# baoe/AlignGraph

Measured on AMD Instinct MI355X. Metric: aligned reads/sec through graph build+extend, higher is better.
Workload: dtype u32

## Files before the change

### aligngraph_amd/__init__.py

```python
import ctypes
import os

_HERE = os.path.dirname(os.path.abspath(__file__))
LIB_PATH = os.environ.get("AGX_LIB_PATH", os.path.join(_HERE, "libagx.so"))

AGX_OK, AGX_E_IO, AGX_E_FORMAT, AGX_E_UNSUPPORTED, AGX_E_ALIGNMENT, AGX_E_DEVICE, AGX_E_ARG, AGX_E_OVERFLOW, AGX_E_NOGPU = 0, -1, -2, -3, -4, -5, -6, -7, -8
AGX_FLAG_KEEP_COUNTS = 1
AGX_FLAG_SPARSE_MIN = 2
AGX_FLAG_TIME_SECTIONS = 4
AGX_FLAG_ONE_SHOT = 8
AGX_FLAG_KEEP_PATHS = 16
AGX_FLAG_EDGE_SUPPORT = 32

EXPORTS = [
    "agx_version", "agx_device_count", "agx_device_memory", "agx_selftest_scan", "agx_unit_create", "agx_unit_destroy", "agx_unit_error", "agx_unit_set_reference",
    "agx_unit_set_contig_threads", "agx_unit_push_pairs", "agx_unit_load_files", "agx_unit_upload", "agx_unit_build", "agx_unit_download",
    "agx_unit_finish", "agx_result_free", "agx_unit_stats", "agx_unit_graph", "agx_graph_free", "agx_run_unit",
    "agx_reads_open", "agx_reads_close", "agx_unit_load_files_shared", "agx_run_unit_shared",
    "agx_unit_stage", "agx_unit_release", "agx_pool_trim", "agx_unit_cache_build", "agx_unit_cache_save", "agx_unit_hbm_needed",
    "agx_unit_trim", "agx_unit_unitigs", "agx_unit_unitigs_region", "agx_unitigs_free", "agx_unitigs_gfa", "agx_text_free",
    "agx_unit_walk_graph", "agx_walk_graph_free", "agx_unit_front", "agx_front_free",
    "agx_unit_unitigs_mapped", "agx_idmap_free", "agx_unit_walk_paths", "agx_walk_paths_free", "agx_unitigs_paths_gfa", "agx_unit_reprune",
    "agx_unit_edge_support", "agx_edge_support_free", "agx_unit_unitigs_support", "agx_link_support_free", "agx_unitigs_gfa_support",
    "agx_unit_walk_evidence", "agx_walk_evidence_free", "agx_walk_evidence_bed",
    "agx_test_scan", "agx_test_zero", "agx_test_copy_out",
]


class Params(ctypes.Structure):
    _fields_ = [("k", ctypes.c_uint32), ("insert_variation", ctypes.c_uint32), ("coverage", ctypes.c_uint32),
                ("batch", ctypes.c_uint32), ("device", ctypes.c_int32), ("flags", ctypes.c_uint32)]


class Run(ctypes.Structure):
    _fields_ = [("q", ctypes.c_uint32), ("t", ctypes.c_uint32), ("n", ctypes.c_uint32)]


class Hit(ctypes.Structure):
    _fields_ = [("slot1", ctypes.c_uint32), ("pos1", ctypes.c_uint32), ("pos2", ctypes.c_uint32), ("runs1", ctypes.c_uint32),
                ("runs2", ctypes.c_uint32), ("nruns1", ctypes.c_uint16), ("nruns2", ctypes.c_uint16), ("len", ctypes.c_uint16),
                ("rev1", ctypes.c_uint8), ("rev2", ctypes.c_uint8), ("back", ctypes.c_uint8), ("pad", ctypes.c_uint8 * 3)]


class ContiMer(ctypes.Structure):
    _fields_ = [("cid", ctypes.c_uint32), ("coff", ctypes.c_uint32), ("next_off", ctypes.c_uint32), ("next_item", ctypes.c_uint32),
                ("nuc", ctypes.c_char), ("pad", ctypes.c_char * 3)]


class PairBatch(ctypes.Structure):
    _fields_ = [("hits", ctypes.POINTER(Hit)), ("n_hits", ctypes.c_uint64), ("runs", ctypes.POINTER(Run)), ("n_runs", ctypes.c_uint64),
                ("bases", ctypes.c_char_p), ("stride", ctypes.c_uint32), ("n_slots", ctypes.c_uint32)]


class Result(ctypes.Structure):
    _fields_ = [("initial_contigs", ctypes.c_void_p), ("initial_len", ctypes.c_size_t), ("pre_extended", ctypes.c_void_p),
                ("pre_len", ctypes.c_size_t), ("extended", ctypes.c_void_p), ("extended_len", ctypes.c_size_t)]


class Stats(ctypes.Structure):
    _fields_ = [(n, ctypes.c_uint64) for n in ("n_pos", "n_ref", "n_hits", "n_runs", "n_nodes", "n_tiles", "n_tile_entries", "n_big_tiles",
                                                "n_edge_overflow", "pairs_in_file", "sam_line_pairs")] + \
               [(n, ctypes.c_double) for n in ("ms_parse", "ms_thread", "ms_upload", "ms_prep", "ms_bin", "ms_node_sweep", "ms_node_big",
                                                "ms_edge_sweep", "ms_compact", "ms_download", "ms_walk")] + \
               [("node_sweep_launches", ctypes.c_uint32), ("edge_sweep_launches", ctypes.c_uint32)] + \
               [(n, ctypes.c_uint64) for n in ("n_walk_ids", "n_special", "n_fetched", "download_bytes")] + \
               [(n, ctypes.c_double) for n in ("ms_edge_fast", "ms_edge_slow")] + [("n_mid_tiles", ctypes.c_uint64), ("ms_build_span", ctypes.c_double)] + \
               [(n, ctypes.c_double) for n in ("ms_stage", "ms_upload_dev")] + \
               [(n, ctypes.c_uint64) for n in ("upload_bytes", "device_bytes", "pinned_bytes_cached", "device_bytes_cached", "n_spilled")] + \
               [("build_attempts", ctypes.c_uint32), ("from_cache", ctypes.c_uint32), ("dense_lists", ctypes.c_uint32), ("rows_by_reference", ctypes.c_uint32)] + \
               [("n_edge_slow", ctypes.c_uint64), ("reprune_attempts", ctypes.c_uint32), ("ms_reprune", ctypes.c_double)] + \
               [("ms_edge_support", ctypes.c_double), ("n_support_events", ctypes.c_uint64), ("ms_walk_evidence", ctypes.c_double)]


class Graph(ctypes.Structure):
    _fields_ = [("n_pos", ctypes.c_uint32), ("n_nodes", ctypes.c_uint32), ("n_edges", ctypes.c_uint32),
                ("node_start", ctypes.POINTER(ctypes.c_uint32)), ("node_key", ctypes.POINTER(ctypes.c_uint32)),
                ("node_cnt", ctypes.POINTER(ctypes.c_int32)), ("node_slen", ctypes.POINTER(ctypes.c_uint32)),
                ("edge_start", ctypes.POINTER(ctypes.c_uint32)), ("edge_dst", ctypes.POINTER(ctypes.c_uint32))]


class Unitigs(ctypes.Structure):
    _fields_ = [("n_segs", ctypes.c_uint32), ("n_links", ctypes.c_uint32), ("n_bases", ctypes.c_uint64),
                ("head_pos", ctypes.POINTER(ctypes.c_uint32)), ("head_var", ctypes.POINTER(ctypes.c_uint32)), ("n_nodes", ctypes.POINTER(ctypes.c_uint32)),
                ("last_pos", ctypes.POINTER(ctypes.c_uint32)), ("coverage", ctypes.POINTER(ctypes.c_uint64)), ("seq_off", ctypes.POINTER(ctypes.c_uint64)),
                ("seq", ctypes.c_void_p), ("link_from", ctypes.POINTER(ctypes.c_uint32)), ("link_to", ctypes.POINTER(ctypes.c_uint32))]


class EdgeSupport(ctypes.Structure):
    _fields_ = [("n_nodes", ctypes.c_uint32), ("n_edges", ctypes.c_uint32), ("n_events", ctypes.c_uint64), ("n_contributions", ctypes.c_uint64)] + \
               [(n, ctypes.POINTER(ctypes.c_uint32)) for n in ("edge_start", "edge_dst", "edge_cnt")]


class IdMap(ctypes.Structure):
    _fields_ = [("n_runs", ctypes.c_uint32), ("n_pos", ctypes.c_uint32), ("n_ids", ctypes.c_uint32)] + \
               [(n, ctypes.POINTER(ctypes.c_uint32)) for n in ("id_first", "id_last", "seg", "rank_first")]


class WalkPaths(ctypes.Structure):
    _fields_ = [("n_recs", ctypes.c_uint32), ("n_stretches", ctypes.c_uint64), ("rec_len", ctypes.POINTER(ctypes.c_uint64)), ("st_off", ctypes.POINTER(ctypes.c_uint64)),
                ("id_first", ctypes.POINTER(ctypes.c_uint32)), ("id_last", ctypes.POINTER(ctypes.c_uint32)), ("base_off", ctypes.POINTER(ctypes.c_uint64)),
                ("joined", ctypes.POINTER(ctypes.c_uint8))]


class WalkEvidence(ctypes.Structure):
# ... 269 lines not shown
    def load_files(self, tmp_dir, unit, reads=None):
        self._check(lib().agx_unit_load_files_shared(self._h, tmp_dir.encode(), unit, reads._h if reads is not None else None))

    def cache_save(self, tmp_dir, unit):
        self._check(lib().agx_unit_cache_save(self._h, tmp_dir.encode(), unit))

    def stage(self):
        self._check(lib().agx_unit_stage(self._h))

    def hbm_needed(self):
        v = ctypes.c_uint64(0)
        self._check(lib().agx_unit_hbm_needed(self._h, ctypes.byref(v)))
        return v.value

    def upload(self):
        self._check(lib().agx_unit_upload(self._h))

    def trim(self):
        v = ctypes.c_uint64(0)
        self._check(lib().agx_unit_trim(self._h, ctypes.byref(v)))
        return v.value

    def release(self):
        self._check(lib().agx_unit_release(self._h))

    def build(self):
        self._check(lib().agx_unit_build(self._h))

    def reprune(self, coverage):
        if not 0 <= int(coverage) <= 0xFFFFFFFF:
            raise AgxError(AGX_E_ARG, "reprune: coverage is an unsigned 32-bit number")
        self._check(lib().agx_unit_reprune(self._h, int(coverage)))
        self.params.coverage = int(coverage)

    def download(self):
        self._check(lib().agx_unit_download(self._h))

    def finish(self):
        r = Result()
        self._check(lib().agx_unit_finish(self._h, ctypes.byref(r)))
        return _take(r)

    def finish_views(self):
        r = Result()
        self._check(lib().agx_unit_finish(self._h, ctypes.byref(r)))
        return ResultViews(r)

    def stats(self):
        s = Stats()
        self._check(lib().agx_unit_stats(self._h, ctypes.byref(s)))
        return {n: getattr(s, n) for n, _ in Stats._fields_}

    def graph(self):
        import numpy as np
        g = Graph()
        self._check(lib().agx_unit_graph(self._h, ctypes.byref(g)))

        def arr(p, n, dt):
            return np.ctypeslib.as_array(p, shape=(n,)).astype(dt, copy=True) if n else np.zeros(0, dt)
        out = {"n_pos": g.n_pos, "n_nodes": g.n_nodes, "n_edges": g.n_edges,
               "node_start": arr(g.node_start, g.n_pos + 1, "uint32"), "node_key": arr(g.node_key, g.n_nodes * 6, "uint32").reshape(-1, 6),
               "node_cnt": arr(g.node_cnt, g.n_nodes * 6, "int32").reshape(-1, 6), "node_slen": arr(g.node_slen, g.n_nodes, "uint32"),
               "edge_start": arr(g.edge_start, g.n_nodes + 1, "uint32"), "edge_dst": arr(g.edge_dst, g.n_edges, "uint32")}
        lib().agx_graph_free(ctypes.byref(g))
        return out

    def walk_graph(self, streamed=False, all_node=False):
        g = WalkGraph()
        g.want_all_node = 1 if all_node else 0
        self._check(lib().agx_unit_walk_graph(self._h, 1 if streamed else 0, ctypes.byref(g)))
        try:
            return walk_graph_arrays(g)
        finally:
            lib().agx_walk_graph_free(ctypes.byref(g))

    def front(self):
        f = Front()
        self._check(lib().agx_unit_front(self._h, ctypes.byref(f)))
        try:
            return front_arrays(f)
        finally:
            lib().agx_front_free(ctypes.byref(f))

    def _window(self, region, min_coverage):
        lo, hi = region if region is not None else (0, self.stats()["n_pos"])
        cov = self.params.coverage if min_coverage is None else min_coverage
        for v in (lo, hi, cov):
            if not 0 <= int(v) <= 0xFFFFFFFF:
                raise AgxError(AGX_E_ARG, "unitigs: region bounds and min_coverage are unsigned 32-bit numbers")
        return int(lo), int(hi), int(cov)

    def _export(self, t, region, min_coverage):
        if region is None and min_coverage is None:
            self._check(lib().agx_unit_unitigs(self._h, ctypes.byref(t)))
            return
        self._check(lib().agx_unit_unitigs_region(self._h, *self._window(region, min_coverage), ctypes.byref(t)))

    def edge_support(self):
        import numpy as np
        s = EdgeSupport()
        self._check(lib().agx_unit_edge_support(self._h, ctypes.byref(s)))
        try:
            def arr(p, n):
                return np.ctypeslib.as_array(p, shape=(n,)).astype("uint32", copy=True) if n else np.zeros(0, "uint32")
            return {"n_nodes": s.n_nodes, "n_edges": s.n_edges, "n_events": s.n_events, "n_contributions": s.n_contributions,
                    "edge_start": arr(s.edge_start, s.n_nodes + 1), "edge_dst": arr(s.edge_dst, s.n_edges), "edge_cnt": arr(s.edge_cnt, s.n_edges)}
        finally:
            lib().agx_edge_support_free(ctypes.byref(s))

    def _export_support(self, t, region, min_coverage, m=None):
        sup = ctypes.POINTER(ctypes.c_uint32)()
        self._check(lib().agx_unit_unitigs_support(self._h, *self._window(region, min_coverage), ctypes.byref(t), ctypes.byref(sup), ctypes.byref(m) if m is not None else None))
        return sup

    def unitigs(self, region=None, min_coverage=None, id_map=False, edge_support=False):
        if edge_support:
            return self._unitigs_support(region, min_coverage, id_map)
        t = Unitigs()
        if not id_map:
            self._export(t, region, min_coverage)
            try:
                return _unitigs_arrays(t)
            finally:
                lib().agx_unitigs_free(ctypes.byref(t))
        m = IdMap()
        self._check(lib().agx_unit_unitigs_mapped(self._h, *self._window(region, min_coverage), ctypes.byref(t), ctypes.byref(m)))
        try:
            out = _unitigs_arrays(t)
            out["id_map"] = _idmap_arrays(m)
            return out
        finally:
            lib().agx_unitigs_free(ctypes.byref(t))
            lib().agx_idmap_free(ctypes.byref(m))

    def _unitigs_support(self, region, min_coverage, id_map):
        import numpy as np
        t, m = Unitigs(), IdMap() if id_map else None
        sup = self._export_support(t, region, min_coverage, m)
        try:
            out = _unitigs_arrays(t)
            out["link_support"] = np.ctypeslib.as_array(sup, shape=(t.n_links,)).astype("uint32", copy=True) if t.n_links else np.zeros(0, "uint32")
            if id_map:
                out["id_map"] = _idmap_arrays(m)
            return out
        finally:
            lib().agx_unitigs_free(ctypes.byref(t))
            lib().agx_link_support_free(sup)
            if id_map:
                lib().agx_idmap_free(ctypes.byref(m))

    def walk_paths(self):
        import numpy as np
        w = WalkPaths()
        self._check(lib().agx_unit_walk_paths(self._h, ctypes.byref(w)))
        try:
            def arr(p, n, dt):
                return np.ctypeslib.as_array(p, shape=(n,)).astype(dt, copy=True) if n else np.zeros(0, dt)
            nr, ns = w.n_recs, w.n_stretches
            return {"rec_len": arr(w.rec_len, nr, "uint64"), "st_off": arr(w.st_off, nr + 1, "uint64"), "id_first": arr(w.id_first, ns, "uint32"),
                    "id_last": arr(w.id_last, ns, "uint32"), "base_off": arr(w.base_off, ns, "uint64"), "joined": arr(w.joined, ns, "uint8")}
        finally:
            lib().agx_walk_paths_free(ctypes.byref(w))

    def walk_evidence(self, w=None, min_depth=0, min_support=0, tracks=False, records=None):
        import numpy as np
        if w is None:
# ... 184 lines not shown
```

### aligngraph_amd/csrc/agx_core.h

```cpp
#pragma once
#include <stdint.h>
#include "../../include/agx.h"

#if defined(__HIPCC__)
#define AGX_HD __host__ __device__ __forceinline__
#else
#define AGX_HD inline
#endif

typedef uint32_t agx_u32;
typedef uint16_t agx_u16;
typedef uint8_t agx_u8;

#define AGX_NONE 0xFFFFFFFFu
#define AGX_TILE 64u
#ifndef AGX_REGION_TILES
#define AGX_REGION_TILES 32u
#endif
#define AGX_REGION_PAD 32u
#ifndef AGX_MAXV_LDS
#define AGX_MAXV_LDS 2u
#endif
#ifndef AGX_SWEEP_FIRST
#define AGX_SWEEP_FIRST 1
#endif
#define AGX_MAXV_MID 4u
#define AGX_MAXV_BIG 64u
#define AGX_MAXV_HUGE 1024u
#define AGX_MAXE 4u
#define AGX_EP25 25



enum { AGX_WF_REV1 = 1, AGX_WF_REV2 = 2, AGX_WF_LEFT2 = 4, AGX_WF_RUNS1 = 8, AGX_WF_RUNS2 = 16,
       AGX_WF_DUP = 32 };
struct agx_whit {
    agx_u32 a, b, row;
    agx_u16 len; agx_u8 flags, back;
};
struct agx_wside { agx_u32 runs1, runs2, nruns; };
struct agx_wrun { agx_u32 t; agx_u16 q, n; };
AGX_HD agx_whit agx_pack_hit(const agx_hit &h, agx_u32 side_index) {
    agx_whit w; w.a = h.nruns1 ? 0u : h.pos1; w.b = h.nruns2 ? 0u : h.pos2; w.row = h.slot1; w.len = h.len; w.back = h.back;
    w.flags = (agx_u8)((h.rev1 ? AGX_WF_REV1 : 0) | (h.rev2 ? AGX_WF_REV2 : 0) | ((h.pad[0] & 1u) ? AGX_WF_LEFT2 : 0) | (h.nruns1 ? AGX_WF_RUNS1 : 0) | (h.nruns2 ? AGX_WF_RUNS2 : 0));
    if (h.nruns1) w.a = side_index; else if (h.nruns2) w.b = side_index;
    return w;
}
AGX_HD agx_hit agx_unpack_hit(const agx_whit &w, const agx_wside *sides) {
    agx_hit h; h.slot1 = w.row; h.len = w.len; h.back = w.back; h.rev1 = (w.flags & AGX_WF_REV1) ? 1 : 0; h.rev2 = (w.flags & AGX_WF_REV2) ? 1 : 0;
    h.pad[0] = (w.flags & AGX_WF_LEFT2) ? 1 : 0; h.pad[1] = h.pad[2] = 0;
    h.pos1 = (w.flags & AGX_WF_RUNS1) ? 0u : w.a; h.pos2 = (w.flags & AGX_WF_RUNS2) ? 0u : w.b; h.runs1 = h.runs2 = 0; h.nruns1 = h.nruns2 = 0;
    if (w.flags & (AGX_WF_RUNS1 | AGX_WF_RUNS2)) {
        const agx_wside sd = sides[(w.flags & AGX_WF_RUNS1) ? w.a : w.b];
        if (w.flags & AGX_WF_RUNS1) { h.runs1 = sd.runs1; h.nruns1 = (agx_u16)(sd.nruns & 0xFFFFu); }
        if (w.flags & AGX_WF_RUNS2) { h.runs2 = sd.runs2; h.nruns2 = (agx_u16)(sd.nruns >> 16); }
    }
    return h;
}
struct agx_refx { agx_u32 pos, len, byte; };
AGX_HD agx_u32 agx_ref_code(agx_u32 c) { return c == 'A' ? 0u : c == 'C' ? 1u : c == 'G' ? 2u : c == 'T' ? 3u : 4u; }
AGX_HD char agx_ref_base(agx_u32 code) { return (char)((0x54474341u >> (8u * (code & 3u))) & 0xFFu); }

struct agx_cmkey { agx_u32 cid, coff; };
struct agx_cmhead { agx_u32 cid, coff, n, start; };


enum { AGX_HF_AREV = 1, AGX_HF_SKIP = 2, AGX_HF_BNONE = 4 };

struct agx_dhit {
    agx_u32 a_t0, b_t0;
    agx_u32 a_runs, b_runs;
    agx_u32 a_slot;
    agx_u16 len, jstar;
    agx_u16 a_nruns, b_nruns;
    agx_u32 flags;
    agx_u32 x_lo, x_hi;
};


enum { AGX_NF_DEAD = 1, AGX_NF_CONTIG = 2, AGX_NF_EOVF = 4 };

struct agx_sref { agx_u32 slot; agx_u32 qlen; };

enum { AGX_F_CID = 0, AGX_F_COFF, AGX_F_CID0, AGX_F_COFF0, AGX_F_OFF0, AGX_F_COV, AGX_F_A, AGX_F_C, AGX_F_G, AGX_F_T, AGX_F_N, AGX_F_S0, AGX_F_S1, AGX_NF };
static_assert(AGX_F_C == AGX_F_A + 1 && AGX_F_G == AGX_F_A + 2 && AGX_F_T == AGX_F_A + 3 && AGX_F_N == AGX_F_A + 4, "agx_class_vote_code relies on the order of the vote counters");

struct agx_key { agx_u32 cid, coff, cid0, coff0, off0; };

AGX_HD int agx_absdiff(agx_u32 a, agx_u32 b) { int d = (int)(a - b); return d < 0 ? -d : d; }

AGX_HD agx_u32 agx_within(agx_u32 a, agx_u32 b, int win) { return (agx_u32)(a - b + (agx_u32)win) <= 2u * (agx_u32)win ? 1u : 0u; }
AGX_HD agx_u32 agx_clause_ab(agx_u32 ac, agx_u32 ao, agx_u32 bc, agx_u32 bo, int win) {
    return ((agx_u32)(ac != bc) | (agx_u32)(ac == AGX_NONE) | agx_within(ao, bo, win)) & 1u;
}
AGX_HD agx_u32 agx_clause_c(agx_u32 ao, agx_u32 bo, int win) { return ((agx_u32)(ao == AGX_NONE) | (agx_u32)(bo == AGX_NONE) | agx_within(ao, bo, win)) & 1u; }

#if defined(__HIP_DEVICE_COMPILE__)
AGX_HD agx_u32 agx_uload(const agx_u32 *p, size_t i) { return ((const __attribute__((address_space(4))) agx_u32 *)p)[i]; }
#else
AGX_HD agx_u32 agx_uload(const agx_u32 *p, size_t i) { return p[i]; }
#endif

struct agx_bucket { agx_u32 *base; agx_u32 stride; agx_u32 maxv; agx_u32 packed; };
#define AGX_NFP 10u
static_assert(AGX_F_COV == AGX_F_OFF0 + 1 && AGX_F_A == AGX_F_COV + 1 && AGX_F_S0 == AGX_F_N + 1 && AGX_NFP == AGX_NF - 3,
              "packed buckets: the six counters from AGX_F_COV on pair up into three words, and agx_b maps S0 / S1 three words down");
AGX_HD agx_u32 &agx_b(const agx_bucket &b, agx_u32 v, agx_u32 f) { return b.base[(b.packed ? v * AGX_NFP + (f >= (agx_u32)AGX_F_S0 ? f - 3u : f) : v * AGX_NF + f) * b.stride]; }
AGX_HD agx_u32 &agx_cnt_word(const agx_bucket &b, agx_u32 v, agx_u32 f) { return b.base[(v * AGX_NFP + (agx_u32)AGX_F_COV + ((f - (agx_u32)AGX_F_COV) >> 1)) * b.stride]; }
template <bool LDS_ADD> AGX_HD void agx_bucket_add(agx_u32 &ref, agx_u32 val) {
#if defined(__HIP_DEVICE_COMPILE__)
    if (LDS_ADD) { (void)__hip_atomic_fetch_add(&ref, val, __ATOMIC_RELAXED, __HIP_MEMORY_SCOPE_WAVEFRONT); return; }
#endif
    ref += val;
}
AGX_HD agx_u32 agx_cnt_get(const agx_bucket &b, agx_u32 v, agx_u32 f) {
    if (b.packed) return (agx_cnt_word(b, v, f) >> (16u * ((f - (agx_u32)AGX_F_COV) & 1u))) & 0xFFFFu;
    return agx_b(b, v, f);
}
template <bool LDS_ADD> AGX_HD void agx_cnt_add(const agx_bucket &b, agx_u32 v, agx_u32 f, agx_u32 val) {
    if (b.packed) agx_bucket_add<LDS_ADD>(agx_cnt_word(b, v, f), val << (16u * ((f - (agx_u32)AGX_F_COV) & 1u)));
    else agx_bucket_add<LDS_ADD>(agx_b(b, v, f), val);
}
AGX_HD void agx_cnt_init(const agx_bucket &b, agx_u32 v, agx_u32 cov) {
    if (b.packed) { agx_cnt_word(b, v, AGX_F_COV) = cov; agx_cnt_word(b, v, AGX_F_C) = 0; agx_cnt_word(b, v, AGX_F_T) = 0; }
    else { agx_b(b, v, AGX_F_COV) = cov; agx_b(b, v, AGX_F_A) = 0; agx_b(b, v, AGX_F_C) = 0; agx_b(b, v, AGX_F_G) = 0; agx_b(b, v, AGX_F_T) = 0; agx_b(b, v, AGX_F_N) = 0; }
}

AGX_HD bool agx_compatible(const agx_key &k, const agx_bucket &b, agx_u32 v, int iv) {
    const agx_u32 c = agx_b(b, v, AGX_F_CID), o = agx_b(b, v, AGX_F_COFF), c0 = agx_b(b, v, AGX_F_CID0), o0 = agx_b(b, v, AGX_F_COFF0), m = agx_b(b, v, AGX_F_OFF0);
    return (agx_clause_ab(k.cid, k.coff, c, o, AGX_EP25) & agx_clause_ab(k.cid0, k.coff0, c0, o0, 2 * iv + AGX_EP25) & agx_clause_c(k.off0, m, 2 * iv + AGX_EP25)) != 0;
}


AGX_HD agx_u32 agx_pos_b(const agx_dhit &d, const agx_run *runs, agx_u32 q) {
    if (d.b_nruns == 0) return d.b_t0 + q;
    agx_u32 res = AGX_NONE;
    for (agx_u32 i = 0; i < d.b_nruns; i++) { const agx_run r = runs[d.b_runs + i]; const agx_u32 o = q - r.q; res = (q >= r.q && o < r.n) ? r.t + o : res; }
    return res;
}

// ... 1032 lines not shown
```

### aligngraph_amd/csrc/agx_engine.cpp

```cpp
#include <hip/hip_runtime_api.h>
#include <hsa/hsa.h>
#include <hsa/hsa_ext_amd.h>
#include <fcntl.h>
#include <sys/stat.h>
#include <unistd.h>

#include <algorithm>
#include <chrono>
#include <cstdio>
#include <cstdlib>
#include <cstring>
#include <memory>
#include <string>
#include <mutex>
#include <system_error>
#include <thread>
#include <type_traits>
#include <pthread.h>
#include <atomic>
#include <condition_variable>
#include <functional>
#include <vector>

#include "agx_host.h"
// ... 102 lines not shown
                try { f(); } catch (...) { }
                l.lock(); running[s] = false; cv.notify_all();
            }
        });
        started = true;
    }
    bool submit(int s, std::function<void()> f) {
        if (!started) return false;
        std::unique_lock<std::mutex> l(m);
        cv.wait(l, [&] { return !queued[s] && !running[s]; });
        job[s] = std::move(f); queued[s] = true; cv.notify_all();
        return true;
    }
    void wait(int s) { if (!started) return; std::unique_lock<std::mutex> l(m); cv.wait(l, [&] { return !queued[s] && !running[s]; }); }
    ~UnitHelper() { if (started) { { std::lock_guard<std::mutex> l(m); stop = true; } cv.notify_all(); th.join(); } }
};

struct WalkerPool {
    enum { N = 64 };
    struct Slot { std::thread th; std::mutex m; std::condition_variable cv; std::function<void()> job; bool queued = false, running = false, taken = false, stop = false; };
    Slot slot[N]; std::mutex take_m; bool started = false;
    void start() {
        if (started) return;
        started = true;
        for (Slot &s : slot) {
            try {
                s.th = std::thread([&s] {
                    pthread_setname_np(pthread_self(), "agx-walker");
                    std::unique_lock<std::mutex> l(s.m);
                    for (;;) {
                        s.cv.wait(l, [&s] { return s.stop || s.queued; });
                        if (s.stop) return;
                        std::function<void()> f = std::move(s.job); s.queued = false; s.running = true;
                        l.unlock();
                        try { f(); } catch (...) { }
                        l.lock(); s.running = false; s.cv.notify_all();
                    }
                });
            } catch (...) { s.taken = true; }
        }
    }
    int take() { std::lock_guard<std::mutex> l(take_m); start(); for (int i = 0; i < N; i++) if (!slot[i].taken) { slot[i].taken = true; return i; } return -1; }
    void give(int i) { std::lock_guard<std::mutex> l(take_m); slot[i].taken = false; }
    void run(int i, std::function<void()> f) { Slot &s = slot[i]; std::unique_lock<std::mutex> l(s.m); s.cv.wait(l, [&s] { return !s.queued && !s.running; }); s.job = std::move(f); s.queued = true; s.cv.notify_all(); }
    void wait(int i) { Slot &s = slot[i]; std::unique_lock<std::mutex> l(s.m); s.cv.wait(l, [&s] { return !s.queued && !s.running; }); }
    ~WalkerPool() { for (Slot &s : slot) if (s.th.joinable()) { { std::lock_guard<std::mutex> l(s.m); s.stop = true; } s.cv.notify_all(); s.th.join(); } }
};
WalkerPool &walker_pool() { static WalkerPool p; return p; }
inline int walkers_now(size_t n_pos) {
    const int want = walkers_wanted(n_pos);
    if (want <= 4 || getenv("AGX_WALK_SPLIT_WALKERS")) return want;
    static const int ranks = [] { const char *e = getenv("LOCAL_WORLD_SIZE"); const int n = e ? atoi(e) : 1; return n < 1 ? 1 : n; }();
    const int cpus = (int)usable_cpus() / ranks;
    return want <= cpus ? want : cpus < 4 ? 4 : cpus;
}

static std::atomic<int> g_walks_pending{0};
static std::atomic<int> g_units_alive{0};

struct agx_unit {
    agx_params prm{};
    std::string err;
    Threads T; Pairs P;
    UnitView V;
    size_t n_chain_str = 0;
    struct Mapped { void *p = nullptr; size_t n = 0; void reset() { if (p) munmap(p, n); p = nullptr; n = 0; } ~Mapped() { reset(); } } cache_map;
    agx_u32 n_seg0 = 0, stride = 0, n_slots = 0, n_rows = 0; unsigned long long pairs_in_file = 0, sam_pairs = 0;
    bool have_ref = false, have_threads = false, staged = false, uploaded = false, built = false, downloaded = false;
    bool consumed = false;
    bool pending_walk = false;
    bool trimmed = false;
    bool expanded = false;
    hipEvent_t ev_built = nullptr;
    UnitOutput out; OutBuf out_initial; bool out_ready = false;
    UnitHelper helper;
    hsa_signal_t dl_signal{}; hsa_agent_t dl_agent{}; bool dl_sdma = false;
    enum { DL_SIGNALS = AGX_DL_PIECES + 2 };
    hsa_signal_t dl_piece[DL_SIGNALS] = {}; bool dl_piece_made = false, dl_streaming = false; agx_cut_args cuts{}; agx_u32 cut_main[AGX_DL_PIECES + 1] = {}, cut_side[AGX_DL_PIECES + 1] = {};
    double dl_t0 = 0, dl_est_ms = 0; size_t dl_stream_bytes = 0; std::atomic<bool> dl_timed{false};
    DevArena arena;
    PBuf<agx_whit> s_hits; PBuf<agx_wside> s_sides; PBuf<agx_wrun> s_runs; PBuf<agx_u8> s_codes; PBuf<unsigned long long> s_other; PBuf<agx_u32> s_jump; size_t n_other = 0, n_sides = 0, n_jump = 0;
    PBuf<agx_u8> s_ref; PBuf<agx_refx> s_refx; size_t n_refx = 0; bool ref_packed = false;
    PBuf<agx_u32> s_chain_end, s_region_off; PBuf<agx_cmseg> s_segs; size_t n_segs = 0;
    PBuf<agx_whit> s_hits_t; PBuf<agx_u8> s_codes_t; PBuf<unsigned long long> s_other_t; size_t n_other_t = 0; bool tiled = false; std::vector<agx_u32> slot_row;
    agx_u32 front_windows = 1;
    agx_u32 n_win = 1, win_tile[9] = {};
    hipEvent_t ev_rows[8] = {}, ev_win[8] = {}, ev_sw0[8] = {}, ev_sw1[8] = {};
    PBuf<agx_u32> s_perm, s_tfirst, s_jump_at; agx_u32 lookback = 2;
    PBuf<char> s_landing;
    PBuf<agx_cntrun> s_cntruns; PBuf<agx_chunk> s_cntchunks, s_segchunks; PBuf<agx_u32> s_segindex; size_t n_cntruns = 0, n_cntchunks = 0, n_segchunks = 0, n_segindex = 0;
    PBuf<agx_u16> s_units; PBuf<agx_u8> s_rowcnt; PBuf<agx_u32> s_blockoff, s_blockfirst, s_anchor; size_t n_units = 0, n_rowcnt = 0, n_blockoff = 0, n_blockfirst = 0, n_anchor = 0, n_rows_explicit = 0; bool rows_diffed = false;
    size_t nh = 0, n_runs = 0, n_cm = 0, n_codes = 0; agx_u32 maxlen = 0;
    std::vector<agx_u32> row_slot;
    std::vector<uint64_t> row_off;
    std::shared_ptr<agx::ReadsIndex> reads_keep;
    std::unique_ptr<agx::FileView> reads_map;
    bool pairs_staged = false;
    agx::PairsFile pairs_file;
    DBuf<agx_u32> d_cm_start; DBuf<agx_cmkey> d_cm; DBuf<agx_cmhead> d_cm_head; DBuf<char> d_ref; DBuf<agx_cmseg> d_segs;
    DBuf<agx_run> d_runs; DBuf<agx_u8> d_codes, d_vcodes; DBuf<unsigned long long> d_other;
    DBuf<agx_u16> d_units; DBuf<agx_u8> d_rowcnt; DBuf<agx_u32> d_blockoff, d_blockfirst, d_anchor;
    DBuf<agx_cntrun> d_cntruns; DBuf<agx_chunk> d_cntchunks, d_segchunks; DBuf<agx_u32> d_jump, d_segindex;
    DBuf<agx_whit> d_whits; DBuf<agx_wside> d_wsides; DBuf<agx_wrun> d_wruns; DBuf<agx_u8> d_wref; DBuf<agx_refx> d_refx;
    DBuf<agx_dhit> d_dhit; DBuf<agx_u32> d_tile_cnt, d_tile_off, d_cursor, d_unsorted, d_tile_recs, d_scan_tmp, d_words; DBuf<unsigned long long> d_scan_desc; size_t scan_desc_n = 0;
    agx_u32 pool_cap = 0, spill_lo = 0, ovf_cap = 0, list_cap = 0, sp_cap = 0;
    DBuf<agx_u32> d_pool_cnt, d_region_off; agx_u32 n_regions = 0;
    DBuf<agx_u32> d_node_start, d_slow_list, d_perm, d_tfirst, d_ckey, d_long; DBuf<agx_u16> d_node_cnt; DBuf<agx_u8> d_pos_succ;
    DBuf<agx_u32> d_cid, d_coff, d_cid0, d_coff0, d_off0, d_next; DBuf<agx_u8> d_base, d_flags; DBuf<agx_sref> d_sref; DBuf<int> d_counts;
    DBuf<agx_u32> d_e_cnt, d_ovf_cnt, d_sup_tot, d_lsup;
    bool support_valid = false; uint64_t sup_events = 0, sup_adds = 0;
    DBuf<char> d_ut;
    DBuf<agx_edge_ovf> d_ovf; DBuf<agx_u32> d_mid_list, d_big_list, d_scratch, d_huge_list, d_scratch_huge; bool huge = false, dense = false;
    agx_u32 n_ids = 0;
    DBuf<agx_u32> d_side_pk, d_tile_side, d_tile_side_start, d_aid_of; DBuf<char> d_a_str;
    DBuf<agx_u8> d_a_meta, d_a_mark; DBuf<agx_walknode> d_fetch, d_sp_node; DBuf<agx_u32> d_a_nid; DBuf<agx_edge_ovf> d_a_ovf; agx_compact_args walk_args{};
    DBuf<agx_u32> d_chain_end, d_side_xpos, d_sp_cnt, d_sp_rank; DBuf<unsigned long long> d_sp_bits;
    agx_u32 n_chain_end = 0, n_special = 0, n_words = 0;
    size_t keep_end = 0;
    PBuf<char> h_a_str; PBuf<agx_u8> h_a_meta; PBuf<agx_u32> h_side_xpos, h_sp_rank; PBuf<unsigned long long> h_sp_bits;
    PBuf<agx_walknode> h_sp_node, h_fetch; PBuf<agx_edge_ovf> h_a_ovf; PBuf<agx_hop> h_sp_hop; DBuf<agx_hop> d_sp_hop;
    PBuf<agx_u32> h_words;
    agx_u32 n_nodes = 0, n_ovf = 0, n_tiles = 0, n_tile_entries = 0, n_big = 0, n_mid = 0, n_slow = 0;
    Boundaries ev; hipEvent_t ev_front = nullptr, ev_passA = nullptr, ev_passJ = nullptr, ev_up0 = nullptr, ev_uploaded = nullptr, ev_dl = nullptr, ev_hits = nullptr;
    bool up_timed = false;
    agx_stats stats{};
    ~agx_unit() {
        arena.reset();
        if (pending_walk) g_walks_pending.fetch_sub(1);
        ev.destroy();
        for (hipEvent_t e : {ev_front, ev_passA, ev_passJ, ev_up0, ev_uploaded, ev_dl, ev_built, ev_hits}) if (e) (void)hipEventDestroy(e);
        for (auto *arr : {ev_rows, ev_win, ev_sw0, ev_sw1}) for (int i = 0; i < 8; i++) if (arr[i]) (void)hipEventDestroy(arr[i]);
        if (dl_signal.handle) (void)hsa_signal_destroy(dl_signal);
        if (dl_piece_made) for (hsa_signal_t g : dl_piece) if (g.handle) (void)hsa_signal_destroy(g);
    }
};

namespace {

struct DeviceTurn { std::mutex m; hipStream_t main = nullptr, front = nullptr, up = nullptr, down = nullptr;
                    hipEvent_t sweep_done[2] = {nullptr, nullptr}, build_done[2] = {nullptr, nullptr};
                    unsigned long long n = 0; bool prev_exclusive = false; hipEvent_t prev_node = nullptr;
                    std::mutex up_m, down_m, make_m;
                    void make() {
                        std::lock_guard<std::mutex> l(make_m);
                        if (main) return;
                        HIP_OK(hipStreamCreateWithFlags(&up, hipStreamNonBlocking)); HIP_OK(hipStreamCreateWithFlags(&front, hipStreamNonBlocking));
                        HIP_OK(hipStreamCreateWithFlags(&down, hipStreamNonBlocking));
                        for (auto &e : sweep_done) HIP_OK(hipEventCreateWithFlags(&e, hipEventDisableTiming));
                        for (auto &e : build_done) HIP_OK(hipEventCreateWithFlags(&e, hipEventDisableTiming));
                        HIP_OK(hipStreamCreateWithFlags(&main, hipStreamNonBlocking));
                    } };
DeviceTurn &turn_of(int device) { static DeviceTurn turns[64]; return turns[device & 63]; }

static const bool g_trace_gap = getenv("AGX_TRACE_GAP") != nullptr;
static const bool g_scan1 = getenv("AGX_SCAN_LEGACY") == nullptr;
static const bool g_debug_sync = getenv("AGX_DEBUG_SYNC") != nullptr;
#define g_tiny (getenv("AGX_TEST_SMALL_CAPS") != nullptr)
#define AGX_CHECKPOINT(name) do { if (g_debug_sync) { hipError_t e_ = hipStreamSynchronize(st); fprintf(stderr, "[agx debug] %s: %s\n", name, hipGetErrorString(e_)); } } while (0)

void join_dl_helper(agx_unit *u);
void drop_outputs(agx_unit *u);
void start_helper(agx_unit *u);

enum { W_CUT = 34 , W_TOTAL = W_CUT + 2 * (AGX_DL_PIECES + 1) };
enum { W_ERR = 0, W_POOL = 1, W_BIGCOUNT = 2, W_STATUS = 3, W_OVFCOUNT = 4, W_SLOWCOUNT = 5, W_LONGCOUNT = 6 , W_UNUSED7 = 7, W_MIDCOUNT = 8, W_JUMPCOUNT = 9, W_SPILL = 10, W_HUGECOUNT = 11, W_N = 12 };

agx_cut_args stream_cuts(agx_u32 n_pos) {
    agx_cut_args C; memset(&C, 0, sizeof C);
    const char *force = getenv("AGX_STREAM_PIECES");
    if (getenv("AGX_NO_STREAM_DOWNLOAD") || n_pos < 4096) return C;
    size_t m = force ? (size_t)atoi(force) : n_pos < AGX_TWO_WALKERS_MIN ? 0 : n_pos / 4000000u;
    if (!force && m && m < 2) m = 2;
    if (m > AGX_DL_PIECES) m = AGX_DL_PIECES;
    if (m > n_pos / 1024u) m = n_pos / 1024u;
    for (size_t w = 0; w < m; w++) C.word[w] = (agx_u32)(((unsigned long long)n_pos * w / m) >> 6);
    C.word[m] = n_pos >> 6; C.n = (agx_u32)m;
    return C;
}

void fill_sweep_args(agx_unit *u, agx_sweep_args &S) {
    memset(&S, 0, sizeof S);
    S.cm_start = u->d_cm_start.p; S.cm = u->d_cm.p; S.cm_head = u->d_cm_head.p; S.ref = u->d_ref.p;
    S.dhit = u->d_dhit.p; S.runs = u->d_runs.p; S.vcodes = u->d_vcodes.p; S.stride = u->stride;
    S.tile_off = u->d_tile_off.p; S.tile_recs = (decltype(S.tile_recs))u->d_tile_recs.p;
    S.n_pos = (agx_u32)u->V.n_pos; S.n_tiles = u->n_tiles; S.k = u->prm.k; S.iv = (int)u->prm.insert_variation; S.coverage = (int)u->prm.coverage;
    S.node_start = u->d_node_start.p; S.node_cnt = u->d_node_cnt.p; S.pos_succ = u->d_pos_succ.p; S.side_pk = u->d_side_pk.p; S.tile_side = u->d_tile_side.p;
    S.nk_cid = u->d_cid.p; S.nk_coff = u->d_coff.p; S.nk_cid0 = u->d_cid0.p; S.nk_coff0 = u->d_coff0.p; S.nk_off0 = u->d_off0.p;
    S.n_base = u->d_base.p; S.n_flags = u->d_flags.p; S.n_sref = u->d_sref.p; S.n_next = u->d_next.p;
    S.n_counts = (u->prm.flags & AGX_FLAG_KEEP_COUNTS) ? u->d_counts.p : nullptr;
    S.pool_cap = u->pool_cap;
    S.sweep_stats = nullptr;
}

inline bool want_tiled() { return !getenv("AGX_NO_TILED_UPLOAD"); }
template <class B> inline void alloc_file_order(B &buf, size_t count) { if (want_tiled()) buf.alloc_plain(count); else buf.alloc(count); }
void *alloc_pair_array(agx_unit *u, int which, size_t bytes) {
    switch (which) {
    case SA_HITS:  alloc_file_order(u->s_hits, bytes / sizeof(agx_whit) + 1); return u->s_hits.p;
    case SA_SIDES: u->s_sides.alloc(bytes / sizeof(agx_wside) + 1); return u->s_sides.p;
    case SA_RUNS:  u->s_runs.alloc(bytes / sizeof(agx_wrun) + 1); return u->s_runs.p;
    case SA_CODES: alloc_file_order(u->s_codes, bytes); return u->s_codes.p;
    case SA_JUMP:  u->s_jump.alloc(bytes / 4 + 1); return u->s_jump.p;
    default:       u->s_other.alloc(bytes / 8 + 1); return u->s_other.p;
    }
}
void alloc_pair_arrays(agx_unit *u) {
    alloc_pair_array(u, SA_HITS, u->nh * sizeof(agx_whit)); alloc_pair_array(u, SA_SIDES, u->n_sides * sizeof(agx_wside)); alloc_pair_array(u, SA_JUMP, u->n_jump * 4);
    alloc_pair_array(u, SA_RUNS, u->n_runs * sizeof(agx_wrun)); alloc_pair_array(u, SA_CODES, u->n_codes + 16); alloc_pair_array(u, SA_OTHER, u->n_other * 8);
}
struct UnitSink : StageSink {
    agx_unit *u; explicit UnitSink(agx_unit *x) : u(x) {}
    void *take(int which, size_t bytes) override { return alloc_pair_array(u, which, bytes); }
};
void adopt_pairs(agx_unit *u, StagedPairs &S) {
    u->nh = S.nh; u->n_runs = S.n_runs; u->n_sides = S.n_sides; u->n_jump = S.n_jump; u->n_codes = S.n_codes; u->n_other = S.n_other; u->stride = S.stride; u->maxlen = S.maxlen;
    u->pairs_in_file = S.n_pairs_in_file; u->sam_pairs = S.n_sam_pairs;
    u->row_off.swap(S.row_off); u->row_slot.swap(S.row_slot); u->n_rows = S.n_rows;
}
void stage_cm_layout(agx_unit *u, const agx_u8 *cm_cnt, size_t n_pos, const agx_cmseg *segs, size_t n_segs) {
    CmLayout L; build_cm_layout(cm_cnt, n_pos, segs, n_segs, L);
    u->n_cntruns = L.cnt_runs.size(); u->n_cntchunks = L.cnt_chunks.size(); u->n_segchunks = L.seg_chunks.size();
    u->s_cntruns.alloc(u->n_cntruns + 1); u->s_cntchunks.alloc(u->n_cntchunks + 1); u->s_segchunks.alloc(u->n_segchunks + 1);
    if (u->n_cntruns) memcpy(u->s_cntruns.p, L.cnt_runs.data(), u->n_cntruns * sizeof(agx_cntrun));
    if (u->n_cntchunks) memcpy(u->s_cntchunks.p, L.cnt_chunks.data(), u->n_cntchunks * sizeof(agx_chunk));
    if (u->n_segchunks) memcpy(u->s_segchunks.p, L.seg_chunks.data(), u->n_segchunks * sizeof(agx_chunk));
    build_seg_index(segs, u->n_seg0, n_pos, L.seg_index);
    u->n_segindex = L.seg_index.size(); u->s_segindex.alloc(u->n_segindex + 1); memcpy(u->s_segindex.p, L.seg_index.data(), u->n_segindex * 4);
}
void stage_reference(agx_unit *u, const char *ref, size_t n_pos, unsigned threads) {
    std::vector<agx_refx> others;
    u->s_ref.alloc((n_pos + 3) / 4 + 32);
    u->ref_packed = getenv("AGX_REF_RAW") == nullptr && pack_reference(ref, n_pos, std::min(threads, 8u), u->s_ref.p, others);
    if (u->ref_packed) { u->n_refx = others.size(); u->s_refx.alloc(u->n_refx + 1); if (u->n_refx) memcpy(u->s_refx.p, others.data(), u->n_refx * sizeof(agx_refx)); return; }
    u->n_refx = 0; u->s_ref.alloc(n_pos + 16);
    const unsigned T = std::max(1u, std::min(threads, 8u));
    on_threads(T, [&](unsigned t) { const size_t lo = n_pos * t / T, hi = n_pos * (t + 1) / T; memcpy(u->s_ref.p + lo, ref + lo, hi - lo); });
}
struct GraphCounts { size_t n_pos, n_ids, n_special, n_ovf; };
enum { GA_BITS = 0, GA_RANK, GA_STR, GA_META, GA_XPOS, GA_NODE, GA_HOP, GA_OVF, GA_N };
template <class F> void graph_arrays(agx_unit *u, const GraphCounts &c, F f) {
    const size_t words = c.n_ids / 64 + 1, sides = c.n_ids - c.n_pos;
    f(GA_BITS, u->h_sp_bits, u->d_sp_bits, words, 1); f(GA_RANK, u->h_sp_rank, u->d_sp_rank, words, 1);
    f(GA_STR, u->h_a_str, u->d_a_str, c.n_ids, 1); f(GA_META, u->h_a_meta, u->d_a_meta, c.n_ids, 64);
    f(GA_XPOS, u->h_side_xpos, u->d_side_xpos, sides, 1);
    f(GA_NODE, u->h_sp_node, u->d_sp_node, c.n_special, 1); f(GA_HOP, u->h_sp_hop, u->d_sp_hop, c.n_special, 2);
    f(GA_OVF, u->h_a_ovf, u->d_a_ovf, c.n_ovf, 1);
}
const int GRAPH_CUT_ORDER[GA_N] = {GA_NODE, GA_META, GA_STR, GA_HOP, GA_XPOS, GA_BITS, GA_RANK, GA_OVF};
inline GraphCounts graph_counts(const agx_unit *u) { return GraphCounts{u->V.n_pos, u->n_ids, u->n_special, u->n_ovf}; }
inline size_t graph_bytes(agx_unit *u, const GraphCounts &c) {
    size_t sum = 0; graph_arrays(u, c, [&](int, auto &h, auto &, size_t n, size_t) { sum += n * sizeof(*h.p); }); return sum;
}
inline GraphCounts helper_estimate(size_t n_pos) { const size_t ni = n_pos + n_pos / 8 + 4096; return GraphCounts{n_pos, ni, ni / 8 + 4096, 63}; }
inline GraphCounts landing_estimate(size_t n_pos) { const size_t ni = n_pos + n_pos / 16 + 4096; return GraphCounts{n_pos, ni, ni / 10 + 4096, 0}; }

const int LANDING_ROOMS = 8;
template <class F> void landing_rooms(agx_unit *u, F f) {
    f(u->s_codes, true); f(u->s_hits, true); f(u->s_landing, false); f(u->s_codes_t, true); f(u->s_hits_t, true); f(u->s_runs, true); f(u->s_sides, true); f(u->s_other, true);
}

void reserve_landing(agx_unit *u) {
    if (!(u->prm.flags & AGX_FLAG_ONE_SHOT)) { u->s_landing.release(); return; }
    const GraphCounts c = landing_estimate(u->V.n_pos); const size_t ni = c.n_ids, ns = c.n_special;
    const size_t need = 2 * (ni + 512) + ns * (sizeof(agx_walknode) + sizeof(agx_hop)) + ni / 4 + (4u << 20);
    size_t have = 0; landing_rooms(u, [&](auto &b, bool input) { if (input) have += b.block_bytes(); });
    if (need > have * 85 / 100) u->s_landing.alloc(need - have * 85 / 100 + (ni + 512)); else u->s_landing.release();
}
void adopt_row_diffs(agx_unit *u, const RowDiffs &D, unsigned threads) {
    u->n_units = D.n_units; u->n_rowcnt = D.cnt.size(); u->n_blockoff = D.block_off.size(); u->n_blockfirst = D.block_first.size(); u->n_anchor = D.anchor_bits.size(); u->n_rows_explicit = D.n_explicit;
    u->s_units.alloc(u->n_units + 2); u->s_rowcnt.alloc(u->n_rowcnt); u->s_blockoff.alloc(u->n_blockoff); u->s_blockfirst.alloc(u->n_blockfirst); u->s_anchor.alloc(u->n_anchor);
    const unsigned T = std::max(1u, std::min(threads, 8u));
    on_threads(T, [&](unsigned t) { const size_t lo = u->n_units * t / T, hi = u->n_units * (t + 1) / T; if (hi > lo) memcpy(u->s_units.p + lo, D.units.data() + lo, (hi - lo) * 2); });
    memcpy(u->s_rowcnt.p, D.cnt.data(), u->n_rowcnt); memcpy(u->s_blockoff.p, D.block_off.data(), u->n_blockoff * 4); memcpy(u->s_blockfirst.p, D.block_first.data(), u->n_blockfirst * 4); memcpy(u->s_anchor.p, D.anchor_bits.data(), u->n_anchor * 4);
    u->rows_diffed = true;
}
void stage_rows(agx_unit *u, unsigned threads) {
    u->rows_diffed = false; u->n_units = u->n_rowcnt = u->n_blockoff = u->n_blockfirst = u->n_anchor = u->n_rows_explicit = 0;
    const char *on = getenv("AGX_ROW_DIFF");
    if (want_tiled()) return;
    if (!on || atoi(on) == 0 || !u->ref_packed || u->n_rows == 0 || u->nh == 0) return;
    const double t0 = now_ms();
    RowDiffs D;
    if (!build_row_diffs(u->s_hits.p, u->nh, u->s_sides.p, u->n_sides, u->s_runs.p, u->n_runs, u->s_codes.p, u->n_rows, u->stride, (const agx_u32 *)u->s_ref.p, u->V.n_pos ? u->V.n_pos : u->T.ref.size(), threads, D)) return;
    if (D.n_units * 2 + D.cnt.size() + (D.block_off.size() + D.block_first.size() + D.anchor_bits.size()) * 4 >= u->n_codes) return;
    adopt_row_diffs(u, D, threads);
    if (getenv("AGX_LOAD_TIMING")) fprintf(stderr, "[agx load] read rows against the reference: %.1f ms, %zu rows (%zu as they are), %.1f -> %.1f bytes per row\n", now_ms() - t0, (size_t)u->n_rows, u->n_rows_explicit,
                                          (double)u->n_codes / u->n_rows, (double)(u->n_units * 2 + u->n_rowcnt + (u->n_blockoff + u->n_blockfirst + u->n_anchor) * 4) / u->n_rows);
}
void stage_order(agx_unit *u, unsigned threads) {
    const double t0 = now_ms();
    const size_t n_pos = u->V.n_pos ? u->V.n_pos : u->T.ref.size(), n_tiles = (n_pos + AGX_TILE - 1) / AGX_TILE;
    u->lookback = agx_tile_lookback(u->maxlen, u->prm.k);
    u->s_perm.alloc(u->nh + 1); u->s_tfirst.alloc(n_tiles + 2); u->s_jump_at.alloc(u->n_jump + 1);
    order_hits(u->s_hits.p, u->nh, u->s_sides.p, u->s_runs.p, u->s_jump.p, u->n_jump, n_pos, threads, u->s_perm.p, u->s_tfirst.p, u->s_jump_at.p);
    if (getenv("AGX_LOAD_TIMING")) fprintf(stderr, "[agx load] hits in tile order: %.1f ms (%zu hits, %zu tiles, window of %u tiles)\n", now_ms() - t0, u->nh, n_tiles, u->lookback);
}
void stage_tiled(agx_unit *u, unsigned threads) {
    u->tiled = false; u->n_other_t = 0; u->slot_row.clear(); u->n_win = 1;
    const size_t nh = u->nh, s4 = u->stride / 4;
    if (u->rows_diffed || getenv("AGX_NO_TILED_UPLOAD") || nh == 0 || u->n_rows == 0) { u->s_hits_t.release(); u->s_codes_t.release(); u->s_other_t.release(); return; }
    const double t0 = now_ms();
    u->s_hits_t.alloc(nh + 1); u->s_codes_t.alloc(nh * s4 + 16); u->slot_row.resize(nh);
    const agx_whit *wh = u->s_hits.p; const agx_wside *sd = u->s_sides.p; const agx_wrun *wr = u->s_runs.p; const agx_u32 *perm = u->s_perm.p;
    const size_t n_rows = u->n_rows; std::vector<agx_u8> has_other((n_rows + 7) / 8, 0);
    for (size_t j = 0; j < u->n_other; j++) { const size_t r = (size_t)(u->s_other.p[j] / u->stride); if (r < n_rows) has_other[r >> 3] |= (agx_u8)(1u << (r & 7)); }
    auto idx0 = [&](const agx_whit &w) -> agx_u32 {
        if (!(w.flags & AGX_WF_RUNS1)) return w.a;
        const agx_wside &g = sd[w.a]; const agx_wrun &r = wr[g.runs1];
        return r.q == 0 ? r.t : AGX_NONE;
    };
    const unsigned T = std::max(1u, std::min(threads, 16u));
    std::vector<std::vector<unsigned long long>> others(T);
    on_threads(T, [&](unsigned t) {
        const size_t AHEAD = 48, NEAR = 24;
        for (size_t i = nh * t / T, hi = nh * (t + 1) / T; i < hi; i++) {
            if (i + AHEAD < hi) __builtin_prefetch(wh + perm[i + AHEAD]);
            if (i + NEAR < hi) { const char *c = (const char *)(u->s_codes.p + (size_t)wh[perm[i + NEAR]].row * s4); __builtin_prefetch(c); if (s4 > 40) __builtin_prefetch(c + 64); }
            const agx_u32 h = perm[i]; agx_whit w = wh[h];
            const agx_u32 row = w.row;
            u->slot_row[i] = row;
            memcpy(u->s_codes_t.p + i * s4, u->s_codes.p + (size_t)row * s4, s4);
            bool dup = false;
            if (w.back) { const agx_u32 me = idx0(w); for (agx_u32 e = 1; e <= w.back && !dup; e++) dup = agx_absdiff(me, idx0(wh[h - e])) < (int)w.len; }
            w.row = h; if (dup) w.flags |= (agx_u8)AGX_WF_DUP;
            u->s_hits_t.p[i] = w;
            if (has_other[row >> 3] & (1u << (row & 7))) {
                const unsigned long long lo = (unsigned long long)row * u->stride, *b = u->s_other.p, *e = b + u->n_other;
                for (const unsigned long long *at = std::lower_bound(b, e, lo); at != e && *at < lo + u->stride; ++at) others[t].push_back((unsigned long long)i * u->stride + (*at - lo));
            }
        }
    });
    size_t no = 0; for (auto &v : others) no += v.size();
    u->s_other_t.alloc(no + 1); u->n_other_t = no;
    { size_t at = 0; for (auto &v : others) { if (!v.empty()) memcpy(u->s_other_t.p + at, v.data(), v.size() * 8); at += v.size(); } }
    u->tiled = true;
    const size_t n_pos = u->V.n_pos ? u->V.n_pos : u->T.ref.size(), n_tiles = (n_pos + AGX_TILE - 1) / AGX_TILE;
    size_t W = getenv("AGX_UPLOAD_WINDOWS") ? (size_t)atoi(getenv("AGX_UPLOAD_WINDOWS")) : n_pos / 8000000u;
    W = std::max<size_t>(1, std::min<size_t>(std::min<size_t>(W, 8), n_tiles));
    u->n_win = (agx_u32)W;
    for (size_t w = 0; w <= W; w++) u->win_tile[w] = (agx_u32)(n_tiles * w / W);
    if (getenv("AGX_LOAD_TIMING")) fprintf(stderr, "[agx load] tile-ordered upload forms: %.1f ms (%zu hits, %zu listed bases, %u windows)\n", now_ms() - t0, nh, no, u->n_win);
}

void stage_rows_tiled(agx_unit *u, unsigned threads) {
    if (!u->tiled || !u->ref_packed || u->stride > AGX_ROW_MAXSTRIDE) return;
    const char *env = getenv("AGX_ROW_DIFF");
    const size_t n_pos = u->V.n_pos ? u->V.n_pos : u->T.ref.size();
    if (!env || atoi(env) == 0) return;
    const double t0 = now_ms();
    RowDiffs D;
    if (!build_row_diffs(u->s_hits_t.p, u->nh, u->s_sides.p, u->n_sides, u->s_runs.p, u->n_runs, u->s_codes_t.p, u->nh, u->stride, (const agx_u32 *)u->s_ref.p, n_pos, threads, D, true)) return;
    if (D.n_units * 2 + D.cnt.size() + (D.block_off.size() + D.block_first.size() + D.anchor_bits.size()) * 4 >= u->nh * (u->stride / 4)) return;
    adopt_row_diffs(u, D, threads);
    if (getenv("AGX_LOAD_TIMING")) fprintf(stderr, "[agx load] tile-ordered rows against the reference: %.1f ms, %zu rows (%zu as they are), %.1f -> %.1f bytes per row\n", now_ms() - t0, u->nh, u->n_rows_explicit,
                                          (double)(u->stride / 4), (double)(u->n_units * 2 + u->n_rowcnt + (u->n_blockoff + u->n_blockfirst + u->n_anchor) * 4) / u->nh);
}

void finish_staging(agx_unit *u, unsigned threads_rows, unsigned threads) {
    stage_rows(u, threads_rows);
    stage_order(u, threads);
    stage_tiled(u, threads);
    stage_rows_tiled(u, threads);
    u->V.slot_row = u->tiled ? u->slot_row.data() : nullptr;
    reserve_landing(u);
    u->staged = true; u->consumed = false; u->uploaded = false; u->built = false; u->downloaded = false;
}

void stage_inputs(agx_unit *u) {
    if (!u->have_ref || !u->have_threads) throw Error{E_ARG, "reference and contig threads must be set before upload"};
    if (u->consumed && u->pairs_staged) throw Error{E_ARG, "one-shot unit: its staged read alignments were overwritten by the download; load the unit again"};
    const double t0 = now_ms();
    HIP_OK(hipSetDevice(u->prm.device));
    u->cache_map.reset(); u->reads_map.reset();
    const size_t n_pos = u->T.ref.size();
    if (n_pos == 0 || n_pos >= 0xFFFFFF00ull) throw Error{E_ARG, "unit sequence is empty or too long"};
    if (u->T.cm_cnt.size() != n_pos) throw Error{E_ARG, "conti-mer chains were not built"};
    { size_t el = 0; for (const agx_cmseg &g : u->T.segs) el += g.len; if (el != u->T.n_cm) throw Error{E_ARG, "conti-mer runs were not built"}; }
    u->n_seg0 = u->T.n_seg0; u->n_cm = u->T.n_cm;
    u->n_segs = u->T.segs.size(); u->s_segs.alloc(u->n_segs + 1);
    if (u->n_segs) memcpy(u->s_segs.p, u->T.segs.data(), u->n_segs * sizeof(agx_cmseg));
    std::vector<agx_u32> ce(u->T.chain_end_pos); std::sort(ce.begin(), ce.end()); ce.erase(std::unique(ce.begin(), ce.end()), ce.end());
    u->n_chain_end = (agx_u32)ce.size(); u->s_chain_end.alloc(ce.size() + 1);
    if (!ce.empty()) memcpy(u->s_chain_end.p, ce.data(), ce.size() * 4);
    const unsigned threads = loader_threads(u->P.bases.size() + n_pos + u->nh * 64);
    stage_reference(u, u->T.ref.data(), n_pos, threads);
    stage_cm_layout(u, u->T.cm_cnt.data(), n_pos, u->T.segs.data(), u->n_segs);
    if (!u->pairs_staged) {
        UnitSink sink(u); StagedPairs S;
        u->n_slots = u->P.n_slots;
        stage_pairs(u->P, u->prm.k, threads, sink, S);
        adopt_pairs(u, S);
    }
    UnitView V = view_of(u->T, u->P);
    if (u->pairs_staged && u->pairs_file.fv) {
        const agx::PairsFile &F = u->pairs_file;
        V.bases = nullptr; V.row_off = nullptr; V.stride = u->stride; V.codes2 = (const agx_u8 *)F.sec(pairsfile::S_CODES);
        V.other_idx = (const unsigned long long *)F.sec(pairsfile::S_OTHER); V.other_byte = (const agx_u8 *)F.sec(pairsfile::S_OTHERB); V.n_other = (size_t)F.H.n_other;
    } else if (u->pairs_staged) { V.bases = u->reads_keep ? u->reads_keep->fv.p : nullptr; V.stride = u->stride; V.row_off = u->row_off.data(); }
    u->V = V; u->n_chain_str = u->T.chain_str.size();
    finish_staging(u, threads, threads);
    u->stats.ms_stage = now_ms() - t0;
}

namespace cache {
enum { S_HITS = 0, S_RUNS, S_CODES, S_SEGS, S_CHAIN_END, S_ROWS, S_REF, S_CM_CNT, S_CHAIN_STR, S_INITIAL, S_BASES, S_OTHER, S_SIDES, S_JUMP, S_OTHERB, S_N };
struct Header {
    char magic[8]; agx_u32 version, batch; unsigned long long stamp[6][2];
    unsigned long long n_pos, n_ref, nh, n_runs, n_cm, n_segs, n_seg0, n_rows, n_chain_end, n_codes, pairs_in_file, sam_pairs;
    agx_u32 stride, maxlen, n_slots, k;
    agx_u32 rows_in_reads;
    agx_u32 slot_stride;
    unsigned long long n_sides, n_jump;
    agx_u32 sizes[5];
    unsigned long long off[S_N], len[S_N];
};
const char MAGIC[8] = {'A', 'G', 'X', 'U', 'N', 'I', 'T', '7'};
void stamps(const std::string &d, int unit, unsigned long long st[6][2]) {
    const std::string s = std::to_string(unit);
    const std::string f[6] = {d + "/_genome." + s + ".fa", d + "/_contigs.fa", d + "/_contigs_genome." + s + ".psl", d + "/_reads.fa", d + "/_reads_genome." + s + ".bowtie", pairsfile::path_of(d, unit)};
    for (int i = 0; i < 6; i++) { struct stat sb; if (stat(f[i].c_str(), &sb) != 0) { st[i][0] = st[i][1] = ~0ull; continue; }
        st[i][0] = (unsigned long long)sb.st_size; st[i][1] = (unsigned long long)sb.st_mtim.tv_sec * 1000000000ull + (unsigned long long)sb.st_mtim.tv_nsec; }
}
std::string path_of(const std::string &d, int unit) { return d + "/_agx_unit." + std::to_string(unit) + ".bin"; }
}

struct Piece { char *mem; unsigned long long off, len; };
void cut_pieces(std::vector<Piece> &pieces, const void *mem, unsigned long long off, unsigned long long len) {
    for (unsigned long long a = 0; a < len; a += 32ull << 20) pieces.push_back(Piece{(char *)mem + a, off + a, std::min<unsigned long long>(32ull << 20, len - a)});
// ... 140 lines not shown
            });
            unsigned long long total = 0; for (unsigned t = 0; t < threads; t++) { total += part[t]; fine = fine && !bad3[t]; }
            fine = fine && total == H.n_cm;
        }
        for (size_t i = 0; i < u->n_chain_end && fine; i++) fine = u->s_chain_end.p[i] < H.n_pos;
        if (fine && in_reads) { const uint64_t *ro = (const uint64_t *)(base + H.off[S_ROWS]); for (size_t r = 0; r < H.n_rows && fine; r++) fine = ro[r] + H.maxlen <= reads_map->n && ro[r] < reads_map->n; }
        if (fine && !in_reads && !from_codes) { const agx_u32 *rs = (const agx_u32 *)(base + H.off[S_ROWS]); for (size_t r = 0; r < H.n_rows && fine; r++) fine = rs[r] < H.n_slots; }
        for (size_t i = 1; i < u->n_other && fine && from_codes; i++) fine = u->s_other.p[i - 1] < u->s_other.p[i];
    }
    if (!fine) { u->cache_map.reset(); return false; }
    const double tv = now_ms();
    stage_reference(u, base + H.off[S_REF], H.n_pos, threads);
    const double tr = now_ms();
    stage_cm_layout(u, (const agx_u8 *)(base + H.off[S_CM_CNT]), H.n_pos, u->s_segs.p, u->n_segs);
    if (getenv("AGX_LOAD_TIMING")) fprintf(stderr, "[agx load] cache: buffers + read + checks %.1f ms, reference %.1f ms, conti-mer layout %.1f ms\n", tv - t0, tr - tv, now_ms() - tr);
    UnitView V; V.ref = base + H.off[S_REF]; V.n_pos = H.n_pos; V.n_ref = (agx_u32)H.n_ref; V.cm_cnt = (const agx_u8 *)(base + H.off[S_CM_CNT]); V.chain_str = base + H.off[S_CHAIN_STR];
    V.hop = nullptr; V.segs = (const agx_cmseg *)(base + H.off[S_SEGS]); V.n_seg0 = (agx_u32)H.n_seg0; V.stride = (in_reads || from_codes) ? H.stride : H.slot_stride; V.initial = base + H.off[S_INITIAL]; V.n_initial = H.len[S_INITIAL];
    u->row_off.clear(); u->row_slot.clear();
    if (from_codes) { V.bases = nullptr; V.codes2 = (const agx_u8 *)(base + H.off[S_CODES]); V.other_idx = (const unsigned long long *)(base + H.off[S_OTHER]); V.other_byte = (const agx_u8 *)(base + H.off[S_OTHERB]); V.n_other = u->n_other; }
    else if (in_reads) { u->reads_map = std::move(reads_map); V.bases = u->reads_map->p; V.row_off = (const uint64_t *)(base + H.off[S_ROWS]); }
    else { V.bases = base + H.off[S_BASES]; u->row_slot.assign((const agx_u32 *)(base + H.off[S_ROWS]), (const agx_u32 *)(base + H.off[S_ROWS]) + H.n_rows); }
    u->V = V; u->n_chain_str = (size_t)H.len[S_CHAIN_STR]; u->pairs_staged = false;
    finish_staging(u, std::max(threads, std::min(8u, usable_cpus())), std::max(threads, std::min(16u, usable_cpus())));
    u->have_ref = u->have_threads = true;
    u->stats.ms_stage = now_ms() - t0; u->stats.ms_parse = 0; u->stats.ms_thread = 0; u->stats.from_cache = 1;
    return true;
}

agx_u32 spill_min(const agx_unit *u) { const size_t n_pos = u->V.n_pos; return (agx_u32)std::min<size_t>(g_tiny ? 64 : n_pos / 8 + 65536, 0x10000000u); }

unsigned long long layout_regions(agx_unit *u, const agx_u32 *demand, agx_u32 main_cap, bool apply, hipStream_t st, size_t *sent = nullptr) {
    const agx_u32 R = u->n_regions;
    u->s_region_off.alloc((size_t)R + 1);
    agx_u32 *off = u->s_region_off.p;
    unsigned long long at = 0;
    for (agx_u32 r = 0; r < R; r++) {
        off[r] = (agx_u32)std::min<unsigned long long>(at, 0xFFFFFFFFull);
        at += demand ? (unsigned long long)demand[r] + demand[r] / 8 + 64 : main_cap / R;
    }
    const unsigned long long need = at + spill_min(u);
    if (!apply || need > u->pool_cap) return need;
    off[R] = (agx_u32)at; u->spill_lo = (agx_u32)at;
    HIP_OK(hipMemcpyAsync(u->d_region_off.p, off, ((size_t)R + 1) * 4, hipMemcpyHostToDevice, st));
    if (sent) *sent += ((size_t)R + 1) * 4;
    return need;
}

struct Take {
    DevArena *arena = nullptr; size_t bytes = 0;
    template <class B> void operator()(B &b, size_t count) {
        bytes += (count * sizeof(*b.p) + 255) & ~(size_t)255;
        if constexpr (!std::is_const_v<B>) if (arena) { b.release(); b.alloc(*arena, count); }
    }
    template <class M> void note(M &member, size_t v) { if constexpr (!std::is_const_v<M>) if (arena) member = (M)v; }
};
inline size_t codes_bytes(const agx_unit *u) { return u->tiled ? u->nh * (u->stride / 4) : u->n_codes; }
inline size_t others_up(const agx_unit *u) { return u->tiled ? u->n_other_t : u->n_other; }
inline agx_u32 tiles_of(const agx_unit *u) { return (agx_u32)((u->V.n_pos + AGX_TILE - 1) / AGX_TILE); }
inline agx_u32 regions_of(const agx_unit *u) { return (tiles_of(u) + AGX_REGION_TILES - 1) / AGX_REGION_TILES; }
inline agx_u32 words_of(const agx_unit *u, agx_u32 pool_cap) { return (agx_u32)((u->V.n_pos + pool_cap) / 64 + 1); }
inline size_t scan_desc_of(const agx_unit *u, agx_u32 pool_cap) { return (std::max<size_t>(tiles_of(u), words_of(u, pool_cap)) + 1) / 4096 + 2; }

template <class U> void pool_bufs(U *u, agx_u32 cap, Take &t) {
    const size_t n_pos = u->V.n_pos, ids_cap = n_pos + cap, n_words = words_of(u, cap);
    t.note(u->pool_cap, cap); t.note(u->n_words, n_words); t.note(u->scan_desc_n, scan_desc_of(u, cap));
    const size_t kcap = (size_t)cap + AGX_SLOW_V;
    t(u->d_aid_of, (size_t)cap + 1); t(u->d_a_nid, ids_cap + 1); t(u->d_off0, kcap); t(u->d_sref, cap); t(u->d_next, (size_t)cap * AGX_MAXE); t(u->d_fetch, 65536);
    t.note(u->keep_end, t.arena ? t.arena->first_block_at() : 0);
    t(u->d_cid, kcap); t(u->d_coff, kcap); t(u->d_cid0, kcap); t(u->d_coff0, kcap); t(u->d_base, cap); t(u->d_flags, cap);
    if (u->prm.flags & AGX_FLAG_KEEP_COUNTS) t(u->d_counts, (size_t)cap * 6);
    if (u->prm.flags & AGX_FLAG_EDGE_SUPPORT) t(u->d_e_cnt, (size_t)cap * AGX_MAXE);
    t(u->d_a_str, ids_cap + 1); t(u->d_a_meta, ids_cap + 16); t(u->d_a_mark, ids_cap + 2); t(u->d_side_xpos, (size_t)cap + 1);
    t(u->d_sp_bits, n_words + 1); t(u->d_sp_cnt, n_words + 1); t(u->d_sp_rank, n_words + 2);
    const size_t nb = (std::max<size_t>(n_pos, n_words) + 1 + 1023) / 1024;
    t(u->d_scan_tmp, 2 * (nb + 1) + 2 * ((nb + 1023) / 1024 + 1) + 16); t(u->d_scan_desc, 3 * scan_desc_of(u, cap));
}
template <class U> void fixed_bufs(U *u, Take &t) {
    const size_t n_pos = u->V.n_pos, nh = u->nh, n_tiles = tiles_of(u), n_regions = regions_of(u);
    t(u->d_cm_start, n_pos + 2); t(u->d_cm, u->n_cm + 1); t(u->d_ref, n_pos + 16); t(u->d_cm_head, n_pos + 1);
    t(u->d_segs, u->n_segs + 1); t(u->d_cntruns, u->n_cntruns + 1); t(u->d_cntchunks, u->n_cntchunks + 1); t(u->d_segchunks, u->n_segchunks + 1); t(u->d_segindex, u->n_segindex + 1);
    t(u->d_runs, u->n_runs + 1); t(u->d_vcodes, codes_bytes(u) * 4 + 16); t(u->d_other, others_up(u) + 1);
    if (u->rows_diffed) { t(u->d_units, u->n_units + 2); t(u->d_rowcnt, u->n_rowcnt); t(u->d_blockoff, u->n_blockoff); t(u->d_blockfirst, u->n_blockfirst); t(u->d_anchor, u->n_anchor); }
    else t(u->d_codes, codes_bytes(u) + 16);
    t(u->d_whits, nh + 1); t(u->d_wsides, u->n_sides + 1); t(u->d_wruns, u->n_runs + 1); t(u->d_jump, u->n_jump + 1);
    if (u->ref_packed) { t(u->d_wref, (n_pos + 3) / 4 + 32); t(u->d_refx, u->n_refx + 1); }
    t(u->d_dhit, nh + 1);
    t(u->d_perm, nh + 1); t(u->d_tfirst, n_tiles + 2); t(u->d_ckey, nh + 1); t(u->d_long, AGX_LONG_MAX);
    t(u->d_tile_cnt, n_tiles + 1); t(u->d_tile_off, n_tiles + 2); t(u->d_cursor, n_tiles + 1);
    t(u->d_words, W_TOTAL);
    t(u->d_chain_end, (size_t)u->n_chain_end + 1);
    t(u->d_node_start, n_pos); t(u->d_node_cnt, n_pos); t(u->d_pos_succ, n_pos); t(u->d_slow_list, n_pos + 64);
    t(u->d_side_pk, n_pos + 2); t(u->d_tile_side, n_tiles + 2); t(u->d_tile_side_start, n_tiles + 2);
    t(u->d_big_list, n_tiles + 1); t(u->d_mid_list, n_tiles + 1);
    t(u->d_scratch, (size_t)AGX_BIG_WAVES * AGX_NF * AGX_MAXV_BIG * 64);
    t(u->d_region_off, n_regions + 1); t(u->d_pool_cnt, n_regions * AGX_REGION_PAD);
    if (u->prm.flags & AGX_FLAG_EDGE_SUPPORT) t(u->d_sup_tot, 2 * n_tiles + 2);
}
template <class U> void list_bufs(U *u, agx_u32 cap, Take &t) { t.note(u->list_cap, cap); t(u->d_unsorted, (size_t)cap + 1); t(u->d_tile_recs, ((size_t)cap + 4) * 8); }
template <class U> void ovf_bufs(U *u, agx_u32 cap, Take &t) { t.note(u->ovf_cap, cap); t(u->d_ovf, cap); t(u->d_a_ovf, (size_t)cap + 1); if (u->prm.flags & AGX_FLAG_EDGE_SUPPORT) t(u->d_ovf_cnt, cap); }
template <class U> void sparse_bufs(U *u, agx_u32 cap, Take &t) { t.note(u->sp_cap, cap); t(u->d_sp_node, (size_t)cap + 1); t(u->d_sp_hop, (size_t)cap + 2); }

void do_release(agx_unit *u);

struct Carve {
    char *base; size_t at = 0;
    template <class T> void operator()(T *&p, size_t n) { at = (at + 255) & ~(size_t)255; p = base ? (T *)(base + at) : nullptr; at += (n ? n : 1) * sizeof(T); }
    size_t bytes() const { return at + 256; }
};
inline size_t scan_words(size_t n, size_t block) { return 2 * ((n + block - 1) / block + 1) + 2 * ((n + block * block - 1) / (block * block) + 1); }

size_t unitig_layout(size_t cap, size_t n_pos, size_t n_ovf, char *base, agx_unitig_args *A, agx_u32 **words) {
    Carve take{base};
    agx_unitig_args T{}; agx_unitig_args &X = A ? *A : T; agx_u32 *w = nullptr, *R = nullptr;
    size_t hash_n = 64; while (hash_n < 2 * n_ovf) hash_n *= 2;
    const size_t nwin = (cap + 63) / 64, nmax = std::max(std::max(cap, n_pos), nwin) + 1;
    take(w, 8); take(R, 5 * cap + n_ovf);
    take(X.indeg, cap); take(X.succ, cap); take(X.osucc, cap); take(X.nxt, cap); take(X.haspred, cap);
    take(X.ovf_hash, hash_n); take(X.ovf_first, n_ovf); take(X.wcnt, nwin + 1); take(X.woff, nwin + 1);
    for (int i = 0; i < 2; i++) { take(X.anc[i], cap); take(X.off[i], cap); }
    take(X.p_seg, cap); take(X.hcnt, n_pos + 1); take(X.hoff, n_pos + 1);
    take(X.s_len, cap + 1); take(X.s_links, cap + 1); take(X.s_hpos, cap); take(X.s_hvar, cap); take(X.s_last, cap); take(X.s_cov, cap);
    take(X.s_off, cap + 1); take(X.l_off, cap + 1); take(X.l_cur, cap + 1);
    take(X.scan_tmp, scan_words(nmax, 4096) + 8);
    if (base) {
        X.pos_of = R; X.outs = R + cap; X.oout = R + 2 * cap; X.p_len = R + 3 * cap; X.p_next = R + 4 * cap;
        X.l_to = R; X.link_cap = (agx_u32)std::min<size_t>(5 * cap + n_ovf, 0xFFFFFFFFull); X.seq = (char *)X.succ; X.seq_cap = (agx_u32)std::min<size_t>(4 * cap, 0xFFFFFFFFull);
        X.hash_mask = (agx_u32)(hash_n - 1);
        if (words) *words = w;
    }
    return take.bytes();
}

size_t unitig_region_layout(size_t cap, size_t n_win, size_t kept, size_t n_ovf, char *base, agx_unitig_region_args *A, agx_u32 **words) {
    Carve take{base};
    agx_unitig_region_args T{}; agx_unitig_region_args &R = A ? *A : T; agx_unitig_args &X = R.U; agx_u32 *w = nullptr, *L = nullptr;
    size_t hash_n = 64; while (hash_n < 2 * n_ovf) hash_n *= 2;
    const size_t ngrp = (kept + 63) / 64, nmax = std::max(n_win, cap) + 1;
    take(w, 8); take(R.rmap, cap); take(R.cntw, n_win + 1); take(R.offw, n_win + 1);
    take(X.scan_tmp, scan_words(nmax, 4096) + 8);
    take(X.ovf_hash, hash_n); take(X.ovf_first, n_ovf);
    take(R.l_slot, kept); take(X.pos_of, kept); take(L, 4 * kept + n_ovf);
    take(X.indeg, kept); take(X.succ, kept); take(X.osucc, kept); take(X.nxt, kept); take(X.haspred, kept);
    take(X.wcnt, ngrp + 1); take(X.woff, ngrp + 1); take(X.hcnt, ngrp + 1); take(X.hoff, ngrp + 1);
    for (int i = 0; i < 2; i++) { take(X.anc[i], kept + 1); take(X.off[i], kept + 1); }
    take(X.p_seg, kept);
    take(X.s_len, kept + 1); take(X.s_links, kept + 1); take(X.s_hpos, kept); take(X.s_hvar, kept); take(X.s_last, kept); take(X.s_cov, kept);
    if (base) {
        X.outs = L; X.oout = L + kept; X.p_len = L + 2 * kept; X.p_next = L + 3 * kept;
        X.l_to = L; X.link_cap = (agx_u32)std::min<size_t>(4 * kept + n_ovf, 0xFFFFFFFFull); X.seq = (char *)X.succ; X.seq_cap = (agx_u32)std::min<size_t>(4 * kept, 0xFFFFFFFFull);
        X.s_off = X.anc[0]; X.l_off = X.off[0]; X.l_cur = X.anc[1];
        X.hash_mask = (agx_u32)(hash_n - 1);
        if (words) *words = w;
    }
    return take.bytes();
}

size_t idmap_layout(size_t ids, size_t runs, char *base, agx_idmap_args *A) {
    Carve take{base};
    agx_idmap_args T{}; agx_idmap_args &M = A ? *A : T;
    take(M.flag, ids + 1); take(M.foff, ids + 1);
    take(M.scan_tmp, scan_words(ids + 1, 1024) + 16);
    take(M.r_first, runs); take(M.r_last, runs); take(M.r_seg, runs); take(M.r_rank, runs);
    return take.bytes();
}
size_t evidence_layout(size_t n_st, size_t n_recs, size_t chunk, bool tracks, char *base, agx_evidence_args *A, agx_u32 **words) {
    Carve take{base};
    agx_evidence_args T{}; agx_evidence_args &E = A ? *A : T; agx_u32 *w = nullptr;
    take(w, 8);
    take(E.T.st_first, n_st); take(E.T.st_base, n_st); take(E.T.st_rec, n_st); take(E.T.st_pre, n_st + 1); take(E.T.st_join, n_st + 1);
    take(E.r_steps, n_recs); take(E.r_dsum, n_recs); take(E.r_dmin, n_recs); take(E.r_smin, n_recs);
    take(E.c_depth, chunk); take(E.c_step, chunk);
    if (tracks) take(E.c_votes, chunk);
    take(E.flag, chunk + 1); take(E.foff, chunk + 1); take(E.scan_tmp, scan_words(chunk + 1, 1024) + 16);
    take(E.iv_rec, chunk); take(E.iv_first, chunk); take(E.iv_last, chunk); take(E.iv_dmin, chunk); take(E.iv_smin, chunk);
    if (base) { E.noedge = w + 1; E.err = w; if (words) *words = w; }
    return take.bytes();
}
inline bool keeps_paths(const agx_unit *u) { return (u->prm.flags & (AGX_FLAG_KEEP_PATHS | AGX_FLAG_KEEP_COUNTS)) == (AGX_FLAG_KEEP_PATHS | AGX_FLAG_KEEP_COUNTS); }
size_t mapped_scratch(size_t cap, size_t n_pos, size_t n_nodes, size_t n_ids, size_t n_ovf, size_t *map_at) {
    const size_t kept = std::min(n_nodes, cap), sides = n_ids > n_pos ? n_ids - n_pos : 0;
    const size_t front = (std::max(unitig_layout(cap, n_pos, n_ovf, nullptr, nullptr, nullptr), unitig_region_layout(cap, n_pos, kept, n_ovf, nullptr, nullptr, nullptr)) + 255) & ~(size_t)255;
    if (map_at) *map_at = front;
    return front + idmap_layout(n_pos + sides, std::min(kept, n_pos + sides), nullptr, nullptr);
}

struct Plan { agx_u32 pool_cap, list_cap, ovf_cap, sp_cap; size_t exact, total; };
inline size_t win_row(const agx_unit *u, agx_u32 w) { const size_t a = u->rows_diffed ? 63 : 15;
    return w == 0 ? 0 : w >= u->n_win ? u->nh : std::min<size_t>(u->nh, ((size_t)u->s_tfirst.p[u->win_tile[w]] + a) & ~a); }
inline size_t regrow_slack(size_t exact) { return exact / 64 + (64u << 10) * 100; }
Plan plan_capacities(const agx_unit *u) {
    const size_t n_pos = u->V.n_pos, nh = u->nh;
    Plan P;
    const agx_u32 main_cap = (agx_u32)std::min<size_t>(g_tiny ? n_pos / 8 + 64 : n_pos + n_pos / 4 + 4096, 0xE0000000ull);
    P.pool_cap = u->pool_cap ? u->pool_cap : main_cap + spill_min(u);
    const double per_hit = 1.0 + (u->maxlen > u->prm.k ? (double)(u->maxlen - u->prm.k) : 0.0) / AGX_TILE;
    P.list_cap = u->list_cap ? u->list_cap : (agx_u32)std::min<double>(g_tiny ? (double)nh / 2 + 16 : (double)nh * per_hit * 1.1 + 4096, 4.0e9);
    P.ovf_cap = u->ovf_cap ? u->ovf_cap : (g_tiny ? 4u : 1u << 16);
    const size_t ids_cap = n_pos + P.pool_cap;
    P.sp_cap = u->sp_cap ? u->sp_cap : (agx_u32)std::min<size_t>(g_tiny ? 32 : ids_cap / 4 + 4096, 0xFFFFFF00ull);
    Take m; pool_bufs(u, P.pool_cap, m); fixed_bufs(u, m); list_bufs(u, P.list_cap, m); ovf_bufs(u, P.ovf_cap, m); sparse_bufs(u, P.sp_cap, m);
    P.exact = m.bytes;
    auto aligned = [](size_t b) { return (b + 255) & ~(size_t)255; };
    const size_t counters = (u->prm.flags & AGX_FLAG_EDGE_SUPPORT) ? aligned((size_t)P.pool_cap * AGX_MAXE * 4) + aligned((size_t)P.ovf_cap * 4) + aligned((2 * (size_t)tiles_of(u) + 2) * 4) : 0;
    const size_t plain = P.exact - counters;
    P.total = plain + regrow_slack(plain) + ((u->prm.flags & AGX_FLAG_KEEP_COUNTS) ? unitig_layout(P.pool_cap, n_pos, P.ovf_cap, nullptr, nullptr, nullptr) : 0);
    if (keeps_paths(u)) P.total += idmap_layout(n_pos + P.pool_cap, P.pool_cap, nullptr, nullptr);
    if (counters) P.total = round_block(P.total) + counters;
    return P;
}

void do_upload(agx_unit *u) {
    if (u->consumed) throw Error{E_ARG, "one-shot unit: hand its inputs over again before another upload"};
    if (!u->staged) stage_inputs(u);
    if (u->arena.used()) do_release(u);
    u->out.paths.clear(); u->out.paths_ready = false;
    const double t0 = now_ms();
    HIP_OK(hipSetDevice(u->prm.device));
    const size_t n_pos = u->V.n_pos, nh = u->nh;
    u->arena.device = u->prm.device;
    u->n_tiles = tiles_of(u); u->n_regions = regions_of(u);
    const Plan plan = plan_capacities(u);
    u->arena.reserve(plan.total);
    Take t{&u->arena};
    pool_bufs(u, plan.pool_cap, t);
    fixed_bufs(u, t); list_bufs(u, plan.list_cap, t); ovf_bufs(u, plan.ovf_cap, t); sparse_bufs(u, plan.sp_cap, t);
    if (u->arena.used() != plan.exact) throw Error{E_DEVICE, "internal: the unit's buffers take " + std::to_string(u->arena.used()) + " bytes, its layout measured " + std::to_string(plan.exact)};
    u->h_words.alloc(W_TOTAL);
    DeviceTurn &turn = turn_of(u->prm.device);
    turn.make();
    hipStream_t st = turn.up;
    trace(u, "upload: allocate", t0, n_pos);
    const double tq = now_ms();
    try {
        std::lock_guard<std::mutex> up_turn(turn.up_m);
        u->up_timed = u->ev.all;
        if (u->up_timed) HIP_OK(hipEventRecord(u->ev_up0, st));
        static const size_t chunk = getenv("AGX_UP_CHUNK_MB") ? (size_t)atoi(getenv("AGX_UP_CHUNK_MB")) << 20 : 0;
        size_t sent = 0;
        auto up = [&](void *dst, const void *src, size_t bytes) {
            for (size_t at = 0; at < bytes;) { const size_t m = chunk ? std::min(chunk, bytes - at) : bytes; HIP_OK(hipMemcpyAsync((char *)dst + at, (const char *)src + at, m, hipMemcpyHostToDevice, st)); at += m; }
            sent += bytes;
        };
        up(u->d_segs.p, u->s_segs.p, u->n_segs * sizeof(agx_cmseg)); up(u->d_cntruns.p, u->s_cntruns.p, u->n_cntruns * sizeof(agx_cntrun));
        up(u->d_cntchunks.p, u->s_cntchunks.p, u->n_cntchunks * sizeof(agx_chunk)); up(u->d_segchunks.p, u->s_segchunks.p, u->n_segchunks * sizeof(agx_chunk)); up(u->d_segindex.p, u->s_segindex.p, u->n_segindex * 4);
        up(u->d_whits.p, u->tiled ? u->s_hits_t.p : u->s_hits.p, nh * sizeof(agx_whit)); up(u->d_wsides.p, u->s_sides.p, u->n_sides * sizeof(agx_wside)); up(u->d_wruns.p, u->s_runs.p, u->n_runs * sizeof(agx_wrun)); up(u->d_jump.p, u->s_jump_at.p, u->n_jump * 4);
        if (!u->tiled) up(u->d_perm.p, u->s_perm.p, nh * 4);
        up(u->d_tfirst.p, u->s_tfirst.p, ((size_t)u->n_tiles + 2) * 4);
        HIP_OK(hipEventRecord(u->ev_hits, st));
        auto small = [&] {
            up(u->d_other.p, u->tiled ? u->s_other_t.p : u->s_other.p, others_up(u) * 8);
            if (u->ref_packed) { up(u->d_wref.p, u->s_ref.p, (n_pos + 3) / 4); up(u->d_refx.p, u->s_refx.p, u->n_refx * sizeof(agx_refx)); } else up(u->d_ref.p, u->s_ref.p, n_pos);
            up(u->d_chain_end.p, u->s_chain_end.p, (size_t)u->n_chain_end * 4);
            layout_regions(u, nullptr, u->pool_cap - spill_min(u), true, st, &sent);
        };
        auto tables = [&] { up(u->d_blockoff.p, u->s_blockoff.p, u->n_blockoff * 4); up(u->d_blockfirst.p, u->s_blockfirst.p, u->n_blockfirst * 4); up(u->d_anchor.p, u->s_anchor.p, u->n_anchor * 4); };
        if (u->tiled) {
            small();
            if (u->rows_diffed) tables();
            const size_t s4 = u->stride / 4;
            for (agx_u32 w = 0; w < u->n_win; w++) {
                const size_t r_lo = win_row(u, w), r_hi = win_row(u, w + 1);
                if (u->rows_diffed) {
                    const size_t b_lo = r_lo / 64, b_hi = (r_hi + 63) / 64, c_hi = std::min<size_t>(u->n_rowcnt, b_hi * 64);
                    up(u->d_rowcnt.p + r_lo, u->s_rowcnt.p + r_lo, c_hi - r_lo);
                    up(u->d_units.p + u->s_blockoff.p[b_lo], u->s_units.p + u->s_blockoff.p[b_lo], ((size_t)u->s_blockoff.p[b_hi] - u->s_blockoff.p[b_lo]) * 2);
                } else up(u->d_codes.p + r_lo * s4, u->s_codes_t.p + r_lo * s4, (r_hi - r_lo) * s4);
                HIP_OK(hipEventRecord(u->ev_rows[w], st));
            }
        } else {
            if (u->rows_diffed) { up(u->d_units.p, u->s_units.p, u->n_units * 2); up(u->d_rowcnt.p, u->s_rowcnt.p, u->n_rowcnt); tables(); }
            else up(u->d_codes.p, u->s_codes.p, u->n_codes);
            small();
        }
        HIP_OK(hipEventRecord(u->ev_uploaded, st));
        u->stats.upload_bytes = sent;
    } catch (...) { (void)hipStreamSynchronize(st); throw; }
    u->expanded = false;
    trace(u, "upload: queue copies", tq, n_pos);
    auto dl_buffers = [u, n_pos] {
        static std::mutex one_at_a_time;
        std::lock_guard<std::mutex> l(one_at_a_time);
        const double th0 = now_ms();
        try {
            if (hipSetDevice(u->prm.device) != hipSuccess) return;
            graph_arrays(u, helper_estimate(n_pos), [](int, auto &h, auto &, size_t n, size_t pad) { h.alloc(n + pad); });
        } catch (...) { }
        trace(u, "helper: download buffers", th0, n_pos);
    };
    if (!(u->prm.flags & AGX_FLAG_ONE_SHOT)) u->helper.submit(UnitHelper::DL, dl_buffers);
    start_helper(u);

    u->uploaded = true; u->built = false; u->downloaded = false; u->support_valid = false;
    if (!u->pending_walk) { u->pending_walk = true; g_walks_pending.fetch_add(1); }
    u->stats.ms_upload = now_ms() - t0;
    u->stats.device_bytes = u->arena.capacity();
    u->stats.rows_by_reference = u->rows_diffed ? (uint32_t)((u->tiled ? u->nh : u->n_rows) - u->n_rows_explicit) : 0u;
}

void prepare_outputs(agx_unit *u) {
    if (u->out_ready) return;
    struct Slots { std::mutex m; std::condition_variable cv; int free = 4; } static slots;
    { std::unique_lock<std::mutex> l(slots.m); slots.cv.wait(l, [] { return slots.free > 0; }); slots.free--; }
    struct Give { ~Give() { { std::lock_guard<std::mutex> l(slots.m); slots.free++; } slots.cv.notify_one(); } } give;
    try {
        const size_t n_pos = u->V.n_pos;
        u->out.pre_extended.n = 0; u->out.extended.n = 0; u->out_initial.n = 0;
        u->out.pre_extended.reserve(n_pos + n_pos / 8 + 8192); u->out.pre_extended.prefault();
        u->out.extended.reserve(n_pos + n_pos / 16 + 4096); u->out.extended.prefault();
        u->out_initial.reserve(u->V.n_initial);
        if (u->V.n_initial) u->out_initial.append(u->V.initial, u->V.n_initial);
        u->out_ready = true;
    } catch (...) { u->out_ready = false; }
}
void join_helper(agx_unit *u) { u->helper.wait(UnitHelper::OUT); }
void join_dl_helper(agx_unit *u) { u->helper.wait(UnitHelper::DL); }
void drop_outputs(agx_unit *u) { join_helper(u); u->out_ready = false; }
void start_helper(agx_unit *u) {
    join_helper(u);
    if (u->out_ready) return;
    u->helper.submit(UnitHelper::OUT, [u] { const double th0 = now_ms(); prepare_outputs(u); trace(u, "helper: output buffers", th0, u->V.n_pos); });
}

template <class F> void queue_walk_prep(agx_unit *u, hipStream_t st, F before_counters) {
    const agx_u32 n_pos = (agx_u32)u->V.n_pos;
    agx_compact_args C; memset(&C, 0, sizeof C);
    C.node_start = u->d_node_start.p; C.node_cnt = u->d_node_cnt.p; C.n_flags = u->d_flags.p; C.n_base = u->d_base.p;
    C.nk_off0 = u->d_off0.p; C.n_sref = u->d_sref.p; C.n_next = u->d_next.p; C.ref = u->d_ref.p; C.n_pos = n_pos;
    C.side_pk = u->d_side_pk.p; C.tile_side_start = u->d_tile_side_start.p; C.aid_of = u->d_aid_of.p;
    C.a_str = u->d_a_str.p; C.a_meta = u->d_a_meta.p; C.a_nid = u->d_a_nid.p; C.ovf = u->d_ovf.p; C.n_ovf = 0; C.a_ovf = u->d_a_ovf.p;
    C.abort = u->d_words.p + W_STATUS;
    C.a_mark = u->d_a_mark.p; C.side_xpos = u->d_side_xpos.p; C.sparse_min = (u->prm.flags & AGX_FLAG_SPARSE_MIN) ? 1u : 0u;
    C.sp_bits = u->d_sp_bits.p; C.sp_cnt = u->d_sp_cnt.p; C.sp_rank = u->d_sp_rank.p; C.sp_node = u->d_sp_node.p; C.sp_cap = u->sp_cap;
    C.segs = u->d_segs.p; C.n_seg0 = u->n_seg0; C.cm_start = u->d_cm_start.p; C.sp_hop = u->d_sp_hop.p; C.seg_index = u->d_segindex.p;
    if (g_scan1) agx_launch_exclusive_scan1(u->d_tile_side.p, u->d_tile_side_start.p, u->n_tiles, u->d_scan_desc.p + u->scan_desc_n, st);
    else agx_launch_exclusive_scan(u->d_tile_side.p, u->d_tile_side_start.p, u->n_tiles, u->d_scan_tmp.p, st);
    agx_launch_compact(&C, u->d_chain_end.p, u->n_chain_end, u->d_words.p + W_OVFCOUNT, u->ovf_cap, st);
    AGX_CHECKPOINT("compact");
    u->cuts = stream_cuts(n_pos); u->cuts.cut_out = u->d_words.p + W_CUT;
    agx_launch_special(&C, u->n_words, u->d_sp_rank.p, u->d_scan_tmp.p, g_scan1 ? u->d_scan_desc.p + 2 * u->scan_desc_n : nullptr,
                       u->d_words.p + W_N, u->d_tile_off.p + u->n_tiles, u->d_tile_side_start.p + u->n_tiles, u->d_pool_cnt.p, u->n_regions, u->d_words.p + W_POOL, u->cuts.n ? &u->cuts : nullptr, st);
    u->walk_args = C;
    AGX_CHECKPOINT("special");
    before_counters();
    {   void *dst = u->h_words.dev(); const void *src = u->d_words.p; const size_t bytes = W_TOTAL * 4;
        agx_launch_copy_out(&dst, &src, &bytes, 1, st); }
    HIP_OK(hipEventRecord(u->ev_built, st));
}

void do_build(agx_unit *u) {
    if (!u->uploaded) do_upload(u);
    HIP_OK(hipSetDevice(u->prm.device));
    const agx_u32 n_pos = (agx_u32)u->V.n_pos, nh = (agx_u32)u->nh;
    hipStream_t st = nullptr;
    u->stats.node_sweep_launches = u->stats.edge_sweep_launches = 0;
    u->support_valid = false; u->stats.n_support_events = 0;
    agx_u32 swept_windows = 1; bool swept_timed = false;
    for (int attempt = 0;; attempt++) {
        if (attempt > 8) throw Error{E_DEVICE, "build did not converge"};
        const size_t ids_cap = (size_t)n_pos + u->pool_cap;

        const double tb0 = now_ms();
        const bool early = !u->expanded && attempt == 0 && !u->ev.all;
        HIP_OK(wait_event(early ? u->ev_hits : u->ev_uploaded));
        trace(u, "build: wait for upload", tb0, n_pos);
        const double tb1 = now_ms();
        DeviceTurn &turn = turn_of(u->prm.device);
        std::unique_lock<std::mutex> my_turn(turn.m);
        st = turn.front;
        if (turn.n) HIP_OK(hipStreamWaitEvent(st, (u->ev.all || turn.prev_exclusive) ? turn.build_done[(turn.n - 1) & 1] : turn.sweep_done[(turn.n - 1) & 1], 0));
        if (u->ev.all) HIP_OK(hipEventRecord(u->ev.first, st));
        if (!u->expanded) {
            agx_launch_expand_runs(u->d_wruns.p, u->d_runs.p, (agx_u32)u->n_runs, st);
            agx_launch_cm_tables(u->d_cntruns.p, u->d_cntchunks.p, (agx_u32)u->n_cntchunks, u->d_segs.p, u->d_segchunks.p, (agx_u32)u->n_segchunks, u->d_cm_start.p, u->d_cm.p, u->d_cm_head.p, n_pos, (agx_u32)u->n_cm, st);
        }
        {
            agx_zero_args Z; memset(&Z, 0, sizeof Z);
            auto seg = [&](int i, agx_u32 *ptr, size_t words) { Z.p[i] = ptr; Z.n[i] = (agx_u32)words; };
            seg(0, u->d_words.p, W_TOTAL); seg(1, u->d_tile_cnt.p, (size_t)u->n_tiles + 1); seg(2, u->d_cursor.p, (size_t)u->n_tiles + 1);
            seg(3, u->d_pool_cnt.p, (size_t)u->n_regions * AGX_REGION_PAD); seg(4, u->d_tile_side.p + u->n_tiles, 1); seg(5, u->d_sp_cnt.p, (size_t)u->n_words + 1);
            seg(6, reinterpret_cast<agx_u32 *>(u->d_scan_desc.p), 6 * u->scan_desc_n); seg(7, reinterpret_cast<agx_u32 *>(u->d_sp_bits.p), 2 * ((size_t)u->n_words + 1));
            agx_launch_zero(&Z, st);
            HIP_OK(hipMemsetAsync(u->d_a_mark.p, 0, ids_cap + 2, st));
        }
        u->ev.begin(); u->ev.mark(B_START, st);
        agx_prep_args PA{(const agx_whit *)u->d_whits.p, (const agx_wside *)u->d_wsides.p, u->d_runs.p, u->d_dhit.p, nh, u->prm.k, n_pos, u->d_tile_cnt.p, u->d_words.p + W_ERR,
                         u->d_perm.p, u->d_tfirst.p, u->d_ckey.p, u->lookback, u->d_long.p, u->d_words.p + W_LONGCOUNT, u->tiled ? 1u : 0u, u->d_perm.p};
        agx_launch_hit_prep(&PA, st);
        AGX_CHECKPOINT("hit_prep");
        u->ev.mark(B_PREP, st);
        if (g_scan1) agx_launch_exclusive_scan1(u->d_tile_cnt.p, u->d_tile_off.p, u->n_tiles, u->d_scan_desc.p, st);
        else agx_launch_exclusive_scan(u->d_tile_cnt.p, u->d_tile_off.p, u->n_tiles, u->d_scan_tmp.p, st);
        agx_fill_args FA{u->d_tile_off.p, u->d_tfirst.p, u->d_perm.p, u->d_ckey.p, u->d_dhit.p, u->d_runs.p, u->d_tile_recs.p, u->d_unsorted.p, u->n_tiles, u->list_cap, u->prm.k, u->lookback,
                         u->d_long.p, u->d_words.p + W_LONGCOUNT, u->d_words.p + W_ERR, u->d_words.p + W_STATUS, u->dense ? 1u : 0u};
        agx_launch_tile_fill(&FA, st);
        if (u->dense) {
            agx_bin_args BA{u->d_dhit.p, nh, u->d_tile_off.p, u->d_cursor.p, u->d_unsorted.p, u->list_cap, u->d_words.p + W_LONGCOUNT};
            agx_launch_bin_fill(&BA, st);
            agx_launch_tile_sort(&FA, st);
        }
        AGX_CHECKPOINT("tile_sort");
        const bool windows = !u->expanded && u->tiled;
        const agx_u32 n_win = (windows && early) ? u->n_win : 1u;
        agx_u32 wt[9]; size_t wr[9];
        for (agx_u32 w = 0; w <= n_win; w++) { wt[w] = n_win == 1 ? (w ? u->n_tiles : 0u) : u->win_tile[w]; wr[w] = n_win == 1 ? (w ? (size_t)nh : 0) : win_row(u, w); }
        swept_windows = windows ? n_win : 1u; swept_timed = windows;
        if (!u->expanded) {
            if (!windows) {
                const size_t n_bases = codes_bytes(u) * 4;
                if (early) HIP_OK(hipStreamWaitEvent(st, u->ev_uploaded, 0));
                if (u->rows_diffed) agx_launch_expand_rows(u->d_whits.p, (agx_u32)nh, u->d_wsides.p, u->d_wruns.p, u->d_anchor.p, u->d_blockfirst.p, u->d_rowcnt.p, u->d_blockoff.p, u->d_units.p, u->d_wref.p, u->d_vcodes.p, u->n_rows, u->stride, u->d_other.p, u->n_other, st);
                else agx_launch_expand_codes(u->d_codes.p, u->d_vcodes.p, (n_bases + 15) / 16 * 16, u->d_other.p, u->n_other, st);
                if (u->ref_packed) agx_launch_expand_ref(u->d_wref.p, u->d_ref.p, ((size_t)n_pos + 15) / 16 * 16, u->d_refx.p, (agx_u32)u->n_refx, st);
            } else {
                if (early) HIP_OK(hipStreamWaitEvent(st, u->ev_rows[0], 0));
                if (u->ref_packed) agx_launch_expand_ref(u->d_wref.p, u->d_ref.p, ((size_t)n_pos + 15) / 16 * 16, u->d_refx.p, (agx_u32)u->n_refx, st);
            }
            u->expanded = true;
        }
        HIP_OK(hipEventRecord(u->ev_front, st));
        if (windows) {
            const size_t s4 = u->stride / 4;
            for (agx_u32 w = 0; w < n_win; w++) {
                const size_t r_lo = wr[w], r_hi = wr[w + 1];
                if (early && w) HIP_OK(hipStreamWaitEvent(st, u->ev_rows[w], 0));
                const unsigned long long *ob = u->s_other_t.p, *oe = ob + u->n_other_t;
                const size_t o_lo = (size_t)(std::lower_bound(ob, oe, (unsigned long long)r_lo * u->stride) - ob), o_hi = (size_t)(std::lower_bound(ob, oe, (unsigned long long)r_hi * u->stride) - ob);
                const size_t b_lo = r_lo * s4 * 4, b_hi = r_hi == (size_t)nh ? (codes_bytes(u) * 4 + 15) / 16 * 16 : r_hi * s4 * 4;
                if (r_hi <= r_lo) { HIP_OK(hipEventRecord(u->ev_win[w], st)); continue; }
                if (u->rows_diffed) agx_launch_expand_rows(u->d_whits.p, (agx_u32)nh, u->d_wsides.p, u->d_wruns.p, u->d_anchor.p, u->d_blockfirst.p + r_lo / 64, u->d_rowcnt.p + r_lo, u->d_blockoff.p + r_lo / 64, u->d_units.p, u->d_wref.p,
                                                           u->d_vcodes.p + b_lo, (agx_u32)(r_hi - r_lo), u->stride, nullptr, 0, st);
                else agx_launch_expand_codes(u->d_codes.p + r_lo * s4, u->d_vcodes.p + b_lo, b_hi - b_lo, nullptr, 0, st);
                agx_launch_patch_codes(u->d_other.p + o_lo, o_hi - o_lo, u->d_vcodes.p, st);
                HIP_OK(hipEventRecord(u->ev_win[w], st));
            }
        }
        st = turn.main;
        HIP_OK(hipStreamWaitEvent(st, u->ev_front, 0));
        u->ev.mark(B_BIN, st);
        agx_node_kargs K; fill_sweep_args(u, K.S);
#ifdef AGX_SWEEP_STATS
        K.S.sweep_stats = u->d_words.p + W_N + 6;
#endif
        K.pool_cnt = u->d_pool_cnt.p; K.region_off = u->d_region_off.p; K.spill_lo = u->spill_lo; K.spill_cnt = u->d_words.p + W_SPILL;
        K.mid_count = u->d_words.p + W_MIDCOUNT; K.mid_list = u->d_mid_list.p; K.mid_n = u->d_words.p + W_MIDCOUNT;
        K.big_count = u->d_words.p + W_BIGCOUNT; K.big_list = u->d_big_list.p; K.status = u->d_words.p + W_STATUS;
        K.list_cap = u->list_cap; K.big_n = u->d_words.p + W_BIGCOUNT; K.scratch = u->d_scratch.p;
        K.slow_list = u->d_slow_list.p; K.slow_count = u->d_words.p + W_SLOWCOUNT; K.fallback_queued = 1u;
        K.huge_count = u->d_words.p + W_HUGECOUNT; K.huge_n = u->d_words.p + W_HUGECOUNT; K.huge_list = u->d_huge_list.p; K.scratch_huge = u->d_scratch_huge.p; K.huge_queued = u->huge ? 1u : 0u;
        for (agx_u32 w = 0; w < n_win; w++) {
            K.tile_lo = windows ? wt[w] : 0u; K.tile_hi = windows ? wt[w + 1] : u->n_tiles;
            if (windows) { HIP_OK(hipStreamWaitEvent(st, u->ev_win[w], 0)); HIP_OK(hipEventRecord(u->ev_sw0[w], st)); }
            agx_launch_node_sweep(&K, st);
            if (windows) HIP_OK(hipEventRecord(u->ev_sw1[w], st));
        }
        AGX_CHECKPOINT("node_sweep");
        u->ev.mark(B_NODE, st); u->stats.node_sweep_launches++;
        hipEvent_t trace_from = turn.prev_node; turn.prev_node = u->ev.e[B_NODE];
        HIP_OK(hipEventRecord(turn.sweep_done[turn.n & 1], st));
        agx_launch_node_sweep_big(&K, st);
        if (u->huge) agx_launch_node_sweep_huge(&K, st);
        AGX_CHECKPOINT("node_sweep_big");
        u->ev.mark(B_BIG, st);
        agx_edge_kargs E; fill_sweep_args(u, E.S); E.ovf = u->d_ovf.p; E.ovf_count = u->d_words.p + W_OVFCOUNT; E.ovf_cap = u->ovf_cap; E.list_cap = u->list_cap;
        E.n_hits = nh; E.jump_list = u->d_jump.p; E.n_jump = (agx_u32)u->n_jump; E.abort = u->d_words.p + W_STATUS; E.big_list = u->d_big_list.p; E.big_n = u->d_words.p + W_BIGCOUNT; E.slow_list = u->d_slow_list.p; E.slow_count = u->d_words.p + W_SLOWCOUNT;
        agx_launch_edge_sweep(&E, st);
        AGX_CHECKPOINT("edge_sweep");
        const bool side_j = !u->ev.all && !g_debug_sync;
        if (side_j) {
            HIP_OK(hipEventRecord(u->ev_passA, st));
            HIP_OK(hipStreamWaitEvent(turn.front, u->ev_passA, 0));
            agx_launch_edge_jump(&E, turn.front);
            HIP_OK(hipEventRecord(u->ev_passJ, turn.front));
        } else {
            agx_launch_edge_jump(&E, st);
            AGX_CHECKPOINT("edge_jump");
        }
        u->ev.mark(B_EDGE, st);
        agx_launch_edge_slow(&E, st);
        AGX_CHECKPOINT("edge_slow");
        u->ev.mark(B_SLOW, st);
        if (side_j) HIP_OK(hipStreamWaitEvent(st, u->ev_passJ, 0));
        queue_walk_prep(u, st, [&] {
            u->ev.mark(B_COMPACT, st);
            u->stats.edge_sweep_launches++;
            if (u->ev.all) HIP_OK(hipEventRecord(u->ev.last, st));
            HIP_OK(hipEventRecord(turn.build_done[turn.n & 1], st));
        });
        turn.n++; turn.prev_exclusive = u->ev.all;
        my_turn.unlock();
        trace(u, "build: queue kernels", tb1, n_pos);
        const double tb2 = now_ms();
        HIP_OK(wait_event(u->ev_built));
        trace(u, "build: wait for kernels", tb2, n_pos);
        HIP_OK(hipGetLastError());
        if (g_trace_gap && trace_from && trace_from != u->ev.e[B_NODE]) {
            float f = 0; if (hipEventElapsedTime(&f, trace_from, u->ev.e[B_BIN]) == hipSuccess) fprintf(stderr, "[agx gap] %.3f ms between sweeps, %.3f ms sweep\n", f, u->ev.ms(B_NODE)); else (void)hipGetLastError(); }
        const agx_u32 *w = u->h_words.p;
        if (w[W_ERR] & 1u) throw Error{E_ALIGNMENT, "BOWTIE ALIGNMENT ERROR"};
        if (w[W_ERR] & 2u) throw Error{E_UNSUPPORTED, "read alignment beyond the end of the unit sequence"};
        if (w[W_ERR] & (4u | 8u)) throw Error{E_DEVICE, (w[W_ERR] & 4u) ? "internal: the staged order of the hits is not the order of their first tiles" : "internal: a tile's list does not hold what its histogram counted"};
        u->n_tile_entries = w[W_N];
        bool again = false; Take grow{&u->arena};
        if ((w[W_STATUS] & 16u) && !u->dense) { u->dense = true; HIP_OK(hipEventRecord(u->ev_uploaded, turn.down)); continue; }
        if (u->n_tile_entries > u->list_cap) { list_bufs(u, u->n_tile_entries + u->n_tile_entries / 8 + 1024, grow); again = true; }
        else {
            if ((w[W_STATUS] & 2u) && !u->huge) {
                u->huge = true; u->d_huge_list.alloc(u->arena, (size_t)u->n_tiles + 1); u->d_scratch_huge.alloc(u->arena, (size_t)AGX_HUGE_WAVES * AGX_NF * AGX_MAXV_HUGE * 64);
                HIP_OK(hipEventRecord(u->ev_uploaded, turn.down)); continue;
            }
            if (w[W_STATUS] & 2u) throw Error{E_OVERFLOW, "more than " + std::to_string(AGX_MAXV_HUGE) + " node variants at one position"};
            if (w[W_STATUS] & 1u) {
                std::vector<agx_u32> padded((size_t)u->n_regions * AGX_REGION_PAD), demand(u->n_regions);
                HIP_OK(hipMemcpyAsync(padded.data(), u->d_pool_cnt.p, padded.size() * 4, hipMemcpyDeviceToHost, turn.down)); HIP_OK(hipStreamSynchronize(turn.down));
                for (agx_u32 r = 0; r < u->n_regions; r++) demand[r] = padded[(size_t)r * AGX_REGION_PAD];
                const unsigned long long need = layout_regions(u, demand.data(), 0, false, turn.down);
                if (need >= 0xFFFFFF00ull) throw Error{E_OVERFLOW, "node table exceeds 2^32 entries"};
                if (need > u->pool_cap) pool_bufs(u, (agx_u32)need, grow);
                layout_regions(u, demand.data(), 0, true, turn.down);
                again = true;
            } else if (w[W_OVFCOUNT] > u->ovf_cap) { ovf_bufs(u, w[W_OVFCOUNT] + w[W_OVFCOUNT] / 2 + 1024, grow); again = true; }
            else if (w[W_N + 2] > u->sp_cap) { sparse_bufs(u, w[W_N + 2] + w[W_N + 2] / 8 + 1024, grow); again = true; }
        }
        if (again) { HIP_OK(hipEventRecord(u->ev_uploaded, turn.down)); continue; }
        u->n_nodes = w[W_POOL]; u->n_big = w[W_BIGCOUNT]; u->n_mid = w[W_MIDCOUNT]; u->n_ovf = w[W_OVFCOUNT]; u->n_slow = w[W_SLOWCOUNT];
        const unsigned long long ids = (unsigned long long)n_pos + w[W_N + 1];
        if (ids >= 0xFFFFFF00ull) throw Error{E_OVERFLOW, "walk graph exceeds 2^32 ids"};
        u->n_ids = (agx_u32)ids; u->n_special = w[W_N + 2];
        u->stats.build_attempts = (uint32_t)attempt + 1; u->stats.n_spilled = w[W_SPILL]; u->stats.dense_lists = w[W_LONGCOUNT] > AGX_LONG_MAX ? 2u : w[W_LONGCOUNT] ? 1u : 0u;
#ifdef AGX_SWEEP_STATS
        {   const agx_u32 *c = w + W_N + 6;
            fprintf(stderr, "[agx sweep stats] wave-entries %u (lanes with an arrival %u = %.1f per entry); leave the fast path: %u entries / %u lanes; of those not a first store: %u / %u; "
                            "variant 0 incompatible: %u / %u; several candidate keys: %u / %u; entries with a multi-run record %u\n",
                    c[0], c[3], c[0] ? (double)c[3] / c[0] : 0.0, c[4], c[5], c[6], c[7], c[8], c[9], c[10], c[11], c[12]); }
#endif
        break;
    }
    u->built = true; u->downloaded = false; u->trimmed = false; u->front_windows = swept_windows;
    u->stats.ms_build_span = u->ev.all ? u->ev.span() : 0.0;
    u->stats.ms_prep = u->ev.ms(B_PREP); u->stats.ms_bin = u->ev.ms(B_BIN); u->stats.ms_node_sweep = u->ev.ms(B_NODE);
    if (swept_windows >= 1 && swept_timed) {
        double sum = 0; for (agx_u32 w = 0; w < swept_windows; w++) { float f = 0; if (hipEventElapsedTime(&f, u->ev_sw0[w], u->ev_sw1[w]) == hipSuccess) sum += f; else (void)hipGetLastError(); }
        u->stats.ms_node_sweep = sum;
    }
    u->stats.ms_node_big = u->ev.ms(B_BIG); u->stats.ms_edge_fast = u->ev.ms(B_EDGE); u->stats.ms_edge_slow = u->ev.ms(B_SLOW); u->stats.ms_edge_sweep = u->stats.ms_edge_fast + u->stats.ms_edge_slow; u->stats.ms_compact = u->ev.ms(B_COMPACT);
    if (u->up_timed) { float f = 0; if (hipEventElapsedTime(&f, u->ev_up0, u->ev_uploaded) == hipSuccess) u->stats.ms_upload_dev = f; else (void)hipGetLastError(); }
}

void stream_wait_all(agx_unit *u);

void do_reprune(agx_unit *u, uint32_t coverage) {
    const double t0 = now_ms();
    if (!(u->prm.flags & AGX_FLAG_KEEP_COUNTS)) throw Error{E_ARG, "reprune: the unit was created without AGX_FLAG_KEEP_COUNTS (the per-node coverage stays on the device only with it)"};
    if (coverage > 0x7FFFFFFFu) throw Error{E_ARG, "reprune: coverage above 2^31 - 1 (the prune compares signed numbers)"};
    if (!u->built || u->trimmed) throw Error{E_ARG, "reprune: the unit is not built (call agx_unit_build; not after agx_unit_trim or agx_unit_release)"};
    if ((u->prm.flags & AGX_FLAG_ONE_SHOT) && (u->consumed || u->downloaded)) throw Error{E_ARG, "reprune: a one-shot unit is re-pruned before its download or finish (its landing memory is used once)"};
    HIP_OK(hipSetDevice(u->prm.device));
    stream_wait_all(u);
    join_helper(u);
    u->out.paths.clear(); u->out.paths_ready = false;
    const agx_u32 n_pos = (agx_u32)u->V.n_pos;
    DeviceTurn &turn = turn_of(u->prm.device);
    struct Failed { agx_unit *u; bool armed; ~Failed() { if (armed) u->built = false; } } failed{u, true};
    for (int attempt = 0;; attempt++) {
        if (attempt > 2) throw Error{E_DEVICE, "reprune did not converge"};
        const size_t ids_cap = (size_t)n_pos + u->pool_cap;
        {
            std::unique_lock<std::mutex> my_turn(turn.m);
            hipStream_t st = turn.main;
            agx_zero_args Z; memset(&Z, 0, sizeof Z);
            auto seg = [&](int i, agx_u32 *ptr, size_t words) { Z.p[i] = ptr; Z.n[i] = (agx_u32)words; };
            seg(0, u->d_words.p + W_N, W_TOTAL - W_N); seg(1, u->d_tile_side.p + u->n_tiles, 1); seg(2, u->d_sp_cnt.p, (size_t)u->n_words + 1);
            seg(3, reinterpret_cast<agx_u32 *>(u->d_scan_desc.p + u->scan_desc_n), 4 * u->scan_desc_n); seg(4, reinterpret_cast<agx_u32 *>(u->d_sp_bits.p), 2 * ((size_t)u->n_words + 1));
            agx_launch_zero(&Z, st);
            HIP_OK(hipMemsetAsync(u->d_a_mark.p, 0, ids_cap + 2, st));
            agx_reprune_args R; memset(&R, 0, sizeof R);
            R.node_start = u->d_node_start.p; R.node_cnt = u->d_node_cnt.p; R.nk_cid = u->d_cid.p; R.n_counts = u->d_counts.p; R.n_flags = u->d_flags.p;
            R.side_pk = u->d_side_pk.p; R.tile_side = u->d_tile_side.p; R.n_pos = n_pos; R.pool_cap = u->pool_cap; R.coverage = (int)coverage; R.abort = u->d_words.p + W_STATUS;
            agx_launch_reprune(&R, u->n_tiles, st);
            AGX_CHECKPOINT("reprune");
            queue_walk_prep(u, st, [] {});
        }
        HIP_OK(wait_event(u->ev_built));
        HIP_OK(hipGetLastError());
        const agx_u32 *w = u->h_words.p;
        if (w[W_STATUS]) throw Error{E_DEVICE, "internal: reprune of a unit whose build left a status word"};
        u->stats.reprune_attempts = (uint32_t)attempt + 1;
        if (w[W_N + 2] > u->sp_cap) { Take grow{&u->arena}; sparse_bufs(u, w[W_N + 2] + w[W_N + 2] / 8 + 1024, grow); u->stats.device_bytes = u->arena.capacity(); continue; }
        const unsigned long long ids = (unsigned long long)n_pos + w[W_N + 1];
        if (ids >= 0xFFFFFF00ull) throw Error{E_OVERFLOW, "walk graph exceeds 2^32 ids"};
        u->n_ids = (agx_u32)ids; u->n_special = w[W_N + 2];
        break;
    }
    failed.armed = false;
    u->prm.coverage = coverage; u->downloaded = false;
    u->stats.ms_reprune = now_ms() - t0;
    trace(u, "reprune", t0, n_pos);
}

void download_buffers(agx_unit *u) {
    const GraphCounts c = graph_counts(u);
    join_dl_helper(u);
    if (u->prm.flags & AGX_FLAG_ONE_SHOT) {
        struct Room { char *at; size_t left; } room[LANDING_ROOMS]; int rooms = 0;
        landing_rooms(u, [&](auto &b, bool) { room[rooms++] = Room{(char *)b.p, b.block_bytes()}; });
        u->consumed = true; u->staged = false;
        size_t want[GA_N]; char *at[GA_N] = {};
        graph_arrays(u, c, [&](int which, auto &h, auto &, size_t n, size_t pad) { h.release(); want[which] = ((n + pad) * sizeof(*h.p) + 255) & ~(size_t)255; });
        for (const int which : GRAPH_CUT_ORDER) for (Room &r : room) if (r.at && r.left >= want[which]) { at[which] = r.at; r.at += want[which]; r.left -= want[which]; break; }
        graph_arrays(u, c, [&](int which, auto &h, auto &, size_t n, size_t pad) { if (at[which]) h.borrow((decltype(h.p))at[which], n + pad); });
    }
    graph_arrays(u, c, [](int, auto &h, auto &, size_t n, size_t pad) { h.alloc(n + pad); });
}

void do_download(agx_unit *u) {
    if (!u->built) do_build(u);
    HIP_OK(hipSetDevice(u->prm.device));
    const double t0 = now_ms();
    const GraphCounts c = graph_counts(u); const size_t n_pos = c.n_pos, ni = c.n_ids, ns = c.n_special;
    DeviceTurn &turn = turn_of(u->prm.device);
    download_buffers(u);
    u->dl_streaming = false;
    {
        void *dst[GA_N]; const void *src[GA_N]; size_t bytes[GA_N]; int n = 0;
        graph_arrays(u, c, [&](int, auto &h, auto &d, size_t count, size_t) { if (ni && count) { dst[n] = h.p; src[n] = d.p; bytes[n] = count * sizeof(*h.p); n++; } });
        bool by_engines = u->dl_sdma && n > 0;
        if (by_engines) {
            hsa_signal_store_relaxed(u->dl_signal, n);
            int queued = 0;
            for (; queued < n; queued++) if (hsa_amd_memory_async_copy(dst[queued], hsa_copy().cpu, src[queued], u->dl_agent, bytes[queued], 0, nullptr, u->dl_signal) != HSA_STATUS_SUCCESS) break;
            if (queued < n) hsa_signal_subtract_relaxed(u->dl_signal, n - queued);
            hsa_signal_value_t v;
            do v = hsa_signal_wait_scacquire(u->dl_signal, HSA_SIGNAL_CONDITION_LT, 1, UINT64_MAX, HSA_WAIT_STATE_BLOCKED); while (v >= 1);
            if (queued < n || v < 0) { u->dl_sdma = false; by_engines = false; }
        }
        if (!by_engines) {
            std::lock_guard<std::mutex> l(turn.down_m);
            for (int i = 0; i < n; i++) HIP_OK(hipMemcpyAsync(dst[i], src[i], bytes[i], hipMemcpyDeviceToHost, turn.down));
            HIP_OK(hipEventRecord(u->ev_dl, turn.down));
        }
    }
    const double t1 = now_ms();
    HIP_OK(wait_event(u->ev_dl));
    if (getenv("AGX_DL_TIMING")) fprintf(stderr, "[agx download] buffers %.2f ms, copies %.2f ms (%zu ids, %zu records)\n", t1 - t0, now_ms() - t1, ni, ns);
    memset(u->h_a_meta.p + ni, 0, 64);
    u->stats.n_walk_ids = ni; u->stats.n_special = ns;
    u->stats.download_bytes = graph_bytes(u, c);
    u->downloaded = true;
    u->stats.ms_download = now_ms() - t0;
    trace(u, u->dl_sdma ? "download (copy engines)" : "download (hipMemcpyAsync)", t0, n_pos);
}

// ... 195 lines not shown
            HIP_OK(hipMemcpy(out + (size_t)s * (m + G), d_out[s].p, (m + G) * 4, hipMemcpyDeviceToHost));
            if (form == 1) HIP_OK(hipMemcpy(desc + (size_t)s * (nb + G), d_desc[s].p, (nb + G) * 8, hipMemcpyDeviceToHost));
            else HIP_OK(hipMemcpy(tmp + (size_t)s * (tw + G), d_tmp[s].p, (tw + G) * 4, hipMemcpyDeviceToHost));
        }
    } catch (const Error &) { rc = AGX_E_DEVICE; }
      catch (const std::bad_alloc &) { rc = AGX_E_ARG; }
    for (hipStream_t s : st) if (s) (void)hipStreamDestroy(s);
    return rc;
}

int agx_test_zero(int device, const uint32_t *len, uint32_t *words) {
    if (!len || !words) return AGX_E_ARG;
    try {
        HIP_OK(hipSetDevice(device));
        const size_t G = AGX_TEST_GUARD;
        DBuf<agx_u32> d[8];
        DevArena arena; arena.device = device;
        agx_zero_args Z; memset(&Z, 0, sizeof Z);
        for (int s = 0; s < 8; s++) {
            d[s].alloc(arena, (size_t)len[s] + 2 * G); HIP_OK(hipMemset(d[s].p, 0xA5, ((size_t)len[s] + 2 * G) * 4));
            Z.p[s] = d[s].p + G; Z.n[s] = len[s];
        }
        HIP_OK(hipDeviceSynchronize());
        agx_launch_zero(&Z, nullptr);
        HIP_OK(hipGetLastError());
        HIP_OK(hipDeviceSynchronize());
        size_t at = 0;
        for (int s = 0; s < 8; s++) { HIP_OK(hipMemcpy(words + at, d[s].p, ((size_t)len[s] + 2 * G) * 4, hipMemcpyDeviceToHost)); at += (size_t)len[s] + 2 * G; }
        return AGX_OK;
    } catch (const Error &) { return AGX_E_DEVICE; }
      catch (const std::bad_alloc &) { return AGX_E_ARG; }
}

int agx_test_copy_out(int device, int n_seg, const uint64_t *bytes, const uint8_t *src, uint8_t *dst) {
    if (n_seg < 1 || n_seg > 16 || !bytes || !src || !dst) return AGX_E_ARG;
    try {
        HIP_OK(hipSetDevice(device));
        const size_t G = AGX_TEST_GUARD * 4;
        DBuf<agx_u8> d_src[16]; PBuf<agx_u8> h_dst;
        DevArena arena; arena.device = device;
        size_t total = 0, at = 0, from = 0;
        for (int s = 0; s < n_seg; s++) total += ((size_t)bytes[s] + 15) / 16 * 16 + G;
        h_dst.alloc(total); memset(h_dst.p, 0xA5, total);
        void *dp[16]; const void *sp[16]; size_t nbytes[16];
        for (int s = 0; s < n_seg; s++) {
            const size_t r = ((size_t)bytes[s] + 15) / 16 * 16;
            d_src[s].alloc(arena, r);
            if (r) HIP_OK(hipMemcpy(d_src[s].p, src + from, r, hipMemcpyHostToDevice));
            dp[s] = (char *)h_dst.dev() + at; sp[s] = d_src[s].p; nbytes[s] = (size_t)bytes[s];
            at += r + G; from += r;
        }
        HIP_OK(hipDeviceSynchronize());
        agx_launch_copy_out(dp, sp, nbytes, n_seg, nullptr);
        HIP_OK(hipGetLastError());
        HIP_OK(hipDeviceSynchronize());
        memcpy(dst, h_dst.p, total);
        return AGX_OK;
    } catch (const Error &) { return AGX_E_DEVICE; }
      catch (const std::bad_alloc &) { return AGX_E_ARG; }
}

int agx_device_memory(int device, uint64_t *free_bytes, uint64_t *total_bytes) {
    size_t f = 0, t = 0;
    if (hipSetDevice(device) != hipSuccess || hipMemGetInfo(&f, &t) != hipSuccess) return AGX_E_DEVICE;
    if (free_bytes) *free_bytes = f;
    if (total_bytes) *total_bytes = t;
    return AGX_OK;
}

int agx_unit_create(const agx_params *p, agx_unit **out) {
    if (!p || !out) return AGX_E_ARG;
    *out = nullptr;
    if (p->k == 0 || p->k >= 32768) return AGX_E_ARG;
    int n = 0;
    if (hipGetDeviceCount(&n) != hipSuccess || n <= 0) return AGX_E_NOGPU;
    if (p->device < 0 || p->device >= n) return AGX_E_ARG;
    agx_unit *u = new (std::nothrow) agx_unit();
    if (!u) return AGX_E_ARG;
    u->prm = *p; if (u->prm.batch == 0) u->prm.batch = 1000000;
    const int rc = guarded(u, [&] {
        try { u->helper.start(); } catch (...) { }
        HIP_OK(hipSetDevice(p->device));
        u->ev.init(); u->ev.all = (u->prm.flags & AGX_FLAG_TIME_SECTIONS) != 0;
        for (hipEvent_t *e : {&u->ev_front, &u->ev_passA, &u->ev_passJ}) HIP_OK(hipEventCreateWithFlags(e, hipEventDisableTiming));
        for (hipEvent_t *e : {&u->ev_dl, &u->ev_built, &u->ev_hits}) HIP_OK(hipEventCreateWithFlags(e, hipEventDisableTiming));
        HIP_OK(hipEventCreate(&u->ev_up0)); HIP_OK(hipEventCreate(&u->ev_uploaded));
        for (int i = 0; i < 8; i++) { HIP_OK(hipEventCreateWithFlags(&u->ev_rows[i], hipEventDisableTiming)); HIP_OK(hipEventCreateWithFlags(&u->ev_win[i], hipEventDisableTiming)); HIP_OK(hipEventCreate(&u->ev_sw0[i])); HIP_OK(hipEventCreate(&u->ev_sw1[i])); }
        u->dl_sdma = hsa_copy().agent_of(p->device, u->dl_agent) && hsa_signal_create(0, 0, nullptr, &u->dl_signal) == HSA_STATUS_SUCCESS;
    });
    if (rc != AGX_OK) { delete u; return rc; }
    g_units_alive.fetch_add(1);
    *out = u;
    return AGX_OK;
}

void agx_unit_destroy(agx_unit *u) { if (u) { (void)hipSetDevice(u->prm.device); do_release(u); delete u; if (g_units_alive.fetch_sub(1) == 1) out_cache_trim(); } }

const char *agx_unit_error(const agx_unit *u) { return u ? u->err.c_str() : "null unit"; }

int agx_unit_set_reference(agx_unit *u, const char *bases, uint32_t n) {
    if (!u || (!bases && n)) return AGX_E_ARG;
    return guarded(u, [&] { drop_outputs(u); u->T = Threads(); u->T.ref.assign(bases, n); u->T.n_ref = n; u->have_ref = true; u->have_threads = false; u->staged = false; u->uploaded = false; u->built = false; });
}

int agx_unit_set_contig_threads(agx_unit *u, const char *appended, uint32_t n_appended, const uint32_t *cm_start, const agx_contimer *cm, uint32_t n_cm,
                                const char *initial_contigs, size_t initial_len) {
    if (!u || !cm_start || (!cm && n_cm) || (!appended && n_appended)) return AGX_E_ARG;
    return guarded(u, [&] {
        if (!u->have_ref) throw Error{E_ARG, "set the reference first"};
        drop_outputs(u);
        u->T.ref.resize(u->T.n_ref); u->T.ref.append(appended ? appended : "", n_appended);
        const size_t n_pos = u->T.ref.size();
        u->T.cm_start.assign(cm_start, cm_start + n_pos + 1);
        if (u->T.cm_start[n_pos] != n_cm) throw Error{E_ARG, "cm_start does not end at n_cm"};
        u->T.cm.resize(n_cm);
        for (uint32_t i = 0; i < n_cm; i++) {
            if (cm[i].next_off != AGX_NONE && cm[i].next_off >= n_pos) throw Error{E_ARG, "conti-mer link beyond the position array"};
            u->T.cm[i] = ContiMer{cm[i].nuc, cm[i].cid, cm[i].coff, cm[i].next_off, cm[i].next_item};
        }
        u->T.initial_contigs.assign(initial_contigs ? initial_contigs : "", initial_len);
        build_chains(u->T);
        u->have_threads = true; u->staged = false; u->uploaded = false; u->built = false;
    });
}

int agx_unit_push_pairs(agx_unit *u, const agx_pair_batch *b) {
    if (!u || !b) return AGX_E_ARG;
    return guarded(u, [&] {
        drop_outputs(u);
        if (u->pairs_staged) { u->pairs_staged = false; u->row_off.clear(); u->reads_keep.reset(); u->P = Pairs(); }
        if (u->P.hits.empty()) { u->P = Pairs(); u->P.stride = b->stride; }
        if (b->stride != u->P.stride) throw Error{E_ARG, "all batches of a unit must use one read stride"};
        const agx_u32 slot0 = u->P.n_slots, run0 = (agx_u32)u->P.runs.size();
        for (uint64_t i = 0; i < b->n_hits; i++) {
            agx_hit h = b->hits[i];
            if (h.len == 0 || h.len > b->stride || (uint64_t)h.slot1 + 1 >= b->n_slots) throw Error{E_ARG, "hit names a read slot outside the batch"};
            if ((h.nruns1 && (uint64_t)h.runs1 + h.nruns1 > b->n_runs) || (h.nruns2 && (uint64_t)h.runs2 + h.nruns2 > b->n_runs)) throw Error{E_ARG, "hit names runs outside the batch"};
            if (h.back > i) throw Error{E_ARG, "hit.back reaches before the batch"};
            h.slot1 += slot0; if (h.nruns1) h.runs1 += run0; if (h.nruns2) h.runs2 += run0;
            u->P.hits.push_back(h);
        }
        u->P.runs.insert(u->P.runs.end(), b->runs, b->runs + b->n_runs);
        u->P.bases.append(b->bases, (size_t)b->n_slots * b->stride);
        u->P.n_slots += b->n_slots;
        u->staged = false; u->uploaded = false; u->built = false;
    });
}

struct agx_reads { std::shared_ptr<agx::ReadsIndex> idx; };

int agx_reads_open(const char *reads_fa, agx_reads **out, char *err, size_t err_len) {
    if (!reads_fa || !out) return AGX_E_ARG;
    *out = nullptr;
    try { std::unique_ptr<agx_reads> r(new agx_reads); r->idx.reset(reads_index_open(reads_fa), reads_index_close); *out = r.release(); return AGX_OK; }
    catch (const Error &e) { if (err && err_len) snprintf(err, err_len, "%s", e.msg.c_str()); return e.code ? e.code : AGX_E_ARG; }
    catch (const std::exception &e) { if (err && err_len) snprintf(err, err_len, "%s", e.what()); return AGX_E_ARG; }
}

void agx_reads_close(agx_reads *reads) { delete reads; }

int agx_unit_load_files(agx_unit *u, const char *tmp_dir, int unit) { return agx_unit_load_files_shared(u, tmp_dir, unit, nullptr); }

int agx_unit_load_files_shared(agx_unit *u, const char *tmp_dir, int unit, const agx_reads *reads) {
    if (!u || !tmp_dir) return AGX_E_ARG;
    return guarded(u, [&] {
        const std::string d = tmp_dir, s = std::to_string(unit);
        u->stats.from_cache = 0;
        if (load_cache(u, d, unit)) return;
        const double t0 = now_ms();
        const bool fast = getenv("AGX_NO_FAST_LOAD") == nullptr;
// ... 187 lines not shown

void agx_graph_free(agx_graph *g) {
    if (!g) return;
    free(g->node_start); free(g->node_key); free(g->node_cnt); free(g->node_slen); free(g->edge_start); free(g->edge_dst); memset(g, 0, sizeof *g);
}

int agx_unit_walk_graph(agx_unit *u, int streamed, agx_walk_graph *g) {
    if (!u || !g) return AGX_E_ARG;
    const bool want_all = g->want_all_node != 0;
    memset(g, 0, sizeof *g);
    const int rc = guarded(u, [&] {
        static_assert(sizeof(agx_walk_rec) == sizeof(agx_walknode) && sizeof(agx_walk_hop) == sizeof(agx_hop), "include/agx.h mirrors the walk graph's records");
        if (u->prm.flags & AGX_FLAG_ONE_SHOT) throw Error{E_ARG, "walk graph: a one-shot unit's download lands in its staged inputs and cannot be repeated for the walk"};
        if (streamed) {
            if (!begin_streamed_download(u)) throw Error{E_ARG, "walk graph: this unit's download cannot be streamed (no window cuts, or no copy engines)"};
            stream_wait_all(u);
        } else do_download(u);
        const GraphView G = view_of(u);
        const size_t ni = G.n_ids; size_t nb[GA_N];
        graph_arrays(u, graph_counts(u), [&](int which, auto &h, auto &, size_t n, size_t) { nb[which] = n * sizeof(*h.p); });
        auto dup = [](const void *p, size_t bytes) { void *q = malloc(bytes + 1); if (!q) throw Error{E_ARG, "out of host memory"}; if (bytes) memcpy(q, p, bytes); return q; };
        g->n_pos = G.n_pos; g->n_ids = G.n_ids; g->n_special = G.n_special; g->n_ovf = (uint32_t)G.n_ovf; g->n_chain_str = u->n_chain_str;
        g->meta = (uint8_t *)dup(G.meta, nb[GA_META]); g->str = (char *)dup(G.str, nb[GA_STR]); g->side_xpos = (uint32_t *)dup(G.side_xpos, nb[GA_XPOS]);
        g->sp_bits = (uint64_t *)dup(G.sp_bits, nb[GA_BITS]); g->sp_rank = (uint32_t *)dup(G.sp_rank, nb[GA_RANK]);
        g->sp_node = (agx_walk_rec *)dup(G.sp_node, nb[GA_NODE]); g->sp_hop = (agx_walk_hop *)dup(G.sp_hop, nb[GA_HOP]);
        g->ovf = (uint32_t *)dup(G.ovf, nb[GA_OVF]); g->chain_str = (char *)dup(u->V.chain_str, u->n_chain_str);
        if (want_all) {
            g->all_node = (agx_walk_rec *)malloc((ni + 1) * sizeof(agx_walknode));
            if (!g->all_node) throw Error{E_ARG, "out of host memory"};
            const agx_u32 rows = (agx_u32)(ni / 64);
            if (rows) G.fetch(G.fetch_ctx, 0, 64, rows, 64, (agx_walknode *)g->all_node);
            if (ni % 64) G.fetch(G.fetch_ctx, rows * 64u, 0, 1, (agx_u32)(ni % 64), (agx_walknode *)g->all_node + (size_t)rows * 64);
        }
        if (streamed) u->downloaded = false;
    });
    if (rc != AGX_OK) agx_walk_graph_free(g);
    return rc;
}

void agx_walk_graph_free(agx_walk_graph *g) {
    if (!g) return;
    free(g->meta); free(g->str); free(g->side_xpos); free(g->sp_bits); free(g->sp_rank); free(g->sp_node); free(g->sp_hop); free(g->ovf); free(g->chain_str); free(g->all_node);
    memset(g, 0, sizeof *g);
}

int agx_unit_front(agx_unit *u, agx_front *f) {
    if (!u || !f) return AGX_E_ARG;
    memset(f, 0, sizeof *f);
    const int rc = guarded(u, [&] {
        static_assert(sizeof(agx_dhit) == 40 && sizeof(agx_cmkey) == 8 && sizeof(agx_cmhead) == 16 && sizeof(agx_run) == 12, "include/agx.h describes the front's records as words");
        if (u->prm.flags & AGX_FLAG_ONE_SHOT) throw Error{E_ARG, "front: a one-shot unit gives its arrays away with its only download"};
        if (!u->built || u->trimmed || u->downloaded) throw Error{E_ARG, "front: the unit is not built (call agx_unit_build; not after agx_unit_download, agx_unit_trim or agx_unit_release)"};
        HIP_OK(hipSetDevice(u->prm.device));
        HIP_OK(wait_event(u->ev_built));
        const size_t n_pos = u->V.n_pos, nh = u->nh, nt = u->n_tiles, vbytes = codes_bytes(u) * 4;
        const agx_u32 *w = u->h_words.p;
        f->n_pos = (uint32_t)n_pos; f->n_hits = (uint32_t)nh; f->n_runs = (uint32_t)u->n_runs; f->n_cm = (uint32_t)u->n_cm; f->n_tiles = (uint32_t)nt; f->stride = u->stride;
        f->n_rows = u->stride ? (uint32_t)(vbytes / u->stride) : 0u; f->lookback = u->lookback;
        f->long_count = w[W_LONGCOUNT]; f->n_long = std::min<agx_u32>(w[W_LONGCOUNT], AGX_LONG_MAX); f->w_err = w[W_ERR]; f->w_status = w[W_STATUS];
        f->tiled = u->tiled; f->rows_diffed = u->rows_diffed; f->ref_packed = u->ref_packed; f->dense_queued = u->dense; f->swept_windows = u->front_windows;
        DeviceTurn &turn = turn_of(u->prm.device);
        std::lock_guard<std::mutex> l(turn.down_m);
        auto down = [&](auto *&dst, const void *src, size_t bytes) {
            dst = (std::remove_reference_t<decltype(dst)>)malloc(bytes + 16);
            if (!dst) throw Error{E_ARG, "out of host memory"};
            if (bytes) HIP_OK(hipMemcpyAsync(dst, src, bytes, hipMemcpyDeviceToHost, turn.down));
        };
        try {
            down(f->tile_off, u->d_tile_off.p, (nt + 1) * 4);
            HIP_OK(hipStreamSynchronize(turn.down));
            f->n_entries = f->tile_off[nt];
            if (f->n_entries > u->list_cap) throw Error{E_DEVICE, "internal: the tile lists of a converged build do not fit their buffer"};
            down(f->ref, u->d_ref.p, n_pos); down(f->vcodes, u->d_vcodes.p, (size_t)f->n_rows * u->stride); down(f->runs, u->d_runs.p, u->n_runs * sizeof(agx_run));
            down(f->cm_start, u->d_cm_start.p, (n_pos + 1) * 4); down(f->cm, u->d_cm.p, u->n_cm * sizeof(agx_cmkey)); down(f->cm_head, u->d_cm_head.p, (n_pos + 1) * sizeof(agx_cmhead));
            down(f->dhit, u->d_dhit.p, nh * sizeof(agx_dhit)); down(f->perm, u->d_perm.p, nh * 4); down(f->tile_first, u->d_tfirst.p, (nt + 1) * 4); down(f->ckey, u->d_ckey.p, nh * 4);
            down(f->tile_cnt, u->d_tile_cnt.p, (nt + 1) * 4); down(f->tile_recs, u->d_tile_recs.p, (size_t)f->n_entries * 32); down(f->long_list, u->d_long.p, (size_t)f->n_long * 4);
            HIP_OK(hipStreamSynchronize(turn.down));
        } catch (...) { (void)hipStreamSynchronize(turn.down); throw; }
    });
    if (rc != AGX_OK) agx_front_free(f);
    return rc;
}

void agx_front_free(agx_front *f) {
    if (!f) return;
    free(f->ref); free(f->vcodes); free(f->runs); free(f->cm_start); free(f->cm); free(f->cm_head); free(f->dhit); free(f->perm); free(f->tile_first); free(f->ckey);
    free(f->tile_cnt); free(f->tile_off); free(f->tile_recs); free(f->long_list);
    memset(f, 0, sizeof *f);
}


static void export_check(const agx_unit *u, bool map) {
    if (!(u->prm.flags & AGX_FLAG_KEEP_COUNTS)) throw Error{E_ARG, "unitigs: the unit was created without AGX_FLAG_KEEP_COUNTS (the segments' coverage needs the counts)"};
    if (!u->built || u->trimmed) throw Error{E_ARG, "unitigs: the unit is not built (call agx_unit_build; not after agx_unit_trim or agx_unit_release)"};
    if ((u->prm.flags & AGX_FLAG_ONE_SHOT) && (u->consumed || u->downloaded)) throw Error{E_ARG, "unitigs: a one-shot unit exports before its download or finish"};
    if (map && !(u->prm.flags & AGX_FLAG_KEEP_PATHS)) throw Error{E_ARG, "unitigs: the unit was created without AGX_FLAG_KEEP_PATHS (the id map's scratch is reserved with the unit's block)"};
}

struct Export {
    agx_unit *u; const agx_u32 n_pos, cap, n_ovf; hipStream_t s = nullptr; size_t map_at = 0;
    explicit Export(agx_unit *unit) : u(unit), n_pos((agx_u32)unit->V.n_pos), cap(unit->pool_cap), n_ovf(std::min(unit->n_ovf, unit->ovf_cap)) {
        HIP_OK(hipSetDevice(u->prm.device));
        HIP_OK(wait_event(u->ev_built));
    }
    Export(const Export &) = delete;
    ~Export() { if (s) { (void)hipStreamSynchronize(s); (void)hipStreamDestroy(s); } }
    void open(size_t own) {
        u->d_ut.alloc(u->arena, keeps_paths(u) ? mapped_scratch(cap, n_pos, u->n_nodes, u->n_ids, n_ovf, &map_at) : own);
        u->stats.device_bytes = u->arena.capacity();
        open_stream();
    }
    void open_stream() { HIP_OK(hipStreamCreateWithFlags(&s, hipStreamNonBlocking)); }
    void fill(void *p, int v, size_t b) const { HIP_OK(hipMemsetAsync(p, v, b ? b : 1, s)); }
    void read(void *host, const void *dev, size_t b) const { HIP_OK(hipMemcpyAsync(host, dev, b, hipMemcpyDeviceToHost, s)); }
    void sync() const { HIP_OK(hipStreamSynchronize(s)); }
};

struct MapJob { agx_idmap *m; agx_idmap_args M{}; agx_u32 n_wids = 0; };
struct SupportJob { uint32_t **out; };

static void support_check(const agx_unit *u) {
    if (!(u->prm.flags & AGX_FLAG_EDGE_SUPPORT)) throw Error{E_ARG, "edge support: the unit was created without AGX_FLAG_EDGE_SUPPORT (the counters are reserved with the unit's block)"};
    if (u->prm.flags & AGX_FLAG_ONE_SHOT) throw Error{E_ARG, "edge support: a one-shot unit gives the arrays the counting reads away with its only download"};
    if (!u->built || u->trimmed || u->downloaded) throw Error{E_ARG, "edge support: the unit is not built (call agx_unit_build; not after agx_unit_download, agx_unit_trim or agx_unit_release)"};
}

static void ensure_support(const Export &E) {
    agx_unit *u = E.u;
    const double t0 = now_ms();
    if (!u->support_valid) {
        const size_t nt = u->n_tiles;
        agx_support_kargs K; fill_sweep_args(u, K.S);
        K.ovf = u->d_ovf.p; K.n_ovf = E.n_ovf; K.n_hits = (agx_u32)u->nh; K.list_cap = u->list_cap;
        K.e_cnt = u->d_e_cnt.p; K.ovf_cnt = u->d_ovf_cnt.p; K.tile_events = u->d_sup_tot.p; K.tile_adds = u->d_sup_tot.p + nt; K.unmatched = u->d_sup_tot.p + 2 * nt;
        K.abort = u->d_words.p + W_STATUS;
        E.fill(K.e_cnt, 0, (size_t)u->pool_cap * AGX_MAXE * 4); E.fill(K.ovf_cnt, 0, (size_t)u->ovf_cap * 4); E.fill(u->d_sup_tot.p, 0, (2 * nt + 2) * 4);
        agx_launch_edge_support(&K, E.s);
        std::vector<agx_u32> tot(2 * nt + 1);
        E.read(tot.data(), u->d_sup_tot.p, tot.size() * 4); E.sync();
        HIP_OK(hipGetLastError());
        if (tot[2 * nt]) throw Error{E_DEVICE, "internal: edge support: " + std::to_string(tot[2 * nt]) + " contributions found no edge of the built graph"};
        uint64_t ev = 0, ad = 0;
        for (size_t t = 0; t < nt; t++) { ev += tot[t]; ad += tot[nt + t]; }
        u->sup_events = ev; u->sup_adds = ad; u->support_valid = true;
        u->stats.n_support_events = ev;
    }
    u->stats.ms_edge_support = now_ms() - t0;
}

static void export_body(const Export &E, agx_unitig_args &A, const agx_unitig_region_args *R, agx_u32 *words, agx_u32 np, agx_u32 max_nodes, agx_unitigs *t, MapJob *J, SupportJob *S = nullptr) {
    A.piece_cap = np;
    agx_u32 rounds = 1; while (rounds < 32 && (1ull << (rounds - 1)) < np) rounds++;
    E.fill(A.p_seg, 0xFF, (size_t)np * 4);
    if (!R) E.fill(A.hcnt, 0, ((size_t)A.n_pos + 1) * 4);
    E.fill(A.s_len, 0, ((size_t)np + 1) * 4); E.fill(A.s_links, 0, ((size_t)np + 1) * 4); E.fill(A.s_cov, 0, (size_t)np * 8);
    agx_launch_unitig_phase2(&A, R, rounds, E.s);
    E.fill(A.l_cur, 0, ((size_t)np + 1) * 4);
    agx_launch_unitig_totals(&A, words + 4, E.s);
    agx_u32 h[4] = {0, 0, 0, 0}, nr = 0;
    if (J) {
        agx_launch_idmap_flags(R, &J->M, E.s);
        E.read(&nr, J->M.foff + J->n_wids, 4);
    }
    E.read(h, words + 4, 16); E.sync();
    if (h[3]) throw Error{E_DEVICE, "unitigs: the unitig ranks are inconsistent (error word " + std::to_string(h[3]) + ")"};
    const agx_u32 ns = h[0], nb = h[1], nl = h[2];
// ... 425 lines not shown
```

### aligngraph_amd/csrc/agx_kargs.h

```cpp
#pragma once
#include <hip/hip_runtime_api.h>
#include "agx_core.h"

struct agx_prep_args {
    const agx_whit *whits; const agx_wside *sides;
    const agx_run *runs; agx_dhit *dhit; agx_u32 n_hits, k, n_pos;
    agx_u32 *tile_cnt;
    agx_u32 *err;
    const agx_u32 *perm, *tile_first; agx_u32 *ckey; agx_u32 lookback; agx_u32 *long_list, *long_count;
    agx_u32 tiled; agx_u32 *perm_out;
};

struct agx_bin_args { const agx_dhit *dhit; agx_u32 n_hits; const agx_u32 *tile_off; agx_u32 *cursor; agx_u32 *unsorted; agx_u32 cap;
                      const agx_u32 *long_count; };

struct agx_node_kargs {
    agx_sweep_args S;
    agx_u32 tile_lo, tile_hi;
    agx_u32 *pool_cnt;
    const agx_u32 *region_off;
    agx_u32 spill_lo; agx_u32 *spill_cnt;
    agx_u32 *mid_count; agx_u32 *mid_list;
    agx_u32 *big_count; agx_u32 *big_list;
    agx_u32 fallback_queued;
    agx_u32 *status;
    agx_u32 list_cap;
    const agx_u32 *big_n;
    const agx_u32 *mid_n;
    agx_u32 *scratch;
    agx_u32 *huge_count; agx_u32 *huge_list; const agx_u32 *huge_n; agx_u32 *scratch_huge; agx_u32 huge_queued;
    agx_u32 *slow_list; agx_u32 *slow_count;
};

struct agx_edge_kargs {
    agx_sweep_args S; agx_edge_ovf *ovf; agx_u32 *ovf_count; agx_u32 ovf_cap; agx_u32 list_cap;
    agx_u32 *slow_list; agx_u32 *slow_count;
    agx_u32 n_hits; const agx_u32 *jump_list; agx_u32 n_jump;
    const agx_u32 *abort;
    const agx_u32 *big_list; const agx_u32 *big_n;
};
struct agx_support_kargs {
    agx_sweep_args S; const agx_edge_ovf *ovf; agx_u32 n_ovf, n_hits, list_cap;
    agx_u32 *e_cnt, *ovf_cnt;
    agx_u32 *tile_events, *tile_adds;
    agx_u32 *unmatched;
    const agx_u32 *abort;
};
struct agx_unitig_args {
    const agx_u32 *node_start; const agx_u16 *node_cnt; const agx_u8 *n_flags; const agx_u8 *n_base; const agx_u32 *n_next; const int *n_counts; const char *ref;
    const agx_edge_ovf *ovf; agx_u32 n_ovf; agx_u32 n_pos, pool_cap;
    agx_u32 *err;
    agx_u32 *pos_of;
    agx_u32 *indeg;
    agx_u32 *outs;
    agx_u32 *succ;
    agx_u32 *oout, *osucc;
    agx_u32 *nxt;
    agx_u8 *haspred;
    unsigned long long *ovf_hash; agx_u32 hash_mask; agx_u8 *ovf_first;
    agx_u32 piece_cap;
    agx_u32 *wcnt, *woff;
    agx_u32 *p_len, *p_next;
    agx_u32 *anc[2], *off[2];
    agx_u32 *p_seg;
    agx_u32 *hcnt, *hoff;
    agx_u32 *s_len, *s_links, *s_hpos, *s_hvar, *s_last; unsigned long long *s_cov;
    agx_u32 *s_off, *l_off, *l_cur;
    char *seq; agx_u32 seq_cap;
    agx_u32 *l_to; agx_u32 link_cap;
    agx_u32 *scan_tmp;
};

struct agx_unitig_region_args {
    agx_unitig_args U;
    const agx_u32 *nk_cid; const agx_u16 *node_cnt; agx_u32 pos_lo, n_win, min_cov, pool_cap;
    agx_u32 *cntw, *offw;
    agx_u32 *l_slot;
    agx_u32 *rmap;
};

struct agx_idmap_args {
    const agx_u32 *a_nid, *side_xpos; agx_u32 n_pos, n_ids;
    agx_u32 n_main, side_lo, n_side;
    agx_u32 *bounds;
    agx_u32 *flag, *foff;
    agx_u32 *scan_tmp;
    agx_u32 *r_first, *r_last, *r_seg, *r_rank; agx_u32 run_cap;
};

struct agx_evidence_args {
    agx_evidence_tab T;
    agx_u32 lo, n, min_depth, min_support, n_recs;
    unsigned long long *r_steps, *r_dsum;
// ... 66 lines not shown
```

### aligngraph_amd/csrc/agx_kernels.hip

```cpp
#include <hip/hip_runtime.h>
#include "agx_kargs.h"

#define AGX_WAVES_PER_BLOCK 4
static_assert(AGX_MAXV_LDS <= AGX_EM_W && AGX_MAXV_MID <= AGX_EM_W, "the LDS sweep writes the x -> x+1 edges of every position it finishes: its buckets must fit the edge matrix");
#define AGX_XCDS 8u
#ifndef AGX_SWEEP_WAVES
#define AGX_SWEEP_WAVES 1
#endif

#define AGX_RETURN_IF_ABORTED(word) do { if (__builtin_amdgcn_readfirstlane((int)*(word)) != 0) return; } while (0)

__global__ void __launch_bounds__(256) agx_k_cm_layout(const agx_cntrun *runs, const agx_chunk *chunks, agx_u32 *cm_start, agx_cmhead *head, agx_u32 n_pos, agx_u32 n_cm) {
    const agx_chunk c = chunks[blockIdx.x];
    const agx_cntrun r = runs[c.run];
    const agx_u32 n = r.len - c.off < AGX_CM_CHUNK ? r.len - c.off : AGX_CM_CHUNK;
    for (agx_u32 j = threadIdx.x; j < n; j += 256u) agx_cm_layout_pos(r, c.off + j, cm_start, head);
    if (blockIdx.x == 0 && threadIdx.x == 0) { cm_start[n_pos] = n_cm; head[n_pos] = agx_cmhead{AGX_NONE, AGX_NONE, 0u, 0u}; }
}
__global__ void __launch_bounds__(256) agx_k_cm_fill(const agx_cmseg *segs, const agx_chunk *chunks, const agx_u32 *cm_start, agx_cmkey *cm, agx_cmhead *head) {
    const agx_chunk c = chunks[blockIdx.x];
    const agx_cmseg g = segs[c.run];
    const agx_u32 n = g.len - c.off < AGX_CM_CHUNK ? g.len - c.off : AGX_CM_CHUNK;
    for (agx_u32 j = threadIdx.x; j < n; j += 256u) agx_cm_fill_elem(g, c.off + j, cm_start, cm, head);
}
// ... 2 lines not shown
    for (int s = 0; s < 8; s++) { if (i < Z.n[s]) { Z.p[s][i] = 0u; return; } i -= Z.n[s]; }
}
struct agx_collect_args { agx_u32 *out; const agx_u32 *a, *b, *c, *pool_cnt; agx_u32 regions; agx_u32 *sum;
                          agx_cut_args cuts; const agx_u32 *sp_rank, *tile_side_start; const unsigned long long *sp_bits; agx_u32 n_pos; };
__device__ __forceinline__ void agx_collect_block(const agx_collect_args &G) {
    __shared__ agx_u32 part[256];
    if (G.cuts.n && threadIdx.x <= G.cuts.n) {
        const agx_u32 t = threadIdx.x; const bool last = t == G.cuts.n;
        const agx_u32 w = last ? G.n_pos >> 6 : G.cuts.word[t];
        agx_u32 r = G.sp_rank[w];
        if (last && (G.n_pos & 63u)) r += (agx_u32)__popcll(G.sp_bits[w] & ((1ull << (G.n_pos & 63u)) - 1ull));
        G.cuts.cut_out[t] = r;
        G.cuts.cut_out[AGX_DL_PIECES + 1u + t] = G.tile_side_start[last ? (G.n_pos + AGX_TILE - 1u) / AGX_TILE : w];
    }
    agx_u32 t = 0;
    for (agx_u32 r = threadIdx.x; r < G.regions; r += 256u) t += G.pool_cnt[(size_t)r * AGX_REGION_PAD];
    part[threadIdx.x] = t; __syncthreads();
    for (agx_u32 o = 128; o; o >>= 1) { if (threadIdx.x < o) part[threadIdx.x] += part[threadIdx.x + o]; __syncthreads(); }
    if (threadIdx.x == 0) { G.out[0] = *G.a; G.out[1] = *G.b; G.out[2] = *G.c; *G.sum = part[0]; }
}
__global__ void __launch_bounds__(256) agx_k_expand_codes(const agx_u32 *packed, uint4 *vcodes, size_t n16) {
    const size_t i = (size_t)blockIdx.x * 256u + threadIdx.x;
    if (i >= n16) return;
    const agx_u32 v = packed[i];
    agx_u32 w[4];
    for (int j = 0; j < 4; j++) {
        agx_u32 o = 0;
        for (int b = 0; b < 4; b++) o |= (agx_u32)agx_class_vote_code((v >> (8 * j + 2 * b)) & 3u) << (8 * b);
        w[j] = o;
    }
    vcodes[i] = make_uint4(w[0], w[1], w[2], w[3]);
}
__global__ void __launch_bounds__(256) agx_k_patch_codes(const unsigned long long *other, size_t n, agx_u8 *vcodes) {
    const size_t i = (size_t)blockIdx.x * 256u + threadIdx.x;
    if (i < n) vcodes[other[i]] = agx_class_vote_code(4u);
}

__global__ void __launch_bounds__(64) agx_k_expand_rows(const agx_whit *hits, agx_u32 nh, const agx_wside *sides, const agx_wrun *runs, const agx_u32 *anchor_bits, const agx_u32 *block_first,
                                                         const agx_u8 *cnt, const agx_u32 *block_off, const agx_u16 *units, const agx_u32 *wref, agx_u8 *vcodes, agx_u32 n_rows, agx_u32 stride) {
    extern __shared__ __attribute__((aligned(16))) agx_u32 row_lds[];
    const agx_u32 b = blockIdx.x, l = threadIdx.x, row = b * 64u + l;
    const bool valid = row < n_rows;
    const agx_u32 c = cnt[row];
    const agx_u32 u = valid ? agx_row_units(c, stride) : 0u;
    agx_u32 incl = u;
    for (agx_u32 o = 1; o < 64u; o <<= 1) { const agx_u32 t = __shfl_up(incl, o, 64); if (l >= o) incl += t; }
    if (valid) {
        const agx_u32 h = agx_anchor_select(anchor_bits, block_first[b], l);
        if (h < nh) {
            const agx_whit w = hits[h];
            const agx_wrun *left = nullptr; agx_u32 nruns = 0;
            if (c != AGX_ROW_EXPLICIT && !agx_whit_left_simple(w)) { const agx_wside sd = sides[agx_whit_side(w)]; left = runs + agx_wside_left_first(w, sd); nruns = agx_wside_left_count(w, sd); }
            agx_row_decode(wref, units + (size_t)block_off[b] + (incl - u), c, w, left, nruns, stride, (agx_u8 *)row_lds + (size_t)l * stride);
        }
    }
    __syncthreads();
    const agx_u32 rows_here = n_rows - b * 64u < 64u ? n_rows - b * 64u : 64u, words = rows_here * (stride / 4u);
    agx_u32 *dst = (agx_u32 *)(vcodes + (size_t)b * 64u * stride);
    for (agx_u32 i = l; i < words / 4u; i += 64u) ((uint4 *)dst)[i] = ((const uint4 *)row_lds)[i];
    for (agx_u32 i = (words & ~3u) + l; i < words; i += 64u) dst[i] = row_lds[i];
}

__global__ void __launch_bounds__(256) agx_k_expand_runs(const agx_wrun *wruns, agx_run *runs, agx_u32 n_runs) {
    const agx_u32 i = blockIdx.x * 256u + threadIdx.x;
    if (i < n_runs) { const agx_wrun r = wruns[i]; runs[i] = agx_run{r.q, r.t, r.n}; }
}
__global__ void __launch_bounds__(256) agx_k_expand_ref(const agx_u32 *packed, uint4 *ref, size_t n16) {
    const size_t i = (size_t)blockIdx.x * 256u + threadIdx.x;
    if (i >= n16) return;
    const agx_u32 v = packed[i];
    agx_u32 w[4];
    for (int j = 0; j < 4; j++) { agx_u32 o = 0; for (int b = 0; b < 4; b++) o |= (agx_u32)(agx_u8)agx_ref_base((v >> (8 * j + 2 * b)) & 3u) << (8 * b); w[j] = o; }
    ref[i] = make_uint4(w[0], w[1], w[2], w[3]);
}
__global__ void __launch_bounds__(256) agx_k_patch_ref(const agx_refx *x, agx_u8 *ref) {
    const agx_refx r = x[blockIdx.x];
    for (agx_u32 j = threadIdx.x; j < r.len; j += 256u) ref[(size_t)r.pos + j] = (agx_u8)r.byte;
}

__global__ void __launch_bounds__(256) agx_k_hit_prep(agx_prep_args A) {
    const agx_u32 i = blockIdx.x * 256u + threadIdx.x, lane = threadIdx.x & 63u;
    const bool mine = i < A.n_hits;
    agx_dhit d; d.flags = AGX_HF_SKIP; d.x_lo = 1; d.x_hi = 0; d.a_nruns = 0;
    if (mine) {
        const agx_whit *wh = A.whits; const agx_wside *sd = A.sides;
        const agx_u32 h = A.tiled ? i : A.perm[i];
        const agx_whit w = wh[h];
        const agx_hit H = agx_unpack_hit(w, sd);
        bool dup; agx_u32 row;
        if (A.tiled) { dup = (w.flags & AGX_WF_DUP) != 0; row = i; A.perm_out[i] = w.row; }
        else { dup = H.back != 0 && agx_hit_dup_by([wh, sd](agx_u32 j) { return agx_unpack_hit(wh[j], sd); }, A.runs, h); row = H.slot1; }
        const int rc = agx_hit_prep(H, dup, (H.pad[0] & 1u) != 0, row, A.runs, A.k, d);
        if (rc) atomicOr(A.err, 1u);
        if (!(d.flags & AGX_HF_SKIP) && (d.x_hi >= A.n_pos || d.x_lo > d.x_hi)) { atomicOr(A.err, 2u); d.flags |= AGX_HF_SKIP; }
    }
    const bool kept = mine && !(d.flags & AGX_HF_SKIP);
    const agx_u32 t0 = kept ? d.x_lo / AGX_TILE : 0u, t1 = kept ? d.x_hi / AGX_TILE : 0u;
    if (kept && !(A.tile_first[t0] <= i && i < A.tile_first[t0 + 1])) atomicOr(A.err, 4u);
    const bool lng = kept && t1 - t0 >= A.lookback;
    if (mine) A.ckey[i] = (kept && !lng) ? t1 : AGX_NONE;
    if (lng) { const agx_u32 at = atomicAdd(A.long_count, 1u); if (at < AGX_LONG_MAX) A.long_list[at] = i; }
    const unsigned long long below = (1ull << lane) - 1ull;
    for (agx_u32 s = 0; s < 4; s++) {
        const agx_u32 t = t0 + s;
        const bool pend = kept && t <= t1;
        const agx_u32 tp = (agx_u32)__shfl_up((int)t, 1, 64);
        const unsigned long long starts = __ballot(lane == 0 || t != tp), pm = __ballot(pend);
        const agx_u32 first = 63u - (agx_u32)__builtin_clzll(starts & (below | (1ull << lane)));
        const unsigned long long after = starts & ~(below | (1ull << lane));
        const agx_u32 end = after ? (agx_u32)__builtin_ctzll(after) : 64u;
        const unsigned long long run = (end == 64u ? ~0ull : ((1ull << end) - 1ull)) & ~((1ull << first) - 1ull);
        const unsigned long long p = pm & run;
        if (pend && lane == (agx_u32)__builtin_ctzll(p)) (void)atomicAdd(&A.tile_cnt[t], (agx_u32)__popcll(p));
    }
    if (kept && t1 - t0 >= 4) for (agx_u32 t = t0 + 4; t <= t1; t++) (void)atomicAdd(&A.tile_cnt[t], 1u);
    if (mine) A.dhit[i] = d;
}

#define AGX_SCAN_ITEMS 16
#define AGX_SCAN_BLOCK (256u * AGX_SCAN_ITEMS)
__global__ void __launch_bounds__(256) agx_k_scan_blocks(const agx_u32 *in, agx_u32 *out, agx_u32 *block_sums, agx_u32 n) {
    __shared__ agx_u32 sh[256];
    const agx_u32 base = blockIdx.x * AGX_SCAN_BLOCK + threadIdx.x * AGX_SCAN_ITEMS;
    agx_u32 v[AGX_SCAN_ITEMS], s = 0;
    for (int i = 0; i < AGX_SCAN_ITEMS; i++) { v[i] = (base + i < n) ? in[base + i] : 0u; s += v[i]; }
    sh[threadIdx.x] = s;
    __syncthreads();
    for (agx_u32 off = 1; off < 256; off <<= 1) {
        agx_u32 t = threadIdx.x >= off ? sh[threadIdx.x - off] : 0u;
        __syncthreads();
        sh[threadIdx.x] += t;
        __syncthreads();
    }
    agx_u32 run = sh[threadIdx.x] - s;
    for (int i = 0; i < AGX_SCAN_ITEMS; i++) { if (base + i < n) out[base + i] = run; run += v[i]; }
    if (threadIdx.x == 255 && block_sums) block_sums[blockIdx.x] = sh[255];
}
__global__ void __launch_bounds__(256) agx_k_scan_add(agx_u32 *out, const agx_u32 *block_offsets, agx_u32 n) {
    const agx_u32 i = blockIdx.x * 256u + threadIdx.x;
    if (i < n) out[i] += block_offsets[i / AGX_SCAN_BLOCK];
}

#define AGX_SCAN_GRID 1024u
__global__ void __launch_bounds__(256) agx_k_scan_lookback(const agx_u32 *in, agx_u32 *out, agx_u32 n, unsigned long long *desc, agx_u32 n_blocks) {
    __shared__ agx_u32 sh[256];
    __shared__ agx_u32 sh_excl;
    for (agx_u32 b = blockIdx.x; b < n_blocks; b += gridDim.x) {
        const agx_u32 base = b * AGX_SCAN_BLOCK + threadIdx.x * AGX_SCAN_ITEMS;
        agx_u32 v[AGX_SCAN_ITEMS], s = 0;
        for (int i = 0; i < AGX_SCAN_ITEMS; i++) { v[i] = (base + i < n) ? in[base + i] : 0u; s += v[i]; }
        __syncthreads();
        sh[threadIdx.x] = s;
        __syncthreads();
        for (agx_u32 off = 1; off < 256; off <<= 1) {
            agx_u32 t = threadIdx.x >= off ? sh[threadIdx.x - off] : 0u;
            __syncthreads();
            sh[threadIdx.x] += t;
            __syncthreads();
        }
        const agx_u32 total = sh[255];
        if (threadIdx.x < 64) {
            const agx_u32 lane = threadIdx.x;
            if (lane == 0) __hip_atomic_store(&desc[b], (b == 0 ? AGX_SCAN_PFX : AGX_SCAN_AGG) | total, __ATOMIC_RELAXED, __HIP_MEMORY_SCOPE_AGENT);
            agx_u32 excl = 0;
            for (long long hi = (long long)b - 1; hi >= 0;) {
                const long long j = hi - lane;
                unsigned long long d = AGX_SCAN_FRONT;
// ... 897 lines not shown
```

### include/agx.h

```cpp
#ifndef AGX_H
#define AGX_H

#include <stddef.h>
#include <stdint.h>

#ifdef __cplusplus
extern "C" {
#endif

#define AGX_OK 0
#define AGX_E_IO (-1)
#define AGX_E_FORMAT (-2)
#define AGX_E_UNSUPPORTED (-3)
#define AGX_E_ALIGNMENT (-4)
#define AGX_E_DEVICE (-5)
#define AGX_E_ARG (-6)
#define AGX_E_OVERFLOW (-7)
#define AGX_E_NOGPU (-8)

typedef struct agx_unit agx_unit;

typedef struct {
    uint32_t k;
    uint32_t insert_variation;
// ... 121 lines not shown
    uint64_t *sp_bits;
    uint32_t *sp_rank;
    agx_walk_rec *sp_node;
    agx_walk_hop *sp_hop;
    uint32_t *ovf;
    char *chain_str;
    agx_walk_rec *all_node;
} agx_walk_graph;

typedef struct {
    uint32_t n_pos, n_hits, n_runs, n_cm, n_tiles, stride, n_rows;
    uint32_t lookback;
    uint32_t n_entries;
    uint32_t long_count, n_long;
    uint32_t w_err, w_status;
    uint32_t tiled, rows_diffed, ref_packed, dense_queued, swept_windows;
    char *ref;
    uint8_t *vcodes;
    agx_run *runs;
    uint32_t *cm_start;
    uint32_t *cm;
    uint32_t *cm_head;
    uint32_t *dhit;
    uint32_t *perm;
    uint32_t *tile_first;
    uint32_t *ckey;
    uint32_t *tile_cnt;
    uint32_t *tile_off;
    uint32_t *tile_recs;
    uint32_t *long_list;
} agx_front;


const char *agx_version(void);
int agx_device_count(void);
int agx_device_memory(int device, uint64_t *free_bytes, uint64_t *total_bytes);
int agx_selftest_scan(int device, uint32_t n, uint32_t seed);

#define AGX_TEST_GUARD 64
int agx_test_scan(int device, int form, const uint32_t *in, uint32_t n, uint32_t *out , uint32_t grid_cap, int seeded, int streams,
                  uint64_t *desc, uint32_t *tmp, uint32_t *grid_limit);
int agx_test_zero(int device, const uint32_t *len, uint32_t *words);
int agx_test_copy_out(int device, int n_seg, const uint64_t *bytes, const uint8_t *src, uint8_t *dst);

int agx_unit_create(const agx_params *p, agx_unit **out);
void agx_unit_destroy(agx_unit *u);
const char *agx_unit_error(const agx_unit *u);

int agx_unit_set_reference(agx_unit *u, const char *bases, uint32_t n);
int agx_unit_set_contig_threads(agx_unit *u, const char *appended, uint32_t n_appended,
                                const uint32_t *cm_start, const agx_contimer *cm, uint32_t n_cm,
                                const char *initial_contigs, size_t initial_len);
int agx_unit_push_pairs(agx_unit *u, const agx_pair_batch *b);

int agx_unit_load_files(agx_unit *u, const char *tmp_dir, int unit);

typedef struct agx_reads agx_reads;
int agx_reads_open(const char *reads_fa, agx_reads **out, char *err, size_t err_len);
void agx_reads_close(agx_reads *reads);
int agx_unit_load_files_shared(agx_unit *u, const char *tmp_dir, int unit, const agx_reads *reads);

int agx_unit_cache_build(const agx_params *p, const char *tmp_dir, int unit, const agx_reads *reads, char *err, size_t err_len);
int agx_unit_cache_save(agx_unit *u, const char *tmp_dir, int unit);

int agx_unit_stage(agx_unit *u);
int agx_unit_hbm_needed(agx_unit *u, uint64_t *bytes);
int agx_unit_upload(agx_unit *u);
int agx_unit_build(agx_unit *u);
int agx_unit_reprune(agx_unit *u, uint32_t coverage);
int agx_unit_download(agx_unit *u);
int agx_unit_finish(agx_unit *u, agx_result *r);
void agx_result_free(agx_result *r);
int agx_unit_trim(agx_unit *u, uint64_t *freed);
int agx_unit_release(agx_unit *u);
void agx_pool_trim(int device);

int agx_unit_stats(const agx_unit *u, agx_stats *s);
int agx_unit_graph(agx_unit *u, agx_graph *g);
void agx_graph_free(agx_graph *g);
int agx_unit_walk_graph(agx_unit *u, int streamed, agx_walk_graph *g);
void agx_walk_graph_free(agx_walk_graph *g);
int agx_unit_front(agx_unit *u, agx_front *f);
void agx_front_free(agx_front *f);
int agx_unit_unitigs(agx_unit *u, agx_unitigs *t);
int agx_unit_unitigs_region(agx_unit *u, uint32_t pos_lo, uint32_t pos_hi, uint32_t min_coverage, agx_unitigs *t);
int agx_unit_unitigs_mapped(agx_unit *u, uint32_t pos_lo, uint32_t pos_hi, uint32_t min_coverage, agx_unitigs *t, agx_idmap *m);
void agx_idmap_free(agx_idmap *m);
int agx_unit_edge_support(agx_unit *u, agx_edge_support *s);
void agx_edge_support_free(agx_edge_support *s);
int agx_unit_unitigs_support(agx_unit *u, uint32_t pos_lo, uint32_t pos_hi, uint32_t min_coverage, agx_unitigs *t, uint32_t **link_support, agx_idmap *m);
void agx_link_support_free(uint32_t *link_support);
int agx_unit_walk_paths(agx_unit *u, agx_walk_paths *w);
void agx_walk_paths_free(agx_walk_paths *w);
int agx_unit_walk_evidence(agx_unit *u, const agx_walk_paths *w, uint32_t min_depth, uint32_t min_support,
                           uint32_t want_tracks, uint32_t rec_lo, uint32_t rec_hi, agx_walk_evidence *e);
void agx_walk_evidence_free(agx_walk_evidence *e);
int agx_walk_evidence_bed(const agx_walk_evidence *e, int unit, char **text, size_t *len);
void agx_unitigs_free(agx_unitigs *t);
int agx_unitigs_gfa(const agx_unitigs *t, int unit, char **text, size_t *len);
int agx_unitigs_gfa_support(const agx_unitigs *t, const uint32_t *link_support, int unit, char **text, size_t *len);
int agx_unitigs_paths_gfa(const agx_unitigs *t, const agx_idmap *m, const agx_walk_paths *w, int unit, char **text, size_t *len);
void agx_text_free(char *text);

int agx_run_unit(const agx_params *p, const char *tmp_dir, int unit, int write_files, agx_result *r, char *err, size_t err_len);
int agx_run_unit_shared(const agx_params *p, const char *tmp_dir, int unit, int write_files, const agx_reads *reads, agx_result *r, char *err, size_t err_len);

#ifdef __cplusplus
}
#endif
#endif
```

Baseline: 1.347 billion.

## Upload hits in a compact delta-coded form and restructure build streams

Adds a compact hit record (position plus 16-bit delta, common length) with full records spilled to a side array and per-group rank bases, chosen when most hits share one length. The front kernel decodes these using a wave ballot to find each hit's full-record rank. This shrinks host-to-device hit upload bytes. The change also drops the separate front stream and edge-jump side stream, folds window expansion inline into the sweep loop, and alternates two build streams across units, gated on the previous unit's sweep event. It adds a diagnostic API reporting the chosen hit form.

```diff
diff --git a/aligngraph_amd/__init__.py b/aligngraph_amd/__init__.py
--- a/aligngraph_amd/__init__.py
+++ b/aligngraph_amd/__init__.py
@@ -19,7 +19,7 @@
     "agx_reads_open", "agx_reads_close", "agx_unit_load_files_shared", "agx_run_unit_shared",
     "agx_unit_stage", "agx_unit_release", "agx_pool_trim", "agx_unit_cache_build", "agx_unit_cache_save", "agx_unit_hbm_needed",
     "agx_unit_trim", "agx_unit_unitigs", "agx_unit_unitigs_region", "agx_unitigs_free", "agx_unitigs_gfa", "agx_text_free",
-    "agx_unit_walk_graph", "agx_walk_graph_free", "agx_unit_front", "agx_front_free",
+    "agx_unit_walk_graph", "agx_walk_graph_free", "agx_unit_front", "agx_front_free", "agx_unit_hit_form",
     "agx_unit_unitigs_mapped", "agx_idmap_free", "agx_unit_walk_paths", "agx_walk_paths_free", "agx_unitigs_paths_gfa", "agx_unit_reprune",
     "agx_unit_edge_support", "agx_edge_support_free", "agx_unit_unitigs_support", "agx_link_support_free", "agx_unitigs_gfa_support",
     "agx_unit_walk_evidence", "agx_walk_evidence_free", "agx_walk_evidence_bed",
@@ -455,6 +455,13 @@
         finally:
             lib().agx_front_free(ctypes.byref(f))
 
+    def hit_form(self):
+        f = lib().agx_unit_hit_form
+        f.argtypes = [ctypes.c_void_p, ctypes.POINTER(ctypes.c_uint64)]
+        out = (ctypes.c_uint64 * 6)()
+        self._check(f(self._h, out))
+        return {"form": ("file", "tiled", "compact")[out[0]], "hits": out[1], "full": out[2], "sides": out[3], "common_len": out[4], "others": out[5]}
+
     def _window(self, region, min_coverage):
         lo, hi = region if region is not None else (0, self.stats()["n_pos"])
         cov = self.params.coverage if min_coverage is None else min_coverage
diff --git a/aligngraph_amd/csrc/agx_core.h b/aligngraph_amd/csrc/agx_core.h
--- a/aligngraph_amd/csrc/agx_core.h
+++ b/aligngraph_amd/csrc/agx_core.h
@@ -56,6 +56,42 @@
         if (w.flags & AGX_WF_RUNS2) { h.runs2 = sd.runs2; h.nruns2 = (agx_u16)(sd.nruns >> 16); }
     }
     return h;
+}
+#define AGX_CGROUP 64u
+enum { AGX_CF_FULL = 64 };
+struct agx_chit { agx_u32 p, number; int16_t d; agx_u8 flags, back; };
+struct agx_cbase { agx_u32 full; };
+AGX_HD agx_u32 agx_chit_side_guess(agx_u32 number, agx_u32 n_sides, agx_u32 n_hits) { return n_hits ? (agx_u32)((unsigned long long)number * n_sides / n_hits) : 0u; }
+AGX_HD bool agx_chit_pack(const agx_whit &w, agx_u32 common_len, agx_u32 n_sides, agx_u32 n_hits, agx_chit &c) {
+    const agx_u32 f = w.flags & (agx_u32)(AGX_WF_RUNS1 | AGX_WF_RUNS2);
+    c.number = w.row; c.back = w.back; c.p = 0; c.d = 0;
+    long long diff;
+    if (!f) { c.p = w.a; diff = (long long)w.b - (long long)w.a; }
+    else {
+        c.p = f == (agx_u32)AGX_WF_RUNS1 ? w.b : f == (agx_u32)AGX_WF_RUNS2 ? w.a : 0u;
+        diff = (long long)((f & AGX_WF_RUNS1) ? w.a : w.b) - (long long)agx_chit_side_guess(w.row, n_sides, n_hits);
+    }
+    const bool full = w.len != common_len || diff < -32768 || diff > 32767;
+    if (!full) c.d = (int16_t)diff;
+    c.flags = (agx_u8)((w.flags & 63u) | (full ? (agx_u32)AGX_CF_FULL : 0u));
+    return full;
+}
+AGX_HD agx_hit agx_chit_unpack(const agx_chit &c, agx_u32 common_len, agx_u32 n_sides, agx_u32 n_hits, const agx_whit *full, agx_u32 full_rank, const agx_wside *sides) {
+    const agx_u32 f = c.flags & (agx_u32)(AGX_WF_RUNS1 | AGX_WF_RUNS2);
+    agx_whit w; w.row = c.number; w.flags = (agx_u8)(c.flags & 63u); w.back = c.back;
+    if (c.flags & AGX_CF_FULL) { const agx_whit x = full[full_rank]; w.a = x.a; w.b = x.b; w.len = x.len; }
+    else {
+        w.len = (agx_u16)common_len;
+        w.a = (f == (agx_u32)AGX_WF_RUNS2 || !f) ? c.p : 0u;
+        w.b = !f ? c.p + (agx_u32)(int)c.d : f == (agx_u32)AGX_WF_RUNS1 ? c.p : 0u;
+        if (f) { const agx_u32 at = agx_chit_side_guess(c.number, n_sides, n_hits) + (agx_u32)(int)c.d; if (f & AGX_WF_RUNS1) w.a = at; else w.b = at; }
+    }
+    return agx_unpack_hit(w, sides);
+}
+inline agx_u32 agx_chit_rank(const agx_chit *recs, const agx_cbase *base, size_t i) {
+    const size_t g = i / AGX_CGROUP; agx_u32 r = base[g].full;
+    for (size_t j = g * AGX_CGROUP; j < i; j++) r += (recs[j].flags & AGX_CF_FULL) ? 1u : 0u;
+    return r;
 }
 struct agx_refx { agx_u32 pos, len, byte; };
 AGX_HD agx_u32 agx_ref_code(agx_u32 c) { return c == 'A' ? 0u : c == 'C' ? 1u : c == 'G' ? 2u : c == 'T' ? 3u : 4u; }
diff --git a/aligngraph_amd/csrc/agx_engine.cpp b/aligngraph_amd/csrc/agx_engine.cpp
--- a/aligngraph_amd/csrc/agx_engine.cpp
+++ b/aligngraph_amd/csrc/agx_engine.cpp
@@ -208,10 +208,11 @@
     PBuf<agx_whit> s_hits; PBuf<agx_wside> s_sides; PBuf<agx_wrun> s_runs; PBuf<agx_u8> s_codes; PBuf<unsigned long long> s_other; PBuf<agx_u32> s_jump; size_t n_other = 0, n_sides = 0, n_jump = 0;
     PBuf<agx_u8> s_ref; PBuf<agx_refx> s_refx; size_t n_refx = 0; bool ref_packed = false;
     PBuf<agx_u32> s_chain_end, s_region_off; PBuf<agx_cmseg> s_segs; size_t n_segs = 0;
+    PBuf<agx_chit> s_chits; PBuf<agx_whit> s_full_t; PBuf<agx_cbase> s_cbase; size_t n_full = 0; bool compact = false; agx_u32 common_len = 0;
     PBuf<agx_whit> s_hits_t; PBuf<agx_u8> s_codes_t; PBuf<unsigned long long> s_other_t; size_t n_other_t = 0; bool tiled = false; std::vector<agx_u32> slot_row;
     agx_u32 front_windows = 1;
     agx_u32 n_win = 1, win_tile[9] = {};
-    hipEvent_t ev_rows[8] = {}, ev_win[8] = {}, ev_sw0[8] = {}, ev_sw1[8] = {};
+    hipEvent_t ev_rows[8] = {}, ev_sw0[8] = {}, ev_sw1[8] = {};
     PBuf<agx_u32> s_perm, s_tfirst, s_jump_at; agx_u32 lookback = 2;
     PBuf<char> s_landing;
     PBuf<agx_cntrun> s_cntruns; PBuf<agx_chunk> s_cntchunks, s_segchunks; PBuf<agx_u32> s_segindex; size_t n_cntruns = 0, n_cntchunks = 0, n_segchunks = 0, n_segindex = 0;
@@ -227,6 +228,7 @@
     DBuf<agx_run> d_runs; DBuf<agx_u8> d_codes, d_vcodes; DBuf<unsigned long long> d_other;
     DBuf<agx_u16> d_units; DBuf<agx_u8> d_rowcnt; DBuf<agx_u32> d_blockoff, d_blockfirst, d_anchor;
     DBuf<agx_cntrun> d_cntruns; DBuf<agx_chunk> d_cntchunks, d_segchunks; DBuf<agx_u32> d_jump, d_segindex;
+    DBuf<agx_chit> d_chits; DBuf<agx_whit> d_wfull; DBuf<agx_cbase> d_cbase;
     DBuf<agx_whit> d_whits; DBuf<agx_wside> d_wsides; DBuf<agx_wrun> d_wruns; DBuf<agx_u8> d_wref; DBuf<agx_refx> d_refx;
     DBuf<agx_dhit> d_dhit; DBuf<agx_u32> d_tile_cnt, d_tile_off, d_cursor, d_unsorted, d_tile_recs, d_scan_tmp, d_words; DBuf<unsigned long long> d_scan_desc; size_t scan_desc_n = 0;
     agx_u32 pool_cap = 0, spill_lo = 0, ovf_cap = 0, list_cap = 0, sp_cap = 0;
@@ -247,15 +249,15 @@
     PBuf<agx_walknode> h_sp_node, h_fetch; PBuf<agx_edge_ovf> h_a_ovf; PBuf<agx_hop> h_sp_hop; DBuf<agx_hop> d_sp_hop;
     PBuf<agx_u32> h_words;
     agx_u32 n_nodes = 0, n_ovf = 0, n_tiles = 0, n_tile_entries = 0, n_big = 0, n_mid = 0, n_slow = 0;
-    Boundaries ev; hipEvent_t ev_front = nullptr, ev_passA = nullptr, ev_passJ = nullptr, ev_up0 = nullptr, ev_uploaded = nullptr, ev_dl = nullptr, ev_hits = nullptr;
+    Boundaries ev; hipEvent_t ev_up0 = nullptr, ev_uploaded = nullptr, ev_dl = nullptr, ev_hits = nullptr;
     bool up_timed = false;
     agx_stats stats{};
     ~agx_unit() {
         arena.reset();
         if (pending_walk) g_walks_pending.fetch_sub(1);
         ev.destroy();
-        for (hipEvent_t e : {ev_front, ev_passA, ev_passJ, ev_up0, ev_uploaded, ev_dl, ev_built, ev_hits}) if (e) (void)hipEventDestroy(e);
-        for (auto *arr : {ev_rows, ev_win, ev_sw0, ev_sw1}) for (int i = 0; i < 8; i++) if (arr[i]) (void)hipEventDestroy(arr[i]);
+        for (hipEvent_t e : {ev_up0, ev_uploaded, ev_dl, ev_built, ev_hits}) if (e) (void)hipEventDestroy(e);
+        for (auto *arr : {ev_rows, ev_sw0, ev_sw1}) for (int i = 0; i < 8; i++) if (arr[i]) (void)hipEventDestroy(arr[i]);
         if (dl_signal.handle) (void)hsa_signal_destroy(dl_signal);
         if (dl_piece_made) for (hsa_signal_t g : dl_piece) if (g.handle) (void)hsa_signal_destroy(g);
     }
@@ -263,18 +265,18 @@
 
 namespace {
 
-struct DeviceTurn { std::mutex m; hipStream_t main = nullptr, front = nullptr, up = nullptr, down = nullptr;
+struct DeviceTurn { std::mutex m; hipStream_t build[2] = {nullptr, nullptr}, up = nullptr, down = nullptr;
                     hipEvent_t sweep_done[2] = {nullptr, nullptr}, build_done[2] = {nullptr, nullptr};
                     unsigned long long n = 0; bool prev_exclusive = false; hipEvent_t prev_node = nullptr;
                     std::mutex up_m, down_m, make_m;
                     void make() {
                         std::lock_guard<std::mutex> l(make_m);
-                        if (main) return;
-                        HIP_OK(hipStreamCreateWithFlags(&up, hipStreamNonBlocking)); HIP_OK(hipStreamCreateWithFlags(&front, hipStreamNonBlocking));
+                        if (build[0]) return;
+                        HIP_OK(hipStreamCreateWithFlags(&up, hipStreamNonBlocking)); HIP_OK(hipStreamCreateWithFlags(&build[1], hipStreamNonBlocking));
                         HIP_OK(hipStreamCreateWithFlags(&down, hipStreamNonBlocking));
                         for (auto &e : sweep_done) HIP_OK(hipEventCreateWithFlags(&e, hipEventDisableTiming));
                         for (auto &e : build_done) HIP_OK(hipEventCreateWithFlags(&e, hipEventDisableTiming));
-                        HIP_OK(hipStreamCreateWithFlags(&main, hipStreamNonBlocking));
+                        HIP_OK(hipStreamCreateWithFlags(&build[0], hipStreamNonBlocking));
                     } };
 DeviceTurn &turn_of(int device) { static DeviceTurn turns[64]; return turns[device & 63]; }
 
@@ -382,7 +384,7 @@
 
 const int LANDING_ROOMS = 8;
 template <class F> void landing_rooms(agx_unit *u, F f) {
-    f(u->s_codes, true); f(u->s_hits, true); f(u->s_landing, false); f(u->s_codes_t, true); f(u->s_hits_t, true); f(u->s_runs, true); f(u->s_sides, true); f(u->s_other, true);
+    f(u->s_codes, true); f(u->s_hits, true); f(u->s_landing, false); f(u->s_codes_t, true); if (u->compact) f(u->s_chits, true); else f(u->s_hits_t, true); f(u->s_runs, true); f(u->s_sides, true); f(u->s_other, true);
 }
 
 void reserve_landing(agx_unit *u) {
@@ -423,10 +425,24 @@
 }
 void stage_tiled(agx_unit *u, unsigned threads) {
     u->tiled = false; u->n_other_t = 0; u->slot_row.clear(); u->n_win = 1;
+    u->compact = false; u->n_full = 0; u->common_len = 0;
+    auto no_compact = [u] { u->s_chits.release(); u->s_full_t.release(); u->s_cbase.release(); };
     const size_t nh = u->nh, s4 = u->stride / 4;
-    if (u->rows_diffed || getenv("AGX_NO_TILED_UPLOAD") || nh == 0 || u->n_rows == 0) { u->s_hits_t.release(); u->s_codes_t.release(); u->s_other_t.release(); return; }
+    if (u->rows_diffed || getenv("AGX_NO_TILED_UPLOAD") || nh == 0 || u->n_rows == 0) { u->s_hits_t.release(); u->s_codes_t.release(); u->s_other_t.release(); no_compact(); return; }
     const double t0 = now_ms();
-    u->s_hits_t.alloc(nh + 1); u->s_codes_t.alloc(nh * s4 + 16); u->slot_row.resize(nh);
+    {   const char *env = getenv("AGX_ROW_DIFF");
+        const bool diffs = env && atoi(env) != 0 && u->ref_packed && u->stride <= AGX_ROW_MAXSTRIDE;
+        const size_t S = std::min<size_t>(nh, 1024); std::vector<agx_u16> len(S);
+        for (size_t j = 0; j < S; j++) len[j] = u->s_hits.p[nh * j / S].len;
+        std::sort(len.begin(), len.end());
+        size_t best = 0;
+        for (size_t j = 0, k; j < S; j = k) { for (k = j; k < S && len[k] == len[j]; k++) { } if (k - j > best) { best = k - j; u->common_len = len[j]; } }
+        u->compact = !diffs && best * 4 >= S * 3;
+    }
+    const bool compact = u->compact;
+    const size_t n_groups = (nh + AGX_CGROUP - 1) / AGX_CGROUP;
+    if (compact) { u->s_chits.alloc(nh + 1); u->s_cbase.alloc(n_groups + 1); u->s_hits_t.release(); } else { u->s_hits_t.alloc(nh + 1); no_compact(); }
+    u->s_codes_t.alloc(nh * s4 + 16); u->slot_row.resize(nh);
     const agx_whit *wh = u->s_hits.p; const agx_wside *sd = u->s_sides.p; const agx_wrun *wr = u->s_runs.p; const agx_u32 *perm = u->s_perm.p;
     const size_t n_rows = u->n_rows; std::vector<agx_u8> has_other((n_rows + 7) / 8, 0);
     for (size_t j = 0; j < u->n_other; j++) { const size_t r = (size_t)(u->s_other.p[j] / u->stride); if (r < n_rows) has_other[r >> 3] |= (agx_u8)(1u << (r & 7)); }
@@ -437,11 +453,17 @@
     };
     const unsigned T = std::max(1u, std::min(threads, 16u));
     std::vector<std::vector<unsigned long long>> others(T);
+    std::atomic<bool> bad_side{false};
+    std::vector<std::vector<agx_whit>> fulls(T);
     on_threads(T, [&](unsigned t) {
         const size_t AHEAD = 48, NEAR = 24;
-        for (size_t i = nh * t / T, hi = nh * (t + 1) / T; i < hi; i++) {
+        agx_cbase in_group{0};
+        const size_t lo = std::min(nh, n_groups * t / T * AGX_CGROUP), hi = std::min(nh, n_groups * (t + 1) / T * AGX_CGROUP);
+        for (size_t i = lo; i < hi; i++) {
             if (i + AHEAD < hi) __builtin_prefetch(wh + perm[i + AHEAD]);
-            if (i + NEAR < hi) { const char *c = (const char *)(u->s_codes.p + (size_t)wh[perm[i + NEAR]].row * s4); __builtin_prefetch(c); if (s4 > 40) __builtin_prefetch(c + 64); }
+            if (i + NEAR < hi) {
+                const char *c = (const char *)(u->s_codes.p + (size_t)wh[perm[i + NEAR]].row * s4); __builtin_prefetch(c); if (s4 > 40) __builtin_prefetch(c + 64);
+            }
             const agx_u32 h = perm[i]; agx_whit w = wh[h];
             const agx_u32 row = w.row;
             u->slot_row[i] = row;
@@ -449,16 +471,29 @@
             bool dup = false;
             if (w.back) { const agx_u32 me = idx0(w); for (agx_u32 e = 1; e <= w.back && !dup; e++) dup = agx_absdiff(me, idx0(wh[h - e])) < (int)w.len; }
             w.row = h; if (dup) w.flags |= (agx_u8)AGX_WF_DUP;
-            u->s_hits_t.p[i] = w;
+            if (compact) {
+                if (i % AGX_CGROUP == 0) in_group = agx_cbase{0};
+                if ((w.flags & (AGX_WF_RUNS1 | AGX_WF_RUNS2)) && agx_whit_side(w) >= u->n_sides) bad_side.store(true);
+                if (agx_chit_pack(w, u->common_len, (agx_u32)u->n_sides, (agx_u32)nh, u->s_chits.p[i])) { fulls[t].push_back(w); in_group.full++; }
+                u->s_cbase.p[i / AGX_CGROUP] = in_group;
+            } else u->s_hits_t.p[i] = w;
             if (has_other[row >> 3] & (1u << (row & 7))) {
                 const unsigned long long lo = (unsigned long long)row * u->stride, *b = u->s_other.p, *e = b + u->n_other;
                 for (const unsigned long long *at = std::lower_bound(b, e, lo); at != e && *at < lo + u->stride; ++at) others[t].push_back((unsigned long long)i * u->stride + (*at - lo));
             }
         }
     });
+    if (bad_side.load()) throw Error{E_ARG, "a hit names a side record beyond the unit's side records"};
     size_t no = 0; for (auto &v : others) no += v.size();
     u->s_other_t.alloc(no + 1); u->n_other_t = no;
     { size_t at = 0; for (auto &v : others) { if (!v.empty()) memcpy(u->s_other_t.p + at, v.data(), v.size() * 8); at += v.size(); } }
+    if (compact) {
+        size_t nf = 0; for (auto &v : fulls) nf += v.size();
+        u->s_full_t.alloc(nf + 1); u->n_full = nf;
+        { size_t at = 0; for (auto &v : fulls) { if (!v.empty()) memcpy(u->s_full_t.p + at, v.data(), v.size() * sizeof(agx_whit)); at += v.size(); } }
+        agx_u32 front = 0;
+        for (size_t g = 0; g < n_groups; g++) { const agx_u32 own = u->s_cbase.p[g].full; u->s_cbase.p[g].full = front; front += own; }
+    }
     u->tiled = true;
     const size_t n_pos = u->V.n_pos ? u->V.n_pos : u->T.ref.size(), n_tiles = (n_pos + AGX_TILE - 1) / AGX_TILE;
     size_t W = getenv("AGX_UPLOAD_WINDOWS") ? (size_t)atoi(getenv("AGX_UPLOAD_WINDOWS")) : n_pos / 8000000u;
@@ -469,7 +504,7 @@
 }
 
 void stage_rows_tiled(agx_unit *u, unsigned threads) {
-    if (!u->tiled || !u->ref_packed || u->stride > AGX_ROW_MAXSTRIDE) return;
+    if (!u->tiled || u->compact || !u->ref_packed || u->stride > AGX_ROW_MAXSTRIDE) return;
     const char *env = getenv("AGX_ROW_DIFF");
     const size_t n_pos = u->V.n_pos ? u->V.n_pos : u->T.ref.size();
     if (!env || atoi(env) == 0) return;
@@ -776,7 +811,10 @@
     t(u->d_runs, u->n_runs + 1); t(u->d_vcodes, codes_bytes(u) * 4 + 16); t(u->d_other, others_up(u) + 1);
     if (u->rows_diffed) { t(u->d_units, u->n_units + 2); t(u->d_rowcnt, u->n_rowcnt); t(u->d_blockoff, u->n_blockoff); t(u->d_blockfirst, u->n_blockfirst); t(u->d_anchor, u->n_anchor); }
     else t(u->d_codes, codes_bytes(u) + 16);
-    t(u->d_whits, nh + 1); t(u->d_wsides, u->n_sides + 1); t(u->d_wruns, u->n_runs + 1); t(u->d_jump, u->n_jump + 1);
+    if (u->compact) { t(u->d_chits, nh + 1); t(u->d_wfull, u->n_full + 1); t(u->d_cbase, (nh + AGX_CGROUP - 1) / AGX_CGROUP + 1); }
+    else t(u->d_whits, nh + 1);
+    t(u->d_wsides, u->n_sides + 1);
+    t(u->d_wruns, u->n_runs + 1); t(u->d_jump, u->n_jump + 1);
     if (u->ref_packed) { t(u->d_wref, (n_pos + 3) / 4 + 32); t(u->d_refx, u->n_refx + 1); }
     t(u->d_dhit, nh + 1);
     t(u->d_perm, nh + 1); t(u->d_tfirst, n_tiles + 2); t(u->d_ckey, nh + 1); t(u->d_long, AGX_LONG_MAX);
@@ -937,7 +975,12 @@
         };
         up(u->d_segs.p, u->s_segs.p, u->n_segs * sizeof(agx_cmseg)); up(u->d_cntruns.p, u->s_cntruns.p, u->n_cntruns * sizeof(agx_cntrun));
         up(u->d_cntchunks.p, u->s_cntchunks.p, u->n_cntchunks * sizeof(agx_chunk)); up(u->d_segchunks.p, u->s_segchunks.p, u->n_segchunks * sizeof(agx_chunk)); up(u->d_segindex.p, u->s_segindex.p, u->n_segindex * 4);
-        up(u->d_whits.p, u->tiled ? u->s_hits_t.p : u->s_hits.p, nh * sizeof(agx_whit)); up(u->d_wsides.p, u->s_sides.p, u->n_sides * sizeof(agx_wside)); up(u->d_wruns.p, u->s_runs.p, u->n_runs * sizeof(agx_wrun)); up(u->d_jump.p, u->s_jump_at.p, u->n_jump * 4);
+        if (u->compact) {
+            up(u->d_chits.p, u->s_chits.p, nh * sizeof(agx_chit)); up(u->d_wfull.p, u->s_full_t.p, u->n_full * sizeof(agx_whit));
+            up(u->d_cbase.p, u->s_cbase.p, (nh + AGX_CGROUP - 1) / AGX_CGROUP * sizeof(agx_cbase));
+        } else up(u->d_whits.p, u->tiled ? u->s_hits_t.p : u->s_hits.p, nh * sizeof(agx_whit));
+        up(u->d_wsides.p, u->s_sides.p, u->n_sides * sizeof(agx_wside));
+        up(u->d_wruns.p, u->s_runs.p, u->n_runs * sizeof(agx_wrun)); up(u->d_jump.p, u->s_jump_at.p, u->n_jump * 4);
         if (!u->tiled) up(u->d_perm.p, u->s_perm.p, nh * 4);
         up(u->d_tfirst.p, u->s_tfirst.p, ((size_t)u->n_tiles + 2) * 4);
         HIP_OK(hipEventRecord(u->ev_hits, st));
@@ -1060,7 +1103,7 @@
         const double tb1 = now_ms();
         DeviceTurn &turn = turn_of(u->prm.device);
         std::unique_lock<std::mutex> my_turn(turn.m);
-        st = turn.front;
+        st = turn.build[turn.n & 1];
         if (turn.n) HIP_OK(hipStreamWaitEvent(st, (u->ev.all || turn.prev_exclusive) ? turn.build_done[(turn.n - 1) & 1] : turn.sweep_done[(turn.n - 1) & 1], 0));
         if (u->ev.all) HIP_OK(hipEventRecord(u->ev.first, st));
         if (!u->expanded) {
@@ -1077,8 +1120,9 @@
             HIP_OK(hipMemsetAsync(u->d_a_mark.p, 0, ids_cap + 2, st));
         }
         u->ev.begin(); u->ev.mark(B_START, st);
-        agx_prep_args PA{(const agx_whit *)u->d_whits.p, (const agx_wside *)u->d_wsides.p, u->d_runs.p, u->d_dhit.p, nh, u->prm.k, n_pos, u->d_tile_cnt.p, u->d_words.p + W_ERR,
-                         u->d_perm.p, u->d_tfirst.p, u->d_ckey.p, u->lookback, u->d_long.p, u->d_words.p + W_LONGCOUNT, u->tiled ? 1u : 0u, u->d_perm.p};
+        agx_prep_args PA{u->compact ? (const agx_whit *)u->d_chits.p : (const agx_whit *)u->d_whits.p, (const agx_wside *)u->d_wsides.p, u->d_runs.p, u->d_dhit.p, nh, u->prm.k, n_pos, u->d_tile_cnt.p, u->d_words.p + W_ERR,
+                         u->d_perm.p, u->d_tfirst.p, u->d_ckey.p, u->lookback, u->d_long.p, u->d_words.p + W_LONGCOUNT, u->compact ? 2u : u->tiled ? 1u : 0u, u->d_perm.p,
+                         u->d_cbase.p, u->d_wfull.p, u->common_len, (agx_u32)u->n_sides};
         agx_launch_hit_prep(&PA, st);
         AGX_CHECKPOINT("hit_prep");
         u->ev.mark(B_PREP, st);
@@ -1111,25 +1155,22 @@
             }
             u->expanded = true;
         }
-        HIP_OK(hipEventRecord(u->ev_front, st));
-        if (windows) {
+        auto expand_window = [&](agx_u32 w) {
             const size_t s4 = u->stride / 4;
-            for (agx_u32 w = 0; w < n_win; w++) {
+            {
                 const size_t r_lo = wr[w], r_hi = wr[w + 1];
                 if (early && w) HIP_OK(hipStreamWaitEvent(st, u->ev_rows[w], 0));
                 const unsigned long long *ob = u->s_other_t.p, *oe = ob + u->n_other_t;
                 const size_t o_lo = (size_t)(std::lower_bound(ob, oe, (unsigned long long)r_lo * u->stride) - ob), o_hi = (size_t)(std::lower_bound(ob, oe, (unsigned long long)r_hi * u->stride) - ob);
                 const size_t b_lo = r_lo * s4 * 4, b_hi = r_hi == (size_t)nh ? (codes_bytes(u) * 4 + 15) / 16 * 16 : r_hi * s4 * 4;
-                if (r_hi <= r_lo) { HIP_OK(hipEventRecord(u->ev_win[w], st)); continue; }
-                if (u->rows_diffed) agx_launch_expand_rows(u->d_whits.p, (agx_u32)nh, u->d_wsides.p, u->d_wruns.p, u->d_anchor.p, u->d_blockfirst.p + r_lo / 64, u->d_rowcnt.p + r_lo, u->d_blockoff.p + r_lo / 64, u->d_units.p, u->d_wref.p,
-                                                           u->d_vcodes.p + b_lo, (agx_u32)(r_hi - r_lo), u->stride, nullptr, 0, st);
-                else agx_launch_expand_codes(u->d_codes.p + r_lo * s4, u->d_vcodes.p + b_lo, b_hi - b_lo, nullptr, 0, st);
-                agx_launch_patch_codes(u->d_other.p + o_lo, o_hi - o_lo, u->d_vcodes.p, st);
-                HIP_OK(hipEventRecord(u->ev_win[w], st));
+                if (r_hi > r_lo) {
+                    if (u->rows_diffed) agx_launch_expand_rows(u->d_whits.p, (agx_u32)nh, u->d_wsides.p, u->d_wruns.p, u->d_anchor.p, u->d_blockfirst.p + r_lo / 64, u->d_rowcnt.p + r_lo, u->d_blockoff.p + r_lo / 64, u->d_units.p, u->d_wref.p,
+                                                               u->d_vcodes.p + b_lo, (agx_u32)(r_hi - r_lo), u->stride, nullptr, 0, st);
+                    else agx_launch_expand_codes(u->d_codes.p + r_lo * s4, u->d_vcodes.p + b_lo, b_hi - b_lo, nullptr, 0, st);
+                    agx_launch_patch_codes(u->d_other.p + o_lo, o_hi - o_lo, u->d_vcodes.p, st);
+                }
             }
-        }
-        st = turn.main;
-        HIP_OK(hipStreamWaitEvent(st, u->ev_front, 0));
+        };
         u->ev.mark(B_BIN, st);
         agx_node_kargs K; fill_sweep_args(u, K.S);
 #ifdef AGX_SWEEP_STATS
@@ -1143,7 +1184,10 @@
         K.huge_count = u->d_words.p + W_HUGECOUNT; K.huge_n = u->d_words.p + W_HUGECOUNT; K.huge_list = u->d_huge_list.p; K.scratch_huge = u->d_scratch_huge.p; K.huge_queued = u->huge ? 1u : 0u;
         for (agx_u32 w = 0; w < n_win; w++) {
             K.tile_lo = windows ? wt[w] : 0u; K.tile_hi = windows ? wt[w + 1] : u->n_tiles;
-            if (windows) { HIP_OK(hipStreamWaitEvent(st, u->ev_win[w], 0)); HIP_OK(hipEventRecord(u->ev_sw0[w], st)); }
+            if (windows) {
+                expand_window(w);
+                HIP_OK(hipEventRecord(u->ev_sw0[w], st));
+            }
             agx_launch_node_sweep(&K, st);
             if (windows) HIP_OK(hipEventRecord(u->ev_sw1[w], st));
         }
@@ -1159,21 +1203,12 @@
         E.n_hits = nh; E.jump_list = u->d_jump.p; E.n_jump = (agx_u32)u->n_jump; E.abort = u->d_words.p + W_STATUS; E.big_list = u->d_big_list.p; E.big_n = u->d_words.p + W_BIGCOUNT; E.slow_list = u->d_slow_list.p; E.slow_count = u->d_words.p + W_SLOWCOUNT;
         agx_launch_edge_sweep(&E, st);
         AGX_CHECKPOINT("edge_sweep");
-        const bool side_j = !u->ev.all && !g_debug_sync;
-        if (side_j) {
-            HIP_OK(hipEventRecord(u->ev_passA, st));
-            HIP_OK(hipStreamWaitEvent(turn.front, u->ev_passA, 0));
-            agx_launch_edge_jump(&E, turn.front);
-            HIP_OK(hipEventRecord(u->ev_passJ, turn.front));
-        } else {
-            agx_launch_edge_jump(&E, st);
-            AGX_CHECKPOINT("edge_jump");
-        }
+        agx_launch_edge_jump(&E, st);
+        AGX_CHECKPOINT("edge_jump");
         u->ev.mark(B_EDGE, st);
         agx_launch_edge_slow(&E, st);
         AGX_CHECKPOINT("edge_slow");
         u->ev.mark(B_SLOW, st);
-        if (side_j) HIP_OK(hipStreamWaitEvent(st, u->ev_passJ, 0));
         queue_walk_prep(u, st, [&] {
             u->ev.mark(B_COMPACT, st);
             u->stats.edge_sweep_launches++;
@@ -1260,7 +1295,8 @@
         const size_t ids_cap = (size_t)n_pos + u->pool_cap;
         {
             std::unique_lock<std::mutex> my_turn(turn.m);
-            hipStream_t st = turn.main;
+            hipStream_t st = turn.build[turn.n & 1];
+            if (turn.n) HIP_OK(hipStreamWaitEvent(st, turn.sweep_done[(turn.n - 1) & 1], 0));
             agx_zero_args Z; memset(&Z, 0, sizeof Z);
             auto seg = [&](int i, agx_u32 *ptr, size_t words) { Z.p[i] = ptr; Z.n[i] = (agx_u32)words; };
             seg(0, u->d_words.p + W_N, W_TOTAL - W_N); seg(1, u->d_tile_side.p + u->n_tiles, 1); seg(2, u->d_sp_cnt.p, (size_t)u->n_words + 1);
@@ -1622,10 +1658,9 @@
         try { u->helper.start(); } catch (...) { }
         HIP_OK(hipSetDevice(p->device));
         u->ev.init(); u->ev.all = (u->prm.flags & AGX_FLAG_TIME_SECTIONS) != 0;
-        for (hipEvent_t *e : {&u->ev_front, &u->ev_passA, &u->ev_passJ}) HIP_OK(hipEventCreateWithFlags(e, hipEventDisableTiming));
         for (hipEvent_t *e : {&u->ev_dl, &u->ev_built, &u->ev_hits}) HIP_OK(hipEventCreateWithFlags(e, hipEventDisableTiming));
         HIP_OK(hipEventCreate(&u->ev_up0)); HIP_OK(hipEventCreate(&u->ev_uploaded));
-        for (int i = 0; i < 8; i++) { HIP_OK(hipEventCreateWithFlags(&u->ev_rows[i], hipEventDisableTiming)); HIP_OK(hipEventCreateWithFlags(&u->ev_win[i], hipEventDisableTiming)); HIP_OK(hipEventCreate(&u->ev_sw0[i])); HIP_OK(hipEventCreate(&u->ev_sw1[i])); }
+        for (int i = 0; i < 8; i++) { HIP_OK(hipEventCreateWithFlags(&u->ev_rows[i], hipEventDisableTiming)); HIP_OK(hipEventCreate(&u->ev_sw0[i])); HIP_OK(hipEventCreate(&u->ev_sw1[i])); }
         u->dl_sdma = hsa_copy().agent_of(p->device, u->dl_agent) && hsa_signal_create(0, 0, nullptr, &u->dl_signal) == HSA_STATUS_SUCCESS;
     });
     if (rc != AGX_OK) { delete u; return rc; }
@@ -1979,6 +2014,14 @@
     return rc;
 }
 
+int agx_unit_hit_form(agx_unit *u, uint64_t *out) {
+    if (!u || !out) return AGX_E_ARG;
+    return guarded(u, [&] {
+        if (!u->staged) throw Error{E_ARG, "hit form: the unit is not staged"};
+        out[0] = u->compact ? 2u : u->tiled ? 1u : 0u; out[1] = u->nh; out[2] = u->n_full; out[3] = u->n_sides; out[4] = u->common_len; out[5] = others_up(u);
+    });
+}
+
 void agx_front_free(agx_front *f) {
     if (!f) return;
     free(f->ref); free(f->vcodes); free(f->runs); free(f->cm_start); free(f->cm); free(f->cm_head); free(f->dhit); free(f->perm); free(f->tile_first); free(f->ckey);
diff --git a/aligngraph_amd/csrc/agx_kargs.h b/aligngraph_amd/csrc/agx_kargs.h
--- a/aligngraph_amd/csrc/agx_kargs.h
+++ b/aligngraph_amd/csrc/agx_kargs.h
@@ -9,6 +9,7 @@
     agx_u32 *err;
     const agx_u32 *perm, *tile_first; agx_u32 *ckey; agx_u32 lookback; agx_u32 *long_list, *long_count;
     agx_u32 tiled; agx_u32 *perm_out;
+    const agx_cbase *cbase; const agx_whit *full; agx_u32 common_len, n_sides;
 };
 
 struct agx_bin_args { const agx_dhit *dhit; agx_u32 n_hits; const agx_u32 *tile_off; agx_u32 *cursor; agx_u32 *unsorted; agx_u32 cap;
diff --git a/aligngraph_amd/csrc/agx_kernels.hip b/aligngraph_amd/csrc/agx_kernels.hip
--- a/aligngraph_amd/csrc/agx_kernels.hip
+++ b/aligngraph_amd/csrc/agx_kernels.hip
@@ -108,7 +108,20 @@
     const agx_u32 i = blockIdx.x * 256u + threadIdx.x, lane = threadIdx.x & 63u;
     const bool mine = i < A.n_hits;
     agx_dhit d; d.flags = AGX_HF_SKIP; d.x_lo = 1; d.x_hi = 0; d.a_nruns = 0;
-    if (mine) {
+    if (A.tiled == 2u) {
+        const agx_chit *ch = (const agx_chit *)A.whits;
+        agx_chit c; c.p = 0; c.number = 0; c.d = 0; c.flags = 0; c.back = 0;
+        if (mine) c = ch[i];
+        const unsigned long long m_full = __ballot((c.flags & AGX_CF_FULL) != 0);
+        if (mine) {
+            const agx_u32 rank = A.cbase[i / AGX_CGROUP].full + (agx_u32)__popcll(m_full & ((1ull << lane) - 1ull));
+            const agx_hit H = agx_chit_unpack(c, A.common_len, A.n_sides, A.n_hits, A.full, rank, A.sides);
+            A.perm_out[i] = c.number;
+            const int rc = agx_hit_prep(H, (c.flags & AGX_WF_DUP) != 0, (H.pad[0] & 1u) != 0, i, A.runs, A.k, d);
+            if (rc) atomicOr(A.err, 1u);
+            if (!(d.flags & AGX_HF_SKIP) && (d.x_hi >= A.n_pos || d.x_lo > d.x_hi)) { atomicOr(A.err, 2u); d.flags |= AGX_HF_SKIP; }
+        }
+    } else if (mine) {
         const agx_whit *wh = A.whits; const agx_wside *sd = A.sides;
         const agx_u32 h = A.tiled ? i : A.perm[i];
         const agx_whit w = wh[h];
diff --git a/include/agx.h b/include/agx.h
--- a/include/agx.h
+++ b/include/agx.h
@@ -227,6 +227,7 @@
 void agx_walk_graph_free(agx_walk_graph *g);
 int agx_unit_front(agx_unit *u, agx_front *f);
 void agx_front_free(agx_front *f);
+int agx_unit_hit_form(agx_unit *u, uint64_t out[6]);
 int agx_unit_unitigs(agx_unit *u, agx_unitigs *t);
 int agx_unit_unitigs_region(agx_unit *u, uint32_t pos_lo, uint32_t pos_hi, uint32_t min_coverage, agx_unitigs *t);
 int agx_unit_unitigs_mapped(agx_unit *u, uint32_t pos_lo, uint32_t pos_hi, uint32_t min_coverage, agx_unitigs *t, agx_idmap *m);
```

Result: slower. 1.179 billion (-12.5%).
